# rslmtoasa/rslmtoasa

Hardware: AMD Instinct MI355X
Metric: block-recursion throughput (H|psi> + A_n + B_n recursion levels, recursion.f90 recur_b) (higher is better)
Workload: dtype f64

## Files before the change

### rslmtoasa_amd/csrc/kernels_mfma.hpp

```cpp
#pragma once
#include <hip/hip_runtime.h>
#include <string>
#include <vector>
#include "kernels_valu.hpp"

namespace rsrec {

typedef double double4_t __attribute__((ext_vector_type(4)));

constexpr int GROUP = 8;
constexpr int MF_WAVES = 4;

struct LayoutCI {
    static __device__ __forceinline__ double2 ld(const double* b, int r, int c) { return make_double2(b[36 * r + 2 * c], b[36 * r + 2 * c + 1]); }
    static __device__ __forceinline__ void st(double* b, int r, int c, double2 v) { b[36 * r + 2 * c] = v.x; b[36 * r + 2 * c + 1] = v.y; }
};
__host__ __device__ constexpr int gram_col(int part, int c, int ci) { return ci ? 2 * c + part : 18 * part + c; }

__device__ __forceinline__ int active_workgroups(int ngroups) { return max(1, min((int)gridDim.x, (ngroups + MF_WAVES - 1) / MF_WAVES)); }

struct GroupWalk {
    int g, end, step;
    __device__ __forceinline__ GroupWalk(int ngroups, int wave, int nbx_eff = 0) {
        const int nbx = nbx_eff > 0 ? nbx_eff : gridDim.x, bx = blockIdx.x;
        const int xcd = bx & 7, j = bx >> 3;
        const int per_xcd = (nbx >> 3) + ((xcd < (nbx & 7)) ? 1 : 0);
        const int chunk = (ngroups + 7) >> 3;
        const int lo = xcd * chunk;
        end = min(ngroups, lo + chunk);
        g = lo + j * MF_WAVES + wave;
        step = per_xcd * MF_WAVES;
        if (nbx < 8) { g = bx * MF_WAVES + wave; end = ngroups; step = nbx * MF_WAVES; }
    }
};


struct RowRef { unsigned off; bool valid; };
__device__ __forceinline__ RowRef group_row(const int* __restrict__ grp, int rho, int zero_block) {
    const int slot = rho / 18, r = rho - 18 * slot;
    const int a = grp[slot];
    RowRef R;
    R.valid = a >= 0;
    R.off = (unsigned)BLD * (unsigned)(R.valid ? a : zero_block) + 36u * (unsigned)r;
    return R;
}

struct GramAcc {
    double4_t t00, t01, t10, t11;
    double tr0, tr1;
    double t0r, t1r;
    double trr;
    __device__ __forceinline__ void zero() { t00 = t01 = t10 = t11 = (double4_t){0, 0, 0, 0}; tr0 = tr1 = t0r = t1r = trr = 0.0; }
    __device__ __forceinline__ void to_lds(double* G , int lane, bool sym) const {
        const int l15 = lane & 15, l4 = lane >> 4, l3 = lane & 3, lg = (lane >> 2) & 3;
#pragma unroll
        for (int j = 0; j < 4; ++j) {
            const int r = l4 + 4 * j;
            G[36 * r + l15] = t00[j];
            G[36 * r + 16 + l15] = t01[j];
            G[36 * (16 + r) + 16 + l15] = t11[j];
            if (!sym) G[36 * (16 + r) + l15] = t10[j];
        }
        G[36 * (32 + l4) + l15] = tr0;
        G[36 * (32 + l4) + 16 + l15] = tr1;
        if (!sym) { G[36 * (4 * lg + l4) + 32 + l3] = t0r; G[36 * (16 + 4 * lg + l4) + 32 + l3] = t1r; }
        if (lg == 0) G[36 * (32 + l4) + 32 + l3] = trr;
    }
};

__device__ __forceinline__ void gram_block_out(const GramAcc& A, double* lds , double* gout , bool sym) {
    const int lane = threadIdx.x & 63, wave = threadIdx.x >> 6;
    A.to_lds(lds + wave * 1296, lane, sym);
    __syncthreads();
    for (int e = threadIdx.x; e < 1296; e += blockDim.x) {
        double s = 0.0;
#pragma unroll
        for (int wv = 0; wv < MF_WAVES; ++wv) s += lds[wv * 1296 + e];
        if (sym) {
            const int r = e / 36, c = e % 36;
            const bool have = (r >= 32) || (r < 16) || (c >= 16 && c < 32);
            if (!have || (r < 32 && c >= 32)) {
                double t = 0.0;
#pragma unroll
                for (int wv = 0; wv < MF_WAVES; ++wv) t += lds[wv * 1296 + 36 * c + r];
                s = t;
            }
        }
        gout[e] = s;
    }
}

#ifndef RSREC_NT_STREAMS
#define RSREC_NT_STREAMS 0
#endif
template <class T> __device__ __forceinline__ T ld_stream(const T* p) {
#if RSREC_NT_STREAMS
    return __builtin_nontemporal_load(p);
#else
    return *p;
#endif
}
__device__ __forceinline__ double2 ld_stream(const double2* p) {
#if RSREC_NT_STREAMS
    typedef double nt_d2 __attribute__((ext_vector_type(2)));
    const nt_d2 v = __builtin_nontemporal_load(reinterpret_cast<const nt_d2*>(p));
    return make_double2(v[0], v[1]);
#else
    return *p;
#endif
}
template <class T> __device__ __forceinline__ void st_stream(T* p, T v) {
#if RSREC_NT_STREAMS
    __builtin_nontemporal_store(v, p);
#else
    *p = v;
#endif
}

#ifndef ADOT_UNROLL
#define ADOT_UNROLL 4
#endif
__global__ __launch_bounds__(MF_WAVES * 64, 2) void k_mfma_adot(ChainView CV, int level, int zero_block, const double* __restrict__ psi,
                                                               const double* __restrict__ tvec, double* partial ) {
    __shared__ double lds[MF_WAVES * 1296];
    const int chain = blockIdx.y;
    const int lane = threadIdx.x & 63;
    const int wave = __builtin_amdgcn_readfirstlane(threadIdx.x >> 6);
    const int ngroups = CV.count_of(chain, level) / GROUP;
    const int* order = CV.order_of(chain, level);
    const size_t vo = (size_t)chain * CV.vstride;
    const double* ps = psi + vo;
    const double* tv = tvec + vo;
    const int l15 = lane & 15, l4 = lane >> 4, l3 = lane & 3;
    GramAcc A;
    A.zero();
    const int nbx = active_workgroups(ngroups);
    for (GroupWalk w((int)blockIdx.x < nbx ? ngroups : 0, wave, nbx); w.g < w.end; w.g += w.step) {
        const int* grp = order + (size_t)w.g * GROUP;
#pragma unroll ADOT_UNROLL
        for (int kq = 0; kq < 36; ++kq) {
            const RowRef rk = group_row(grp, 4 * kq + l4, zero_block);
            const double p0 = ld_stream(ps + rk.off + l15), p1 = ld_stream(ps + rk.off + 16 + l15), pr = ld_stream(ps + rk.off + 32 + l3);
            const double h0 = ld_stream(tv + rk.off + l15), h1 = ld_stream(tv + rk.off + 16 + l15), hr = ld_stream(tv + rk.off + 32 + l3);
            A.t00 = __builtin_amdgcn_mfma_f64_16x16x4f64(p0, h0, A.t00, 0, 0, 0);
            A.t01 = __builtin_amdgcn_mfma_f64_16x16x4f64(p0, h1, A.t01, 0, 0, 0);
            A.t10 = __builtin_amdgcn_mfma_f64_16x16x4f64(p1, h0, A.t10, 0, 0, 0);
            A.t11 = __builtin_amdgcn_mfma_f64_16x16x4f64(p1, h1, A.t11, 0, 0, 0);
            A.tr0 = __builtin_amdgcn_mfma_f64_4x4x4f64(pr, h0, A.tr0, 0, 0, 0);
            A.tr1 = __builtin_amdgcn_mfma_f64_4x4x4f64(pr, h1, A.tr1, 0, 0, 0);
            A.t0r = __builtin_amdgcn_mfma_f64_4x4x4f64(p0, hr, A.t0r, 0, 0, 0);
            A.t1r = __builtin_amdgcn_mfma_f64_4x4x4f64(p1, hr, A.t1r, 0, 0, 0);
            A.trr = __builtin_amdgcn_mfma_f64_4x4x4f64(pr, hr, A.trr, 0, 0, 0);
        }
    }
    gram_block_out(A, lds, partial + ((size_t)chain * gridDim.x + blockIdx.x) * 1296, false);
}

struct SpmmDims {
    int kk, nslots, nmax, nlev, cpo, ostride, level; size_t vstride; const int* obase; int nchains = 0;
    int sat_base = 0, run_lo = 0, run_hi = 0, nskip = 0, skip_lo[4] = {0, 0, 0, 0}, skip_hi[4] = {0, 0, 0, 0};
    int nruns = 0, run_tau[4] = {0, 0, 0, 0}, run_glo[4] = {0, 0, 0, 0}, run_ghi[4] = {0, 0, 0, 0}, run_row0[5] = {0, 0, 0, 0, 0};
    int skip_pa = 0;
};

__device__ __forceinline__ double2 reduce_gram(const double* __restrict__ partial , int nblk, double* lds , int ci = 0) {
    for (int e = threadIdx.x; e < 1296; e += blockDim.x) {
        double s = 0.0;
        for (int p = 0; p < nblk; ++p) s += partial[(size_t)p * 1296 + e];
        lds[e] = s;
    }
    __syncthreads();
    double2 c = make_double2(0, 0);
    if (threadIdx.x < BLK) {
        const int cp = threadIdx.x % NB, cc = threadIdx.x / NB;
        const int rp = gram_col(0, cp, ci), ip = gram_col(1, cp, ci), rc = gram_col(0, cc, ci), ic = gram_col(1, cc, ci);
        c.x = lds[36 * rp + rc] + lds[36 * ip + ic];
        c.y = lds[36 * rp + ic] - lds[36 * ip + rc];
    }
    __syncthreads();
    return c;
}

}
```

### rslmtoasa_amd/csrc/kernels_spmm5.hpp

```cpp
#pragma once
#include <hip/hip_runtime.h>
#include <algorithm>
#include <type_traits>
#include <vector>
#include "kernels_valu.hpp"
#include "kernels_mfma.hpp"
#include "kernels_spmm4.hpp"

namespace rsrec {

#ifndef RSREC_S5_KSPLIT_PROBE
#define RSREC_S5_KSPLIT_PROBE 0
#endif
#ifndef RSREC_S5_PRIO
#define RSREC_S5_PRIO 0
#endif
#ifndef S5_WG_GROUPS
#define S5_WG_GROUPS 4
#endif
constexpr int S5_TRIPLE = 640;
constexpr int S5_TRIPLE_BYTES = S5_TRIPLE * 8;
constexpr int S5_HEAD_TRIPLES = 2;
constexpr int S5_HEAD_DOUBLES = 2 * S5_HEAD_TRIPLES * S5_TRIPLE;
constexpr int S5_MAXENT = 2 * S4_MAXSLOTS + 2;
// ... 262 lines not shown
struct S5Acc { double4_t m[9]; double r[9]; };

struct S5Ent { unsigned off[GROUP]; unsigned rem; };

template <int S> struct S5St {
    static constexpr int T = S / 3, K = S % 3;
    static constexpr int W = K == 2 ? 2 : 4;
    static constexpr int o0 = 10 * T + (K == 0 ? 0 : K == 1 ? 4 : 8);
    static constexpr int eA = o0 / 9, mA0 = o0 % 9, sp = 9 - mA0;
    static constexpr bool straddle = sp < W;
    static constexpr bool opens = straddle || mA0 == 0;
    static constexpr int eOpen = mA0 == 0 ? eA : eA + 1;
};

template <int NL, int NM>
__device__ __forceinline__ void s5_interleave() {
    constexpr int PER = NM / NL;
#pragma unroll
    for (int i = 0; i < NL; ++i) {
        __builtin_amdgcn_sched_group_barrier(0x20, 1, 0);
        __builtin_amdgcn_sched_group_barrier(0x8, PER, 0);
    }
    __builtin_amdgcn_sched_group_barrier(0x8, NM - PER * NL, 0);
}

template <int NL = 11>
__device__ __forceinline__ void s5_mfma(S5Acc& acc, const S5Pair& o) {
#pragma unroll
    for (int e = 0; e < 2; ++e)
#pragma unroll
        for (int t = 0; t < 9; ++t) {
            acc.m[t] = __builtin_amdgcn_mfma_f64_16x16x4f64(o.a[0][e], o.b[t][e], acc.m[t], 0, 0, 0);
            acc.r[t] = __builtin_amdgcn_mfma_f64_4x4x4f64(o.a[1][e], o.b[t][e], acc.r[t], 0, 0, 0);
        }
    s5_interleave<NL, 36>();
}
template <int NL = 11>
__device__ __forceinline__ void s5_mfma(S5Acc& acc, const S5Single& o) {
#pragma unroll
    for (int t = 0; t < 9; ++t) {
        acc.m[t] = __builtin_amdgcn_mfma_f64_16x16x4f64(o.a[0], o.b[t], acc.m[t], 0, 0, 0);
        acc.r[t] = __builtin_amdgcn_mfma_f64_4x4x4f64(o.a[1], o.b[t], acc.r[t], 0, 0, 0);
    }
    s5_interleave<NL, 18>();
}

template <int N> using S5C = std::integral_constant<int, N>;
#define S5_GLOBAL __attribute__((address_space(1)))
#define S5_CONST __attribute__((address_space(4)))
#define S5_LDS __attribute__((address_space(3)))
typedef const S5_GLOBAL char* s5_gp;

template <bool TWO, bool LDSA, bool OCT = false>
__device__ __forceinline__ void s5_run_stream(S5Acc& acc, const int* __restrict__ meta, const char* __restrict__ fr , const char* __restrict__ fr_head,
                                              const char* __restrict__ inb, const char* __restrict__ in2b,
                                              const int* __restrict__ nbr5 ,
                                              const int (&atom)[GROUP] , int rem_sel ,
                                              int ncol, int sig, int l4,
                                              unsigned lane_main, unsigned lane_z, unsigned lane_rem, unsigned lane_rem_z, unsigned lane16, unsigned lane8,
                                              const int (&tile_blk)[GROUP], int rem_blk , int kpart = 0) {
    int left = meta[0];
    int ebase = 0, tbase = 0;
    bool first = true;
#if RSREC_S5_KSPLIT_PROBE
    if (kpart == 0) left = min(left, 27);
    else { left -= 27; ebase = 10; tbase = 9; first = false; }
#endif
    if (left <= 0) return;
    const bool extras = TWO && meta[1] != 0;
    const S5_CONST int* codes = (const S5_CONST int*)(meta + 2);
    const S5_CONST int* nbr = (const S5_CONST int*)nbr5;
    S5Ent E0, E1;
    int raw[GROUP];
    int code_cur = codes[ebase], code_nxt = codes[ebase + 1];
    auto load_idx = [&](int col) {
#pragma unroll
        for (int t = 0; t < GROUP; ++t) raw[t] = nbr[(size_t)ncol * atom[t] + col];
    };
    load_idx(code_cur & 255);
    unsigned vlane_main = lane_main, vlane_z = lane_z, vlane16 = lane16, vlane8 = lane8;
    auto open_entry = [&](int j, S5Ent& E) {
        const unsigned so = 2592u * (unsigned)((code_cur >> 8) ? 1 - sig : sig);
#pragma unroll
        for (int t = 0; t < GROUP; ++t) E.off[t] = (unsigned)(OCT ? raw[t] + tile_blk[t] : raw[t]) * (BLD * 8u) + so;
        const int r01 = (rem_sel & 1) ? raw[1] : raw[0], r23 = (rem_sel & 1) ? raw[3] : raw[2], r45 = (rem_sel & 1) ? raw[5] : raw[4], r67 = (rem_sel & 1) ? raw[7] : raw[6];
        const int r03 = (rem_sel & 2) ? r23 : r01, r47 = (rem_sel & 2) ? r67 : r45;
        E.rem = (unsigned)(((rem_sel & 4) ? r47 : r03) + (OCT ? rem_blk : 0)) * (BLD * 8u) + so;
        code_cur = code_nxt;
        code_nxt = codes[j + 2];
        load_idx(code_cur & 255);
    };
    auto issue = [&](auto s2c, auto& o) {
        constexpr int S2 = decltype(s2c)::value, S = S2 % 27, wrap = S2 / 27;
        using I = S5St<S>;
        S5Ent& EA = (I::eA & 1) ? E1 : E0;
        S5Ent& EB = (I::eA & 1) ? E0 : E1;
        if constexpr (I::opens) open_entry(ebase + 10 * wrap + I::eOpen, (I::eOpen & 1) ? E1 : E0);
        const bool head = wrap == 0 && first && extras;
        const char* __restrict__ base = (TWO && S < 5 && head) ? in2b : inb;
        s5_gp fbg = nullptr;
        if constexpr (!LDSA) {
            const char* fb = ((TWO && I::T < S5_HEAD_TRIPLES && head && fr_head) ? fr_head + I::T * S5_TRIPLE_BYTES
                                                                                 : fr + (size_t)(tbase + 9 * wrap + I::T) * S5_TRIPLE_BYTES)
                             + (I::K == 0 ? 0 : I::K == 1 ? 2048 : 4096);
            fbg = (s5_gp)fb;
            asm("" : "+s"(fbg));
        }
        constexpr unsigned rowA = 288u * I::mA0, rowB = 0u - 288u * I::sp;
        unsigned& lm = I::K < 2 ? vlane_main : vlane_z;
        unsigned& lf = I::K < 2 ? vlane16 : vlane8;
        const unsigned lr = I::K < 2 ? lane_rem : lane_rem_z;
        asm volatile("" : "+v"(lm));
        asm volatile("" : "+v"(lf));
        using V = std::remove_reference_t<decltype(o.b[0])>;
        if constexpr (!I::straddle) {
#pragma unroll
            for (int t = 0; t < GROUP; ++t) {
                s5_gp pt = (s5_gp)base + EA.off[t];
                asm("" : "+s"(pt));
                o.b[t] = *(const S5_GLOBAL V*)(pt + lm + rowA);
            }
            o.b[8] = *(const S5_GLOBAL V*)((s5_gp)base + (EA.rem + lr) + rowA);
        } else {
            const bool inB = (I::K < 2 ? l4 : (l4 >> 1)) >= I::sp;
#pragma unroll
            for (int t = 0; t < GROUP; ++t) {
                const unsigned off = (inB ? EB.off[t] + rowB : EA.off[t] + rowA) + lm;
                o.b[t] = *(const S5_GLOBAL V*)((s5_gp)base + off);
            }
            const unsigned off = (inB ? EB.rem + rowB : EA.rem + rowA) + lr;
            o.b[8] = *(const S5_GLOBAL V*)((s5_gp)base + off);
        }
        if constexpr (LDSA) {
            const S5_LDS char* fl = (const S5_LDS char*)fr + (unsigned)(tbase + 9 * wrap + I::T) * S5_TRIPLE_BYTES + (I::K == 0 ? 0 : I::K == 1 ? 2048 : 4096);
#pragma unroll
            for (int q = 0; q < 2; ++q) o.a[q] = *(const S5_LDS V*)(fl + lf + q * (I::K < 2 ? 1024 : 512));
        } else if constexpr (I::K < 2) {
#pragma unroll
            for (int q = 0; q < 2; ++q) o.a[q] = *(const S5_GLOBAL V*)(fbg + lf + q * 1024);
        } else {
#pragma unroll
            for (int q = 0; q < 2; ++q) o.a[q] = *(const S5_GLOBAL V*)(fbg + lf + q * 512);
        }
    };
    S5Pair X, Y;
    S5Single Z;
    issue(S5C<0>{}, X);
    issue(S5C<1>{}, Y);
#define S5_STEP(S, NEXT, CUR)                 \
    if (left > (S)) {                         \
        issue(S5C<(S) + 2>{}, NEXT);          \
        s5_mfma<LDSA ? 9 : 11>(acc, CUR);     \
        __builtin_amdgcn_sched_barrier(0);    \
    }
    for (;; left -= 27) {
        S5_STEP(0, Z, X) S5_STEP(1, X, Y) S5_STEP(2, Y, Z) S5_STEP(3, Z, X) S5_STEP(4, X, Y) S5_STEP(5, Y, Z)
        S5_STEP(6, Z, X) S5_STEP(7, X, Y) S5_STEP(8, Y, Z) S5_STEP(9, Z, X) S5_STEP(10, X, Y) S5_STEP(11, Y, Z)
        S5_STEP(12, Z, X) S5_STEP(13, X, Y) S5_STEP(14, Y, Z) S5_STEP(15, Z, X) S5_STEP(16, X, Y) S5_STEP(17, Y, Z)
        S5_STEP(18, Z, X) S5_STEP(19, X, Y) S5_STEP(20, Y, Z) S5_STEP(21, Z, X) S5_STEP(22, X, Y) S5_STEP(23, Y, Z)
        S5_STEP(24, Z, X) S5_STEP(25, X, Y) S5_STEP(26, Y, Z)
        if (left <= 27) break;
        ebase += 10; tbase += 9; first = false;
    }
#undef S5_STEP
}


template <int NT> struct S5PairN { s5_d2 b[NT]; s5_d2 a[2]; };
template <int NT> struct S5SingleN { double b[NT]; double a[2]; };
template <int NT> struct S5AccN { double4_t m[NT]; double r[NT]; };

template <int NT>
__device__ __forceinline__ void s5_mfma_n(S5AccN<NT>& acc, const S5PairN<NT>& o) {
#pragma unroll
    for (int e = 0; e < 2; ++e)
#pragma unroll
        for (int t = 0; t < NT; ++t) {
            acc.m[t] = __builtin_amdgcn_mfma_f64_16x16x4f64(o.a[0][e], o.b[t][e], acc.m[t], 0, 0, 0);
            acc.r[t] = __builtin_amdgcn_mfma_f64_4x4x4f64(o.a[1][e], o.b[t][e], acc.r[t], 0, 0, 0);
        }
    s5_interleave<NT, 4 * NT>();
}
template <int NT>
__device__ __forceinline__ void s5_mfma_n(S5AccN<NT>& acc, const S5SingleN<NT>& o) {
#pragma unroll
    for (int t = 0; t < NT; ++t) {
        acc.m[t] = __builtin_amdgcn_mfma_f64_16x16x4f64(o.a[0], o.b[t], acc.m[t], 0, 0, 0);
        acc.r[t] = __builtin_amdgcn_mfma_f64_4x4x4f64(o.a[1], o.b[t], acc.r[t], 0, 0, 0);
    }
    s5_interleave<NT, 2 * NT>();
}

struct S5EntN { unsigned off[3]; unsigned rem; };

template <bool TWO, int NMAIN, bool HASREM>
__device__ __forceinline__ void s5_run_stream_n(S5AccN<NMAIN + (HASREM ? 1 : 0)>& acc, const int* __restrict__ meta, const char* __restrict__ fr ,
                                                const char* __restrict__ inb, const char* __restrict__ in2b, const int* __restrict__ nbr5,
                                                const int (&atom)[NMAIN], const int (&ratom)[GROUP], int rem_sel, int ncol, int sig, int l4,
                                                unsigned lane_main, unsigned lane_z, unsigned lane_rem, unsigned lane_rem_z, unsigned lane16, unsigned lane8) {
    constexpr int NT = NMAIN + (HASREM ? 1 : 0);
    int left = meta[0];
    int ebase = 0, tbase = 0;
    bool first = true;
    if (left <= 0) return;
    const bool extras = TWO && meta[1] != 0;
    const S5_CONST int* codes = (const S5_CONST int*)(meta + 2);
    const S5_CONST int* nbr = (const S5_CONST int*)nbr5;
    S5EntN E0, E1;
    int raw[NMAIN], rraw[GROUP];
    int code_cur = codes[ebase], code_nxt = codes[ebase + 1];
    auto load_idx = [&](int col) {
#pragma unroll
        for (int t = 0; t < NMAIN; ++t) raw[t] = nbr[(size_t)ncol * atom[t] + col];
        if constexpr (HASREM) {
#pragma unroll
            for (int t = 0; t < GROUP; ++t) rraw[t] = nbr[(size_t)ncol * ratom[t] + col];
        }
    };
    load_idx(code_cur & 255);
    unsigned vlane_main = lane_main, vlane_z = lane_z, vlane16 = lane16, vlane8 = lane8;
    auto open_entry = [&](int j, S5EntN& E) {
        const unsigned so = 2592u * (unsigned)((code_cur >> 8) ? 1 - sig : sig);
#pragma unroll
        for (int t = 0; t < NMAIN; ++t) E.off[t] = (unsigned)raw[t] * (BLD * 8u) + so;
        if constexpr (HASREM) {
            const int r01 = (rem_sel & 1) ? rraw[1] : rraw[0], r23 = (rem_sel & 1) ? rraw[3] : rraw[2], r45 = (rem_sel & 1) ? rraw[5] : rraw[4], r67 = (rem_sel & 1) ? rraw[7] : rraw[6];
            const int r03 = (rem_sel & 2) ? r23 : r01, r47 = (rem_sel & 2) ? r67 : r45;
            E.rem = (unsigned)((rem_sel & 4) ? r47 : r03) * (BLD * 8u) + so;
        }
        code_cur = code_nxt;
        code_nxt = codes[j + 2];
        load_idx(code_cur & 255);
    };
    auto issue = [&](auto s2c, auto& o) {
        constexpr int S2 = decltype(s2c)::value, S = S2 % 27, wrap = S2 / 27;
        using I = S5St<S>;
        S5EntN& EA = (I::eA & 1) ? E1 : E0;
        S5EntN& EB = (I::eA & 1) ? E0 : E1;
        if constexpr (I::opens) open_entry(ebase + 10 * wrap + I::eOpen, (I::eOpen & 1) ? E1 : E0);
        const bool head = wrap == 0 && first && extras;
        const char* __restrict__ base = (TWO && S < 5 && head) ? in2b : inb;
        constexpr unsigned rowA = 288u * I::mA0, rowB = 0u - 288u * I::sp;
        unsigned& lm = I::K < 2 ? vlane_main : vlane_z;
        unsigned& lf = I::K < 2 ? vlane16 : vlane8;
        const unsigned lr = I::K < 2 ? lane_rem : lane_rem_z;
        asm volatile("" : "+v"(lm));
        asm volatile("" : "+v"(lf));
        using V = std::remove_reference_t<decltype(o.b[0])>;
        if constexpr (!I::straddle) {
#pragma unroll
            for (int t = 0; t < NMAIN; ++t) {
                s5_gp pt = (s5_gp)base + EA.off[t];
                asm("" : "+s"(pt));
                o.b[t] = *(const S5_GLOBAL V*)(pt + lm + rowA);
            }
            if constexpr (HASREM) o.b[NMAIN] = *(const S5_GLOBAL V*)((s5_gp)base + (EA.rem + lr) + rowA);
        } else {
            const bool inB = (I::K < 2 ? l4 : (l4 >> 1)) >= I::sp;
#pragma unroll
            for (int t = 0; t < NMAIN; ++t) {
                const unsigned off = (inB ? EB.off[t] + rowB : EA.off[t] + rowA) + lm;
                o.b[t] = *(const S5_GLOBAL V*)((s5_gp)base + off);
            }
            if constexpr (HASREM) {
                const unsigned off = (inB ? EB.rem + rowB : EA.rem + rowA) + lr;
                o.b[NMAIN] = *(const S5_GLOBAL V*)((s5_gp)base + off);
            }
        }
        const S5_LDS char* fl = (const S5_LDS char*)fr + (unsigned)(tbase + 9 * wrap + I::T) * S5_TRIPLE_BYTES + (I::K == 0 ? 0 : I::K == 1 ? 2048 : 4096);
#pragma unroll
        for (int q = 0; q < 2; ++q) o.a[q] = *(const S5_LDS V*)(fl + lf + q * (I::K < 2 ? 1024 : 512));
    };
    S5PairN<NT> X0, Y0, X1, Y1;
    S5SingleN<NT> Z0, Z1;
    issue(S5C<0>{}, X0);
    issue(S5C<1>{}, Y0);
    issue(S5C<2>{}, Z0);
    issue(S5C<3>{}, X1);
    issue(S5C<4>{}, Y1);
#define S5_STEP(S, NEXT, CUR)                 \
    if (left > (S)) {                         \
        issue(S5C<(S) + 5>{}, NEXT);          \
        s5_mfma_n<NT>(acc, CUR);              \
        __builtin_amdgcn_sched_barrier(0);    \
    }
    for (;; left -= 54) {
        S5_STEP(0, Z1, X0) S5_STEP(1, X0, Y0) S5_STEP(2, Y0, Z0) S5_STEP(3, Z0, X1) S5_STEP(4, X1, Y1) S5_STEP(5, Y1, Z1)
        S5_STEP(6, Z1, X0) S5_STEP(7, X0, Y0) S5_STEP(8, Y0, Z0) S5_STEP(9, Z0, X1) S5_STEP(10, X1, Y1) S5_STEP(11, Y1, Z1)
        S5_STEP(12, Z1, X0) S5_STEP(13, X0, Y0) S5_STEP(14, Y0, Z0) S5_STEP(15, Z0, X1) S5_STEP(16, X1, Y1) S5_STEP(17, Y1, Z1)
        S5_STEP(18, Z1, X0) S5_STEP(19, X0, Y0) S5_STEP(20, Y0, Z0) S5_STEP(21, Z0, X1) S5_STEP(22, X1, Y1) S5_STEP(23, Y1, Z1)
        S5_STEP(24, Z1, X0) S5_STEP(25, X0, Y0) S5_STEP(26, Y0, Z0) S5_STEP(27, Z0, X1) S5_STEP(28, X1, Y1) S5_STEP(29, Y1, Z1)
        S5_STEP(30, Z1, X0) S5_STEP(31, X0, Y0) S5_STEP(32, Y0, Z0) S5_STEP(33, Z0, X1) S5_STEP(34, X1, Y1) S5_STEP(35, Y1, Z1)
        S5_STEP(36, Z1, X0) S5_STEP(37, X0, Y0) S5_STEP(38, Y0, Z0) S5_STEP(39, Z0, X1) S5_STEP(40, X1, Y1) S5_STEP(41, Y1, Z1)
        S5_STEP(42, Z1, X0) S5_STEP(43, X0, Y0) S5_STEP(44, Y0, Z0) S5_STEP(45, Z0, X1) S5_STEP(46, X1, Y1) S5_STEP(47, Y1, Z1)
        S5_STEP(48, Z1, X0) S5_STEP(49, X0, Y0) S5_STEP(50, Y0, Z0) S5_STEP(51, Z0, X1) S5_STEP(52, X1, Y1) S5_STEP(53, Y1, Z1)
        if (left <= 54) break;
        ebase += 20; tbase += 18; first = false;
    }
#undef S5_STEP
}

struct S5Epilogue { int kind = 0; const double* cur = nullptr; const double* old = nullptr; double a = 1.0, b = 0.0; };

template <bool TWO, bool LDSA, bool OCT = false, int NSP = 1>
__global__ __launch_bounds__(NSP == 3 ? 768 : S5_WG_GROUPS * 128) void k_spmm5(SpmmDims D, const int* __restrict__ order_all, const int* __restrict__ cum,
                                               const int* __restrict__ nbr ,
                                               const int* __restrict__ izp, const double* __restrict__ frag, const int* __restrict__ meta, int ntr,
                                               const double* __restrict__ in_all, double* __restrict__ out_all,
                                               const double* __restrict__ in2_all = nullptr,
                                               const double* __restrict__ frag_head = nullptr ,
                                               int ntau = 0, int lds_tau = 0 ,
                                               int* __restrict__ queue = nullptr ,
                                               int spin_by_xcd = 1 ,
                                               S5Epilogue epi = S5Epilogue()) {
    extern __shared__ double s5_lds[];
    const int lane = threadIdx.x & 63;
    const int wave = __builtin_amdgcn_readfirstlane(threadIdx.x >> 6);
    const int sig = LDSA ? (int)((spin_by_xcd ? blockIdx.x : (blockIdx.x >> 3)) & 1) : wave / S5_WG_GROUPS, gslot = LDSA ? wave : wave % S5_WG_GROUPS;
#if RSREC_S5_PRIO
    if (wave >= (int)(blockDim.x >> 7)) __builtin_amdgcn_s_setprio(1);
#endif
    const int WGG = LDSA ? (int)(blockDim.x >> 6) : S5_WG_GROUPS;
    int bxl = blockIdx.x, gdxl = gridDim.x, run_lo = D.run_lo, run_hi = D.run_hi, qrun = 0;
    if (LDSA && D.nruns > 0) {
        const int row = spin_by_xcd ? 8 : 16, rowi = (int)blockIdx.x / row;
        int r = 0;
#pragma unroll
        for (int q = 1; q < 4; ++q) if (q < D.nruns && rowi >= D.run_row0[q]) r = q;
        lds_tau = D.run_tau[r]; run_lo = D.run_glo[r]; run_hi = D.run_ghi[r];
        bxl = (int)blockIdx.x - row * D.run_row0[r];
        gdxl = row * (D.run_row0[r + 1] - D.run_row0[r]);
        qrun = r;
    }
    if constexpr (LDSA) {
        const s5_d2* __restrict__ src = reinterpret_cast<const s5_d2*>(frag + ((size_t)lds_tau * 2 + sig) * ntr * S5_TRIPLE);
        s5_d2* dst = reinterpret_cast<s5_d2*>(s5_lds);
        const int n = ntr * (S5_TRIPLE / 2);
        constexpr int PER = (int)(160 * 1024 / 16 / (NSP == 3 ? 512 : S5_WG_GROUPS * 64));
        const int nthr = (int)blockDim.x;
        s5_d2 v[PER];
#pragma unroll
        for (int i = 0; i < PER; ++i) { const int e = threadIdx.x + i * nthr; if (e < n) v[i] = src[e]; }
#pragma unroll
        for (int i = 0; i < PER; ++i) { const int e = threadIdx.x + i * nthr; if (e < n) dst[e] = v[i]; }
        __syncthreads();
    }
    const int l15 = lane & 15, l4 = lane >> 4;
    const unsigned lane_main = 8u * (36 * l4 + 2 * l15), lane_z = 8u * (36 * (l4 >> 1) + 2 * l15 + (l4 & 1));
    const unsigned lane_rem = 8u * (36 * l4 + 32 + 2 * (l15 & 1)), lane_rem_z = 8u * (36 * (l4 >> 1) + 32 + 2 * (l15 & 1) + (l4 & 1));
    const unsigned lane16 = 16u * lane, lane8 = 8u * lane;
    const int ncol = D.nslots + 2;
#pragma unroll 1
    for (int chain = OCT ? GROUP * (int)blockIdx.y : (int)blockIdx.y; chain < D.nchains; chain += OCT ? GROUP * (int)gridDim.y : (int)gridDim.y) {
    const int count = cum[(chain / D.cpo) * D.nlev + D.level];
    int ngroups = count / GROUP;
    const int ob = D.obase[(chain / D.cpo) * D.nlev + D.level];
    const int* __restrict__ order = order_all + (size_t)(chain / D.cpo) * D.ostride + ob;
    const bool on_full_list = D.sat_base > 0 && ob == D.sat_base;
    if constexpr (OCT) ngroups = D.nmax;
    else if (run_hi > 0) {
        if (!on_full_list) continue;
        order += (size_t)run_lo * GROUP;
        ngroups = run_hi - run_lo;
    }
    const bool skipping = D.nskip > 0 && on_full_list;
    const size_t vo = (size_t)chain * D.vstride;
    const char* __restrict__ inb = reinterpret_cast<const char*>(in_all + vo);
    const char* __restrict__ in2b = TWO ? reinterpret_cast<const char*>(in2_all + vo) : nullptr;
    double* __restrict__ out = out_all + vo;
    const int zero_block = D.kk;

    int g, gend, gstep, glo = 0;
    bool dynamic = false;
    {
        const int bx = bxl;
        const int need = (ngroups + WGG - 1) / WGG;
        if constexpr (!LDSA) {
            const int nbx = max(1, min((int)gridDim.x, need));
            if (bx >= nbx) continue;
            if (nbx < 8) { g = bx * WGG + gslot; gend = ngroups; gstep = nbx * WGG; }
            else {
                const int xcd = bx & 7, j = bx >> 3;
                const int per_xcd = (nbx >> 3) + ((xcd < (nbx & 7)) ? 1 : 0);
                const int chunk = (ngroups + 7) >> 3;
                const int lo = xcd * chunk;
                gend = min(ngroups, lo + chunk);
                g = lo + j * WGG + gslot;
                gstep = per_xcd * WGG;
            }
        } else {
            const int row = spin_by_xcd ? 8 : 16;
            const int nbx = max(row, min(gdxl / row * row, (2 * need + row - 1) / row * row));
            if (bx >= nbx) continue;
            const int xcd = bx & 7, j = bx >> 3;
            if (2 * need <= row) {
                const int per_spin = row / 2, idx = spin_by_xcd ? (xcd >> 1) : xcd;
                if (j >= row / 8) continue;
                g = idx * WGG + gslot; gend = ngroups; gstep = per_spin * WGG;
            } else {
                const int rows = nbx / row;
                const int nchunk = spin_by_xcd ? 4 : 8, ichunk = spin_by_xcd ? (xcd >> 1) : xcd;
                const int chunk = (ngroups + nchunk - 1) / nchunk;
                const int lo = ichunk * chunk;
                gend = min(ngroups, lo + chunk);
                g = lo + (spin_by_xcd ? j : (j >> 1)) * WGG + gslot;
                gstep = rows * WGG;
                glo = lo;
                dynamic = queue != nullptr;
            }
        }
    }
    int* __restrict__ ctr = dynamic ? queue + ((size_t)qrun * D.nchains + chain) * 16 + 2 * (blockIdx.x & 7) + (spin_by_xcd ? 0 : sig) : nullptr;
    int part = 0;
    auto next_task = [&]() {
        if (NSP == 3 && !dynamic && part < 2) { ++part; return; }
        part = 0; g += gstep;
    };
    for (;; next_task()) {
        int kpart = 0;
        if (dynamic) {
            int gi = 0;
            if (lane == 0) gi = atomicAdd(ctr, 1);
            gi = __builtin_amdgcn_readfirstlane(gi);
#if RSREC_S5_KSPLIT_PROBE
            kpart = gi & 1; gi >>= 1;
#endif
            if constexpr (NSP == 3) { const unsigned gu = (unsigned)gi, gq = gu / 3u; part = (int)(gu - 3u * gq); gi = (int)gq; }
            g = glo + gi;
        }
        if (g >= gend) break;
        if (skipping) {
            bool skip = false;
#pragma unroll
            for (int r = 0; r < 4; ++r) skip |= r < D.nskip && g >= D.skip_lo[r] && g < D.skip_hi[r];
            if (skip) continue;
        }
        const int* __restrict__ grp = order + (size_t)g * GROUP;
        if constexpr (NSP == 3) {
            static_assert(NSP != 3 || (LDSA && !OCT), "split tasks: LDS / persistent form only");
            const int g0 = grp[0];
            const int first3 = g0 >= 0 ? g0 : zero_block;
            if (D.skip_pa && first3 < D.nmax) continue;
            const int tau3 = first3 < D.nmax ? first3 : D.nmax + izp[first3];
            const int* __restrict__ M3 = meta + (size_t)tau3 * Spmm5Operator::META;
            const char* __restrict__ fr3 = reinterpret_cast<const char*>(s5_lds);
            S5AccN<3> acc3;
#pragma unroll
            for (int t = 0; t < 3; ++t) { acc3.m[t] = (double4_t){0, 0, 0, 0}; acc3.r[t] = 0.0; }
            auto finish3 = [&](auto remc, const int (&av)[3]) {
                constexpr bool REM = decltype(remc)::value;
                size_t eo[3];
#pragma unroll
                for (int i = 0; i < 3; ++i) eo[i] = (size_t)BLD * av[i] + 324 * sig + ((REM && i == 2) ? 32 + 2 * (l15 & 1) : 2 * l15);
                s5_d2 ec[3][2], ez[3][2];
                double ecr[3], ezr[3];
                if (epi.kind) {
                    const double* cb = epi.cur + vo;
#pragma unroll
                    for (int i = 0; i < 3; ++i) {
#pragma unroll
                        for (int p = 0; p < 2; ++p) ec[i][p] = *reinterpret_cast<const s5_d2*>(cb + eo[i] + 36 * (4 * p + l4));
                        ecr[i] = cb[eo[i] + 288 + (l4 & 1)];
                    }
                    if (epi.kind == 2) {
                        const double* zb = epi.old + vo;
#pragma unroll
                        for (int i = 0; i < 3; ++i) {
#pragma unroll
                            for (int p = 0; p < 2; ++p) ez[i][p] = *reinterpret_cast<const s5_d2*>(zb + eo[i] + 36 * (4 * p + l4));
                            ezr[i] = zb[eo[i] + 288 + (l4 & 1)];
                        }
                    }
                }
#pragma unroll
                for (int i = 0; i < 3; ++i) {
                    const int a = av[i];
                    double* ob = out + eo[i];
#pragma unroll
                    for (int p = 0; p < 2; ++p) {
                        s5_d2 v; v[0] = acc3.m[i][2 * p]; v[1] = acc3.m[i][2 * p + 1];
                        if (epi.kind) {
                            v[0] = (v[0] - epi.b * ec[i][p][0]) / epi.a; v[1] = (v[1] - epi.b * ec[i][p][1]) / epi.a;
                            if (epi.kind == 2) { v[0] = v[0] * 2.0 - ez[i][p][0]; v[1] = v[1] * 2.0 - ez[i][p][1]; }
                        }
                        if (a != zero_block) *reinterpret_cast<s5_d2*>(ob + 36 * (4 * p + l4)) = v;
                    }
                    double r = acc3.r[i];
                    if (epi.kind) {
                        r = (r - epi.b * ecr[i]) / epi.a;
                        if (epi.kind == 2) r = r * 2.0 - ezr[i];
                    }
                    if (a != zero_block && l4 < 2) ob[288 + l4] = r;
                }
            };
            int ratom[GROUP];
            if (part < 2) {
                int a3[3];
#pragma unroll
                for (int j = 0; j < 3; ++j) { const int a = grp[3 * part + j]; a3[j] = a >= 0 ? a : zero_block; }
#pragma unroll
                for (int t = 0; t < GROUP; ++t) ratom[t] = zero_block;
                s5_run_stream_n<TWO, 3, false>(acc3, M3, fr3, inb, in2b, nbr, a3, ratom, 0, ncol, sig, l4, lane_main, lane_z, lane_rem, lane_rem_z, lane16, lane8);
                finish3(std::false_type{}, a3);
            } else {
#pragma unroll
                for (int t = 0; t < GROUP; ++t) { const int a = grp[t]; ratom[t] = a >= 0 ? a : zero_block; }
                const int a2[2] = {ratom[6], ratom[7]};
                int mra = grp[l15 >> 1];
                mra = mra >= 0 ? mra : zero_block;
                s5_run_stream_n<TWO, 2, true>(acc3, M3, fr3, inb, in2b, nbr, a2, ratom, l15 >> 1, ncol, sig, l4, lane_main, lane_z, lane_rem, lane_rem_z, lane16, lane8);
                const int av[3] = {a2[0], a2[1], mra};
                finish3(std::true_type{}, av);
            }
            continue;
        }
        int atom[GROUP];
        int vatom[GROUP], tile_blk[GROUP];
        int my_rem_atom, rem_blk = 0;
        if constexpr (OCT) {
            const int a0 = g;
#pragma unroll
            for (int t = 0; t < GROUP; ++t) {
                const bool ok = a0 >= 0 && chain + t < D.nchains;
                atom[t] = ok ? a0 : zero_block;
                tile_blk[t] = ok ? t * (D.kk + 1) : 0;
                vatom[t] = ok ? a0 + t * (D.kk + 1) : zero_block;
            }
            const int tr = l15 >> 1;
            const bool okr = a0 >= 0 && chain + tr < D.nchains;
            rem_blk = okr ? tr * (D.kk + 1) : 0;
            my_rem_atom = okr ? a0 + tr * (D.kk + 1) : zero_block;
        } else {
#pragma unroll
            for (int t = 0; t < GROUP; ++t) { const int a = grp[t]; atom[t] = a >= 0 ? a : zero_block; vatom[t] = atom[t]; tile_blk[t] = 0; }
            my_rem_atom = grp[l15 >> 1];
            my_rem_atom = my_rem_atom >= 0 ? my_rem_atom : zero_block;
        }
        const int first = atom[0];
        if (!OCT && D.skip_pa && first < D.nmax) continue;
        const int tau = first < D.nmax ? first : D.nmax + izp[first];
        const int* __restrict__ M = meta + (size_t)tau * Spmm5Operator::META;
        const char* __restrict__ fr = LDSA ? reinterpret_cast<const char*>(s5_lds) : reinterpret_cast<const char*>(frag + ((size_t)tau * 2 + sig) * ntr * S5_TRIPLE);
        const char* __restrict__ fh = (TWO && frag_head) ? reinterpret_cast<const char*>(frag_head + ((size_t)chain * ntau + tau) * S5_HEAD_DOUBLES + (size_t)sig * S5_HEAD_TRIPLES * S5_TRIPLE) : nullptr;

        S5Acc acc;
#pragma unroll
        for (int t = 0; t < 9; ++t) { acc.m[t] = (double4_t){0, 0, 0, 0}; acc.r[t] = 0.0; }

        if constexpr (OCT) s5_run_stream<TWO, LDSA, true>(acc, M, fr, fh, inb, in2b, nbr, atom, l15 >> 1, ncol, sig, l4, lane_main, lane_z, lane_rem, lane_rem_z, lane16, lane8, tile_blk, rem_blk);
        else s5_run_stream<TWO, LDSA>(acc, M, fr, fh, inb, in2b, nbr, atom, l15 >> 1, ncol, sig, l4, lane_main, lane_z, lane_rem, lane_rem_z, lane16, lane8, tile_blk, rem_blk, kpart);
#if RSREC_S5_KSPLIT_PROBE
        if (kpart) continue;
#endif

        auto finish = [&](auto t0c, auto t1c) {
            constexpr int T0 = decltype(t0c)::value, T1 = decltype(t1c)::value, NT = T1 - T0;
            size_t eo[NT];
#pragma unroll
            for (int i = 0; i < NT; ++i) { const int t = T0 + i; eo[i] = (size_t)BLD * ((t < 8) ? vatom[t] : my_rem_atom) + 324 * sig + ((t < 8) ? 2 * l15 : 32 + 2 * (l15 & 1)); }
            s5_d2 ec[NT][2], ez[NT][2];
            double ecr[NT], ezr[NT];
            if (epi.kind) {
                const double* cb = epi.cur + vo;
#pragma unroll
                for (int i = 0; i < NT; ++i) {
#pragma unroll
                    for (int p = 0; p < 2; ++p) ec[i][p] = *reinterpret_cast<const s5_d2*>(cb + eo[i] + 36 * (4 * p + l4));
                    ecr[i] = cb[eo[i] + 288 + (l4 & 1)];
                }
                if (epi.kind == 2) {
                    const double* zb = epi.old + vo;
#pragma unroll
                    for (int i = 0; i < NT; ++i) {
#pragma unroll
                        for (int p = 0; p < 2; ++p) ez[i][p] = *reinterpret_cast<const s5_d2*>(zb + eo[i] + 36 * (4 * p + l4));
                        ezr[i] = zb[eo[i] + 288 + (l4 & 1)];
                    }
                }
            }
#pragma unroll
            for (int i = 0; i < NT; ++i) {
                const int t = T0 + i;
                const int a = (t < 8) ? vatom[t] : my_rem_atom;
                double* ob = out + eo[i];
#pragma unroll
                for (int p = 0; p < 2; ++p) {
                    s5_d2 v; v[0] = acc.m[t][2 * p]; v[1] = acc.m[t][2 * p + 1];
                    if (epi.kind) {
                        v[0] = (v[0] - epi.b * ec[i][p][0]) / epi.a; v[1] = (v[1] - epi.b * ec[i][p][1]) / epi.a;
                        if (epi.kind == 2) { v[0] = v[0] * 2.0 - ez[i][p][0]; v[1] = v[1] * 2.0 - ez[i][p][1]; }
                    }
                    if (a != zero_block) *reinterpret_cast<s5_d2*>(ob + 36 * (4 * p + l4)) = v;
                }
                double r = acc.r[t];
                if (epi.kind) {
                    r = (r - epi.b * ecr[i]) / epi.a;
                    if (epi.kind == 2) r = r * 2.0 - ezr[i];
                }
                if (a != zero_block && l4 < 2) ob[288 + l4] = r;
            }
        };
        finish(S5C<0>{}, S5C<5>{});
        finish(S5C<5>{}, S5C<9>{});
    }
    }
}

}
```

### rslmtoasa_amd/csrc/rsrec.hip

```cpp
#include <hip/hip_runtime.h>
#include <hsa/hsa.h>
#include <hsa/hsa_ext_amd.h>
#include <dlfcn.h>
#include <algorithm>
#include <atomic>
#include <chrono>
#include <cmath>
#include <cstdarg>
#include <cstdio>
#include <cstdlib>
#include <cstring>
#include <memory>
#include <string>
#include <thread>
#include <tuple>
#include <vector>

#include "../../include/rsrec.h"
#include "kernels_valu.hpp"
#include "kernels_mfma.hpp"
#include "kernels_spmm4.hpp"
#include "kernels_spmm5.hpp"
#include "kernels_uscheme.hpp"
#include "kernels_green.hpp"
#include "kernels_ldos.hpp"
#include "kernels_spectra.hpp"
#include "kernels_kubo.hpp"
#include "kernels_cond.hpp"
#include "kernels_exchange.hpp"
#include "kernels_auxgreen.hpp"
#include "kernels_contour.hpp"
#include "kernels_assemble.hpp"

using namespace rsrec;

namespace {

struct DevBuf {
    void* p = nullptr;
    size_t bytes = 0;
    DevBuf() = default;
    DevBuf(DevBuf&& o) noexcept : p(o.p), bytes(o.bytes) { o.p = nullptr; o.bytes = 0; }
    DevBuf& operator=(DevBuf&& o) noexcept { std::swap(p, o.p); std::swap(bytes, o.bytes); return *this; }
    ~DevBuf() { release(); }
    hipError_t reserve(size_t n) {
        if (n <= bytes) return hipSuccess;
        release();
        hipError_t e = hipMalloc(&p, n);
        if (e == hipSuccess) bytes = n;
        return e;
    }
    void release() { if (p) (void)hipFree(p); p = nullptr; bytes = 0; }
    template <class T> T* as() const { return reinterpret_cast<T*>(p); }
};

}

struct rsrec_handle {
    int device = 0;
    hipStream_t stream = nullptr;
    hipStream_t copy_stream = nullptr;
    hipEvent_t ev_green[2] = {nullptr, nullptr};
    hipStream_t side_stream = nullptr;
    hipEvent_t ev_orth = nullptr, ev_bred = nullptr;
    hipStream_t oct_stream = nullptr;
    hipEvent_t ev_oct_in = nullptr, ev_oct_out = nullptr;
    size_t p2_slot = 0;
    std::string err;
    bool have_lattice = false, have_ham = false;
    std::vector<int32_t> lat_nn, lat_iz;
    int lat_nncols = 0;
    std::vector<double> lat_cr;
    int kk = 0, nslots = 0, nmax = 0, ntype = 0;
    std::vector<int> nbr;
    std::vector<int> iz0;
    std::vector<int> radj_ptr, radj;
    DevBuf d_nbr, d_iz, d_nbr5;
    int hslots = 0, hoh = 0, nsp = 2;
    DevBuf d_hst, d_hloc, d_host, d_holoc, d_enim, d_lsham;
    Spmm4Operator s4_op;
    int s4_built_split = 0;
    Spmm5Operator s5_op;
    DevBuf d_s5queue;
    int s5_built = 0;
    size_t s5_lds_limit = (size_t)-1;
    int n_cu = 0;
    bool s4_attr = false;
    size_t term_lds = 0, cheb_ldos_lds = (size_t)64 * 1024, cheb_spec_lds = (size_t)64 * 1024;
    std::vector<double> host_ee, host_lsham, host_eeo, host_enim, host_hall, host_hallo;
    std::vector<double> host_st, host_loc;
    DevBuf d_asm[2][2], d_asm_in;
    std::vector<double> asm_host[2][2];
    int asm_nslots[2] = {0, 0}, asm_ncls[2] = {0, 0}, asm_hoh[2] = {0, 0};
    int n_octet_launch = 0;
    int n_asm_reused = 0;
    long n_asm_calls = 0, n_ldos_calls = 0, n_recursion_calls = 0;
    Spmm5Operator s5_la; int s5_la_ok = 0;
    DevBuf d_la_extra, d_rot;
    Spmm5Operator kubo_op[2], kubo_hbulk;
    Spmm5Operator orb_plain;
    DevBuf d_green_in, d_green_out;
    DevBuf d_kubo[5];
    DevBuf d_cond[4];
    DevBuf d_ctens[2];
    DevBuf d_bsqrt, d_term, d_gim, d_ldos;
    DevBuf d_ops, d_spec;
    void* pin = nullptr;
    size_t pin_bytes = 0;
    DevBuf d_frags, d_vec[6], d_partial, d_partial2, d_coefA, d_coefB, d_bmats, d_status, d_seed, d_seedcoef, d_mu, d_scal, d_zsqr;
    long opt_batch = 0, opt_kernels = 0, opt_nblk = 0, opt_spmm5 = 2, opt_chain_fold = 1, opt_s5_cap = 0, opt_side = 1, opt_s5_lds = 1, opt_s5_queue = 1, opt_cheb_fused = 1;
    long opt_s5_waves = 8;
    long opt_sat_pct = 100;
    long opt_orth_oop = 1;
    long opt_s5_split = 0;
    long opt_s5_run_min = 0;
    long opt_s5_spin_xcd = 0;
    long opt_s5_octet = 8;
    long opt_s5_host_emit = 0;
    long opt_kubo_lchunk = 0;
    long opt_kubo_vbatch = 0;
    int n_kubo_left_chunks = 0;
    int kubo_diag_nvec = 0, kubo_diag_ll = 0;
    long opt_orth3 = 1;
    long opt_graph = 1;
    hipGraphExec_t graph_exec = nullptr;
    std::vector<uintptr_t> graph_key;
    bool capturing = false;
    double t_total_ms = 0, t_hop_ms = 0, t_rest_ms = 0, t_host_ms = 0;
    double t_rot_ms = 0;
    double n_hop_launch = 0, n_atom_steps = 0, n_block_mult = 0, n_hop_mfma_flop = 0;
    double n_req_flop = 0;
    int hop_fuses_a = 1;
    std::vector<hipEvent_t> ev_pool;
    size_t ev_used = 0;
    struct RegionEntry {
        std::vector<int> seeds;
        int nlev, napply, flags, epoch, ostride;
        double atom_steps, block_mults;
        DevBuf order, cum;
        std::vector<int> level_max;
        std::vector<double> level_groups;
        std::vector<double> mult_hist;
        struct ClassRun { int tau, lo, hi; };
        std::vector<ClassRun> sat_runs;
        std::vector<int> level_sat;
        int sat_base = 0;
    };
    std::vector<std::unique_ptr<RegionEntry>> region_cache;
    int lattice_epoch = 0;
    const int* cur_order = nullptr;
    const int* cur_cum = nullptr;
    const std::vector<int>* cur_level_max = nullptr;
    const std::vector<double>* cur_level_groups = nullptr;
    const std::vector<double>* cur_mult_hist = nullptr;
    const RegionEntry* cur_entry = nullptr;
    int cur_nrows = 0;
    std::vector<unsigned> spatial_key;
    int res_kind = 0, res_n = 0, res_lld = 0;
    bool res_seeded = false;
    void* comm = nullptr;
    int comm_rank = 0, comm_nranks = 1;
    DevBuf d_comm;
    ~rsrec_handle();
};

namespace {

struct OptionEntry { const char* name; long rsrec_handle::*member; };
const OptionEntry OPTIONS[] = {
    {"batch", &rsrec_handle::opt_batch},
    {"kernels", &rsrec_handle::opt_kernels},
    {"nblk", &rsrec_handle::opt_nblk},
    {"spmm5", &rsrec_handle::opt_spmm5},
    {"chain_fold", &rsrec_handle::opt_chain_fold},
    {"s5_cap", &rsrec_handle::opt_s5_cap},
    {"s5_lds", &rsrec_handle::opt_s5_lds},
    {"s5_queue", &rsrec_handle::opt_s5_queue},
    {"cheb_fused", &rsrec_handle::opt_cheb_fused},
    {"side_stream", &rsrec_handle::opt_side},
    {"graph", &rsrec_handle::opt_graph},
    {"orth3", &rsrec_handle::opt_orth3},
    {"s5_waves", &rsrec_handle::opt_s5_waves},
    {"s5_split", &rsrec_handle::opt_s5_split},
    {"orth_oop", &rsrec_handle::opt_orth_oop},
    {"sat_pct", &rsrec_handle::opt_sat_pct},
    {"kubo_lchunk", &rsrec_handle::opt_kubo_lchunk},
    {"kubo_vbatch", &rsrec_handle::opt_kubo_vbatch},
    {"s5_host_emit", &rsrec_handle::opt_s5_host_emit},
    {"s5_octet", &rsrec_handle::opt_s5_octet},
    {"s5_spin_xcd", &rsrec_handle::opt_s5_spin_xcd},
    {"s5_run_min", &rsrec_handle::opt_s5_run_min},
};

int fail(rsrec_t* h, int code, const char* fmt, ...) {
    char buf[512];
    va_list ap;
    va_start(ap, fmt);
    vsnprintf(buf, sizeof buf, fmt, ap);
    va_end(ap);
    if (h) h->err = buf;
    return code;
}

#define HIPCK(h, call)                                                                                         \
    do {                                                                                                       \
        hipError_t e_ = (call);                                                                                \
        if (e_ != hipSuccess) return fail(h, RSREC_ERR_DEVICE, "%s failed: %s (%s:%d)", #call, hipGetErrorString(e_), __FILE__, __LINE__); \
    } while (0)

hipEvent_t next_event(rsrec_t* h) {
    static const bool off = getenv("RSREC_NO_EVENTS") != nullptr;
    if (off || h->capturing) return nullptr;
    if (h->ev_used == h->ev_pool.size()) {
        hipEvent_t e;
        if (hipEventCreate(&e) != hipSuccess) return nullptr;
        h->ev_pool.push_back(e);
    }
    hipEvent_t e = h->ev_pool[h->ev_used++];
    (void)hipEventRecord(e, h->stream);
    return e;
}

constexpr size_t PIN_BYTES = (size_t)8 << 20;
int pin_ready(rsrec_t* h) {
    if (h->pin) return RSREC_OK;
    if (hipHostMalloc(&h->pin, PIN_BYTES, hipHostMallocDefault) != hipSuccess) { h->pin = nullptr; return fail(h, RSREC_ERR_DEVICE, "hipHostMalloc of the staging buffer failed"); }
    h->pin_bytes = PIN_BYTES;
    return RSREC_OK;
}
constexpr size_t PIN_MAX_XFER = (size_t)8 << 20;
int xfer_d2h(rsrec_t* h, void* dst, const void* src_dev, size_t bytes) {
    if (bytes > PIN_MAX_XFER) {
        HIPCK(h, hipMemcpyAsync(dst, src_dev, bytes, hipMemcpyDeviceToHost, h->stream));
        HIPCK(h, hipStreamSynchronize(h->stream));
        return RSREC_OK;
    }
    int rc = pin_ready(h);
    if (rc) return rc;
    for (size_t off = 0; off < bytes; off += h->pin_bytes) {
        const size_t n = std::min(h->pin_bytes, bytes - off);
        HIPCK(h, hipMemcpyAsync(h->pin, static_cast<const char*>(src_dev) + off, n, hipMemcpyDeviceToHost, h->stream));
        HIPCK(h, hipStreamSynchronize(h->stream));
        memcpy(static_cast<char*>(dst) + off, h->pin, n);
    }
    return RSREC_OK;
}
int xfer_h2d(rsrec_t* h, void* dst_dev, const void* src, size_t bytes) {
    if (bytes > PIN_MAX_XFER) {
        HIPCK(h, hipMemcpyAsync(dst_dev, src, bytes, hipMemcpyHostToDevice, h->stream));
        HIPCK(h, hipStreamSynchronize(h->stream));
        return RSREC_OK;
    }
    int rc = pin_ready(h);
    if (rc) return rc;
    for (size_t off = 0; off < bytes; off += h->pin_bytes) {
        const size_t n = std::min(h->pin_bytes, bytes - off);
        memcpy(h->pin, static_cast<const char*>(src) + off, n);
        HIPCK(h, hipMemcpyAsync(static_cast<char*>(dst_dev) + off, h->pin, n, hipMemcpyHostToDevice, h->stream));
        HIPCK(h, hipStreamSynchronize(h->stream));
    }
    return RSREC_OK;
}
#define XFER(call) do { int rc__ = (call); if (rc__) return rc__; } while (0)

struct Region {
    std::vector<int> order;
    std::vector<int> cum;
};

void grow_region(const rsrec_t* h, const int* seeds, int nseed, int nlev, Region& R) {
    const int kk = h->kk;
    std::vector<int> dist(kk, -1);
    R.order.clear();
    R.order.reserve(kk);
    R.cum.assign(nlev, 0);
    std::vector<int> frontier, next;
    for (int s = 0; s < nseed; ++s)
        if (dist[seeds[s]] < 0) { dist[seeds[s]] = 0; frontier.push_back(seeds[s]); }
    std::sort(frontier.begin(), frontier.end());
    int level = 0;
    while (!frontier.empty() && level < nlev) {
        R.order.insert(R.order.end(), frontier.begin(), frontier.end());
        R.cum[level] = (int)R.order.size();
        next.clear();
        for (int n : frontier)
            for (int q = h->radj_ptr[n]; q < h->radj_ptr[n + 1]; ++q) {
                const int i = h->radj[q];
                if (dist[i] < 0) { dist[i] = level + 1; next.push_back(i); }
            }
        std::sort(next.begin(), next.end());
        frontier.swap(next);
        ++level;
    }
    for (int L = std::max(level, 1); L < nlev; ++L) R.cum[L] = R.cum[L - 1];
    R.order.resize(kk, 0);
}

inline unsigned spread3(unsigned v) {
    v &= 1023u;
    v = (v | (v << 16)) & 0x030000FFu;
    v = (v | (v << 8)) & 0x0300F00Fu;
    v = (v | (v << 4)) & 0x030C30C3u;
    v = (v | (v << 2)) & 0x09249249u;
    return v;
}
inline unsigned morton3(unsigned x, unsigned y, unsigned z) { return spread3(x) | (spread3(y) << 1) | (spread3(z) << 2); }

void bfs_dist(const rsrec_t* h, int start, std::vector<int>& dist) {
    const int kk = h->kk, ns = h->nslots;
    dist.assign(kk, -1);
    std::vector<int> cur{start}, nxt;
    dist[start] = 0;
    int d = 0;
    while (!cur.empty()) {
        nxt.clear();
        for (int n : cur) {
            for (int j = 1; j < ns; ++j) { const int i = h->nbr[(size_t)n * ns + j]; if (i >= 0 && dist[i] < 0) { dist[i] = d + 1; nxt.push_back(i); } }
            for (int q = h->radj_ptr[n]; q < h->radj_ptr[n + 1]; ++q) { const int i = h->radj[q]; if (dist[i] < 0) { dist[i] = d + 1; nxt.push_back(i); } }
        }
        cur.swap(nxt);
        ++d;
    }
}

void spatial_key_from_graph(rsrec_t* h) {
    const int kk = h->kk;
    std::vector<int> d0, d1, d2;
    bfs_dist(h, 0, d0);
    int l1 = 0;
    for (int i = 0; i < kk; ++i) if (d0[i] >= d0[l1]) l1 = i;
    bfs_dist(h, l1, d1);
    int l2 = 0, best = -1;
    for (int i = 0; i < kk; ++i) { const int m = std::min(d0[i], d1[i]); if (m >= best) { best = m; l2 = i; } }
    bfs_dist(h, l2, d2);
    h->spatial_key.resize(kk);
    for (int i = 0; i < kk; ++i) h->spatial_key[i] = morton3((unsigned)std::max(d0[i], 0), (unsigned)std::max(d1[i], 0), (unsigned)std::max(d2[i], 0));
}

}

extern "C" int rsrec_version(void) { return 101; }

extern "C" int rsrec_device_count(void) {
    int n = 0;
    if (hipGetDeviceCount(&n) != hipSuccess) return 0;
    return n;
}

static rsrec_handle* g_report_handle = nullptr;
static void report_at_exit() {
    const rsrec_handle* h = g_report_handle;
    if (!h) return;
    std::printf("rsrec report: library_calls=%ld device_assemblies=%ld operator_arrays_from_device=%d device_ldos_calls=%ld\n", h->n_recursion_calls, h->n_asm_calls,
                h->n_asm_reused, h->n_ldos_calls);
    std::fflush(stdout);
}

extern "C" int rsrec_create(rsrec_t** out, int device) {
    if (!out) return RSREC_ERR_ARG;
    *out = nullptr;
    int ndev = 0;
    if (hipGetDeviceCount(&ndev) != hipSuccess || ndev <= 0) return RSREC_ERR_DEVICE;
    if (device < 0 || device >= ndev) return RSREC_ERR_ARG;
    if (hipSetDevice(device) != hipSuccess) return RSREC_ERR_DEVICE;
    rsrec_t* h = new rsrec_handle();
    h->device = device;
    if (hipStreamCreateWithFlags(&h->stream, hipStreamNonBlocking) != hipSuccess) { delete h; return RSREC_ERR_DEVICE; }
    if (hipDeviceGetAttribute(&h->n_cu, hipDeviceAttributeMultiprocessorCount, device) != hipSuccess || h->n_cu <= 0) h->n_cu = 256;
    *out = h;
    if (getenv("RSREC_REPORT") && !g_report_handle) {
        static bool registered = false;
        if (!registered) { registered = std::atexit(report_at_exit) == 0; }
        g_report_handle = h;
    }
    return RSREC_OK;
}

rsrec_handle::~rsrec_handle() {
    (void)hipSetDevice(device);
    if (stream) (void)hipStreamSynchronize(stream);
    if (graph_exec) (void)hipGraphExecDestroy(graph_exec);
    (void)rsrec_comm_destroy(this);
    for (hipEvent_t e : ev_pool) (void)hipEventDestroy(e);
    for (hipStream_t s : {stream, copy_stream, side_stream, oct_stream}) if (s) (void)hipStreamDestroy(s);
    for (hipEvent_t e : {ev_green[0], ev_green[1], ev_orth, ev_bred, ev_oct_in, ev_oct_out}) if (e) (void)hipEventDestroy(e);
    if (pin) (void)hipHostFree(pin);
}

extern "C" int rsrec_destroy(rsrec_t* h) {
    if (!h) return RSREC_ERR_ARG;
    if (g_report_handle == h) { report_at_exit(); g_report_handle = nullptr; }
    delete h;
    return RSREC_OK;
}

extern "C" int rsrec_last_error(rsrec_t* h, char* buf, size_t n) {
    if (!h || !buf || n == 0) return RSREC_ERR_ARG;
    snprintf(buf, n, "%s", h->err.c_str());
    return RSREC_OK;
}

extern "C" int rsrec_set_option(rsrec_t* h, const char* key, long value) {
    if (!h || !key) return RSREC_ERR_ARG;
    for (const OptionEntry& o : OPTIONS)
        if (!strcmp(key, o.name)) { h->*o.member = value; return RSREC_OK; }
    return fail(h, RSREC_ERR_ARG, "unknown option '%s'", key);
}

extern "C" int rsrec_get_timing(rsrec_t* h, double* out, int n) {
    if (!h || !out) return RSREC_ERR_ARG;
    const double v[13] = {h->t_total_ms, h->t_hop_ms, h->n_hop_launch, h->n_atom_steps, h->n_block_mult, h->t_rest_ms, h->t_host_ms, (double)h->hop_fuses_a, h->n_hop_mfma_flop,
                          h->n_req_flop, (double)h->n_asm_reused, (double)h->n_octet_launch, h->t_rot_ms};
    for (int i = 0; i < n && i < 13; ++i) out[i] = v[i];
    return RSREC_OK;
}

extern "C" void rsrec_site_partition(int rank, int nprocs, int nsites, int* start_atom, int* end_atom) {
    int per = nsites / nprocs;
    const int rem = nsites % nprocs;
    int start;
    if (rank < rem) { per += 1; start = rank * per + 1; }
    else start = rank * per + rem + 1;
    *start_atom = start;
    *end_atom = start + per - 1;
}

static void release_graph(rsrec_t* h) {
    if (h->graph_exec) { (void)hipDeviceSynchronize(); (void)hipGraphExecDestroy(h->graph_exec); h->graph_exec = nullptr; }
    h->graph_key.clear();
}

static void release_regions(rsrec_t* h) {
    release_graph(h);
    if (!h->region_cache.empty()) (void)hipDeviceSynchronize();
    h->region_cache.clear();
    h->cur_order = nullptr; h->cur_cum = nullptr; h->cur_entry = nullptr; h->cur_level_max = nullptr; h->cur_level_groups = nullptr; h->cur_mult_hist = nullptr;
}

extern "C" int rsrec_set_lattice(rsrec_t* h, int kk, int nncols, const int32_t* nn, const int32_t* iz, int nmax, int ntype) {
    if (!h || !nn || !iz || kk <= 0 || nncols < 1 || nmax < 0 || nmax > kk || ntype < 1) return fail(h, RSREC_ERR_ARG, "rsrec_set_lattice: bad argument");
    HIPCK(h, hipSetDevice(h->device));
    if (h->have_lattice && kk == h->kk && nncols == h->lat_nncols && nmax == h->nmax && ntype == h->ntype &&
        h->lat_nn.size() == (size_t)kk * nncols && std::memcmp(h->lat_nn.data(), nn, h->lat_nn.size() * sizeof(int32_t)) == 0 &&
        std::memcmp(h->lat_iz.data(), iz, (size_t)kk * sizeof(int32_t)) == 0)
        return RSREC_OK;
    int nslots = 1;
    for (int i = 0; i < kk; ++i) {
        const int nr = nn[i];
        if (nr < 0 || nr > nncols) return fail(h, RSREC_ERR_ARG, "rsrec_set_lattice: nn(%d,1)=%d outside 0..%d", i + 1, nr, nncols);
        nslots = std::max(nslots, nr);
        if (iz[i] < 1 || iz[i] > ntype) return fail(h, RSREC_ERR_ARG, "rsrec_set_lattice: iz(%d)=%d outside 1..%d", i + 1, iz[i], ntype);
    }
    std::vector<int> nbr_new((size_t)kk * nslots, -1), iz_new(kk), deg(kk + 1, 0);
    for (int i = 0; i < kk; ++i) {
        iz_new[i] = iz[i] - 1;
        nbr_new[(size_t)i * nslots] = i;
        const int nr = nn[i];
        for (int j = 1; j < nr; ++j) {
            const int n = nn[(size_t)i + (size_t)kk * j];
            if (n == 0) continue;
            if (n < 0 || n > kk) return fail(h, RSREC_ERR_ARG, "rsrec_set_lattice: nn(%d,%d)=%d outside 0..%d", i + 1, j + 1, n, kk);
            nbr_new[(size_t)i * nslots + j] = n - 1;
            deg[n - 1]++;
        }
    }
    h->have_lattice = false;
    h->have_ham = false;
    h->kubo_diag_nvec = h->kubo_diag_ll = 0;
    h->lat_nn.clear(); h->lat_iz.clear();
    release_regions(h);
    h->kk = kk; h->nslots = nslots; h->nmax = nmax; h->ntype = ntype;
    h->nbr.swap(nbr_new);
    h->iz0.swap(iz_new);
    h->radj_ptr.assign(kk + 1, 0);
    for (int n = 0; n < kk; ++n) h->radj_ptr[n + 1] = h->radj_ptr[n] + deg[n];
    h->radj.resize(h->radj_ptr[kk]);
    std::vector<int> fill(h->radj_ptr.begin(), h->radj_ptr.end() - 1);
    for (int i = 0; i < kk; ++i)
        for (int j = 1; j < nslots; ++j) {
            const int n = h->nbr[(size_t)i * nslots + j];
            if (n >= 0) h->radj[fill[n]++] = i;
        }
    HIPCK(h, h->d_nbr.reserve(h->nbr.size() * sizeof(int)));
    HIPCK(h, h->d_iz.reserve((size_t)kk * sizeof(int)));
    HIPCK(h, hipMemcpy(h->d_nbr.p, h->nbr.data(), h->nbr.size() * sizeof(int), hipMemcpyHostToDevice));
    HIPCK(h, hipMemcpy(h->d_iz.p, h->iz0.data(), (size_t)kk * sizeof(int), hipMemcpyHostToDevice));
    {
        std::vector<int> n5((size_t)(kk + 1) * (nslots + 2), kk);
        for (int i = 0; i < kk; ++i) {
            for (int j = 0; j < nslots; ++j) { const int n = h->nbr[(size_t)i * nslots + j]; if (n >= 0) n5[(size_t)i * (nslots + 2) + j] = n; }
            n5[(size_t)i * (nslots + 2) + nslots] = i;
        }
        HIPCK(h, h->d_nbr5.reserve(n5.size() * sizeof(int)));
        HIPCK(h, hipMemcpy(h->d_nbr5.p, n5.data(), n5.size() * sizeof(int), hipMemcpyHostToDevice));
    }
    spatial_key_from_graph(h);
    h->lat_nn.assign(nn, nn + (size_t)kk * nncols);
    h->lat_iz.assign(iz, iz + kk);
    h->lat_nncols = nncols;
    h->lat_cr.clear();
    h->have_lattice = true;
    h->lattice_epoch++;
    h->have_ham = false;
    return RSREC_OK;
}

extern "C" int rsrec_set_positions(rsrec_t* h, const double* cr) {
    if (!h || !cr) return fail(h, RSREC_ERR_ARG, "rsrec_set_positions: bad argument");
    if (!h->have_lattice) return fail(h, RSREC_ERR_ARG, "rsrec_set_positions: call rsrec_set_lattice first");
    const int kk = h->kk;
    if (h->lat_cr.size() == 3 * (size_t)kk && std::memcmp(h->lat_cr.data(), cr, h->lat_cr.size() * sizeof(double)) == 0) return RSREC_OK;
    h->lat_cr.assign(cr, cr + 3 * (size_t)kk);
    double lo[3] = {1e300, 1e300, 1e300}, hi[3] = {-1e300, -1e300, -1e300};
    for (int i = 0; i < kk; ++i)
        for (int a = 0; a < 3; ++a) { lo[a] = std::min(lo[a], cr[3 * (size_t)i + a]); hi[a] = std::max(hi[a], cr[3 * (size_t)i + a]); }
    double span = 1e-300;
    for (int a = 0; a < 3; ++a) span = std::max(span, hi[a] - lo[a]);
    h->spatial_key.resize(kk);
    for (int i = 0; i < kk; ++i) {
        unsigned q[3];
        for (int a = 0; a < 3; ++a) q[a] = (unsigned)std::min(1023.0, std::max(0.0, (cr[3 * (size_t)i + a] - lo[a]) / span * 1023.0));
        h->spatial_key[i] = morton3(q[0], q[1], q[2]);
    }
    h->lattice_epoch++;
    release_regions(h);
    return RSREC_OK;
}

extern "C" int rsrec_set_hamiltonian(rsrec_t* h, int nslots, int hoh, int nsp, const double* ee, const double* lsham, const double* eeo,
                                     const double* enim, const double* hall, const double* hallo) {
    if (!h) return RSREC_ERR_ARG;
    if (!h->have_lattice) return fail(h, RSREC_ERR_ARG, "rsrec_set_hamiltonian: call rsrec_set_lattice first");
    if (!ee || !lsham || nslots < h->nslots) return fail(h, RSREC_ERR_ARG, "rsrec_set_hamiltonian: ee/lsham missing or nslots=%d < lattice slots %d", nslots, h->nslots);
    if (hoh && (!eeo || !enim)) return fail(h, RSREC_ERR_ARG, "rsrec_set_hamiltonian: hoh requires eeo and enim");
    if (h->nmax > 0 && (!hall || (hoh && !hallo))) return fail(h, RSREC_ERR_ARG, "rsrec_set_hamiltonian: nmax>0 requires hall (and hallo with hoh)");
    HIPCK(h, hipSetDevice(h->device));
    const size_t B = 2 * (size_t)BLK;
    const int ntype = h->ntype, nmax = h->nmax;
    h->hslots = nslots; h->hoh = hoh ? 1 : 0; h->nsp = nsp;
    h->kubo_diag_nvec = h->kubo_diag_ll = 0;
    h->host_ee.assign(ee, ee + 2 * (size_t)BLK * nslots * h->ntype);
    h->host_lsham.assign(lsham, lsham + 2 * (size_t)BLK * h->ntype);
    h->host_eeo.clear(); h->host_enim.clear(); h->host_hall.clear(); h->host_hallo.clear();
    if (hoh) { h->host_eeo.assign(eeo, eeo + 2 * (size_t)BLK * nslots * h->ntype); h->host_enim.assign(enim, enim + 2 * (size_t)BLK * h->ntype); }
    if (h->nmax > 0) { h->host_hall.assign(hall, hall + 2 * (size_t)BLK * nslots * h->nmax); if (hoh) h->host_hallo.assign(hallo, hallo + 2 * (size_t)BLK * nslots * h->nmax); }
    h->s5_la_ok = 0;
    std::vector<double> st(ee, ee + B * nslots * ntype);
    if (!hoh)
        for (int t = 0; t < ntype; ++t)
            for (size_t e = 0; e < B; ++e) st[B * nslots * t + e] += lsham[B * t + e];
    h->n_asm_reused = 0;
    auto resident = [&](int part, int which, const double* arr, int ncls) -> const double* {
        const size_t n = B * nslots * ncls;
        if (!arr || h->asm_nslots[part] != nslots || h->asm_ncls[part] != ncls || h->asm_host[part][which].size() != n) return nullptr;
        if (std::memcmp(arr, h->asm_host[part][which].data(), n * 8) != 0) return nullptr;
        h->n_asm_reused++;
        return h->d_asm[part][which].as<double>();
    };
    auto place = [&](DevBuf& dst, const double* dev_src, const double* host_src, size_t n) -> hipError_t {
        hipError_t e = dst.reserve(n * 8);
        if (e != hipSuccess) return e;
        if (dev_src) return hipMemcpyAsync(dst.p, dev_src, n * 8, hipMemcpyDeviceToDevice, h->stream);
        return hipMemcpy(dst.p, host_src, n * 8, hipMemcpyHostToDevice);
    };
    HIPCK(h, h->d_lsham.reserve(B * ntype * 8));
    HIPCK(h, hipMemcpy(h->d_lsham.p, lsham, B * ntype * 8, hipMemcpyHostToDevice));
    {
        const double* dev = resident(0, 0, ee, ntype);
        HIPCK(h, place(h->d_hst, dev, st.data(), st.size()));
        if (dev && !hoh) k_fold_onsite<<<ntype, 324, 0, h->stream>>>(h->d_hst.as<double2>(), nslots, h->d_lsham.as<double2>(), nullptr);
    }
    std::vector<double> loc;
    if (nmax > 0) {
        loc.assign(hall, hall + B * nslots * nmax);
        if (!hoh)
            for (int i = 0; i < nmax; ++i)
                for (size_t e = 0; e < B; ++e) loc[B * nslots * i + e] += lsham[B * h->iz0[i] + e];
        const double* dev = resident(1, 0, hall, nmax);
        HIPCK(h, place(h->d_hloc, dev, loc.data(), loc.size()));
        if (dev && !hoh) k_fold_onsite<<<nmax, 324, 0, h->stream>>>(h->d_hloc.as<double2>(), nslots, h->d_lsham.as<double2>(), h->d_iz.as<int>());
    }
    if (hoh) {
        HIPCK(h, place(h->d_host, resident(0, 1, eeo, ntype), eeo, B * nslots * ntype));
        HIPCK(h, h->d_enim.reserve(B * ntype * 8));
        HIPCK(h, hipMemcpy(h->d_enim.p, enim, B * ntype * 8, hipMemcpyHostToDevice));
        if (nmax > 0) HIPCK(h, place(h->d_holoc, resident(1, 1, hallo, nmax), hallo, B * nslots * nmax));
    }
    HIPCK(h, hipGetLastError());
    {
        h->s4_built_split = 0; h->s5_built = 0;
        if (h->nslots + 1 <= S4_MAXSLOTS) {
            h->host_st.swap(st);
            h->host_loc.swap(loc);
            const double* dev[6] = {h->d_hst.as<double>(), h->d_hloc.as<double>(), h->d_host.as<double>(), h->d_holoc.as<double>(), h->d_enim.as<double>(), h->d_lsham.as<double>()};
            const char* msg = h->s5_op.build(h->nslots, nslots, ntype, nmax, h->hoh, h->host_st.data(), nmax > 0 ? h->host_loc.data() : nullptr, hoh ? eeo : nullptr,
                                             (hoh && nmax > 0) ? hallo : nullptr, hoh ? enim : nullptr, lsham, h->iz0.data(), h->opt_s5_host_emit ? nullptr : dev, h->stream);
            if (msg) return fail(h, RSREC_ERR_DEVICE, "rsrec_set_hamiltonian: %s", msg);
            h->s5_built = 1;
        }
    }
    h->have_ham = true;
    return RSREC_OK;
}

extern "C" int rsrec_assemble_blocks(rsrec_t* h, int part, int ncls, int nslots, int hoh, const double* hmag, const int32_t* nbr_type, const double* obarm, int ntype,
                                     double* blocks, double* blocks_o) {
    if (!h) return RSREC_ERR_ARG;
    if (part < 0 || part > 1 || ncls < 1 || nslots < 1 || !hmag || !blocks) return fail(h, RSREC_ERR_ARG, "rsrec_assemble_blocks: part=%d ncls=%d nslots=%d or a missing array", part, ncls, nslots);
    if (hoh && (!nbr_type || !obarm || !blocks_o || ntype < 1)) return fail(h, RSREC_ERR_ARG, "rsrec_assemble_blocks: hoh needs nbr_type, obarm (ntype=%d) and blocks_o", ntype);
    if (hoh)
        for (size_t q = 0; q < (size_t)ncls * nslots; ++q)
            if (nbr_type[q] < 0 || nbr_type[q] > ntype) return fail(h, RSREC_ERR_ARG, "rsrec_assemble_blocks: nbr_type[%zu]=%d outside 0..%d", q, nbr_type[q], ntype);
    HIPCK(h, hipSetDevice(h->device));
    h->n_asm_calls++;
    h->asm_nslots[part] = h->asm_ncls[part] = 0;
    const size_t nblk = (size_t)ncls * nslots, hm_bytes = nblk * 4 * 81 * 16, ty_bytes = nblk * 4, ob_bytes = hoh ? (size_t)ntype * 324 * 16 : 0;
    const size_t ty_off = (hm_bytes + 255) / 256 * 256, ob_off = ty_off + (ty_bytes + 255) / 256 * 256;
    HIPCK(h, h->d_asm_in.reserve(ob_off + ob_bytes + 256));
    char* in = h->d_asm_in.as<char>();
    XFER(xfer_h2d(h, in, hmag, hm_bytes));
    if (hoh) { XFER(xfer_h2d(h, in + ty_off, nbr_type, ty_bytes)); XFER(xfer_h2d(h, in + ob_off, obarm, ob_bytes)); }
    HIPCK(h, h->d_asm[part][0].reserve(nblk * 324 * 16));
    if (hoh) HIPCK(h, h->d_asm[part][1].reserve(nblk * 324 * 16));
    k_assemble_blocks<<<dim3(nslots, ncls), 384, 0, h->stream>>>(reinterpret_cast<const double2*>(in), reinterpret_cast<const int*>(in + ty_off),
                                                                 reinterpret_cast<const double2*>(in + ob_off), nslots, hoh ? 1 : 0, h->d_asm[part][0].as<double2>(),
                                                                 hoh ? h->d_asm[part][1].as<double2>() : nullptr);
    HIPCK(h, hipGetLastError());
    XFER(xfer_d2h(h, blocks, h->d_asm[part][0].p, nblk * 324 * 16));
    if (hoh) XFER(xfer_d2h(h, blocks_o, h->d_asm[part][1].p, nblk * 324 * 16));
    h->asm_host[part][0].assign(blocks, blocks + nblk * 648);
    if (hoh) h->asm_host[part][1].assign(blocks_o, blocks_o + nblk * 648); else h->asm_host[part][1].clear();
    h->asm_nslots[part] = nslots; h->asm_ncls[part] = ncls; h->asm_hoh[part] = hoh ? 1 : 0;
    return RSREC_OK;
}

namespace {

DevProblem make_problem(const rsrec_t* h) {
    DevProblem P;
    P.kk = h->kk; P.nslots = h->nslots; P.hstride = h->hslots; P.nmax = h->nmax; P.hoh = h->hoh;
    P.nbr = h->d_nbr.as<int>(); P.iz = h->d_iz.as<int>();
    P.h_st = h->d_hst.as<double2>(); P.h_loc = h->d_hloc.as<double2>();
    P.ho_st = h->d_host.as<double2>(); P.ho_loc = h->d_holoc.as<double2>();
    P.enim = h->d_enim.as<double2>(); P.lsham = h->d_lsham.as<double2>();
    return P;
}

void release_kubo_buffers(rsrec_t* h, bool moments, bool integrand) {
    if (moments) { for (auto& kb : h->d_kubo) kb.release(); h->kubo_diag_nvec = h->kubo_diag_ll = 0; }
    if (integrand) { for (auto& cb : h->d_cond) cb.release(); for (auto& cb : h->d_ctens) cb.release(); }
}

struct BatchPlan {
    int batch = 1, nblk = 1;
};

int plan_batch(rsrec_t* h, int nchains, int nvec, size_t vec_elems_per_chain, BatchPlan& bp) {
    release_kubo_buffers(h, true, true);
    size_t free_b = 0, total_b = 0;
    HIPCK(h, hipMemGetInfo(&free_b, &total_b));
    size_t reusable = 0;
    for (int v = 0; v < 5; ++v) reusable += h->d_vec[v].bytes;
    const double per_chain = (double)nvec * vec_elems_per_chain * sizeof(double2) + (double)h->kk * 4 + 4096;
    long cap = (long)((0.85 * (double)(free_b + reusable)) / per_chain);
    if (cap < 1) return fail(h, RSREC_ERR_DEVICE, "not enough device memory for one chain (%.1f MB needed, %.1f MB free)", per_chain / 1e6, free_b / 1e6);
    long b = h->opt_batch > 0 ? h->opt_batch : 64;
    b = std::min<long>(b, cap);
    b = std::min<long>(b, nchains);
    bp.batch = (int)std::max<long>(b, 1);
    long nblk = h->opt_nblk > 0 ? h->opt_nblk : std::max<long>(2048 / bp.batch, 16);
    nblk = std::min<long>(nblk, 256);
    nblk = std::min<long>(nblk, (h->kk + TILE_ATOMS - 1) / TILE_ATOMS);
    bp.nblk = (int)std::max<long>(nblk, 1);
    return RSREC_OK;
}

int upload_regions(rsrec_t* h, const int* seeds0, int nb, int nseed, int nlev, int napply, bool two_pass, bool grouped, int& ostride,
                   double& atom_steps, double& block_mults) {
    const int kk = h->kk;
    const int cap = grouped ? kk + 7 * h->nmax + 7 * h->ntype + 8 : kk;
    const int cap_pre = ((grouped ? kk + 7 * h->nmax + 7 * h->ntype * nlev + 8 : kk) + GROUP - 1) / GROUP * GROUP;
    const int flags = (two_pass ? 1 : 0) | (grouped ? 2 : 0) | ((int)std::min<long>(100, std::max<long>(1, h->opt_sat_pct)) << 2) | (nseed << 9);
    for (const auto& e : h->region_cache)
        if (e->epoch == h->lattice_epoch && e->nlev == nlev && e->napply == napply && e->flags == flags && (int)e->seeds.size() == nb * nseed &&
            std::equal(e->seeds.begin(), e->seeds.end(), seeds0)) {
            h->cur_order = e->order.as<int>(); h->cur_cum = e->cum.as<int>(); h->cur_nrows = nb; h->cur_level_max = &e->level_max; h->cur_level_groups = &e->level_groups;
            h->cur_mult_hist = &e->mult_hist;
            h->cur_entry = e.get();
            ostride = e->ostride;
            atom_steps += e->atom_steps; block_mults += e->block_mults;
            return RSREC_OK;
        }
    const int ntau_h = h->nmax + h->ntype, nfs_h = h->nslots + 1;
    const int sat_pct = (int)std::min<long>(100, std::max<long>(1, h->opt_sat_pct));
    const int sat_from = (int)(((long)sat_pct * kk + 99) / 100);
    std::vector<Region> regs(nb);
    auto run_threads = [&](auto&& fn) {
        const int nthr = std::max(1, std::min({nb, 8, (int)std::thread::hardware_concurrency()}));
        if (nthr == 1) { for (int c = 0; c < nb; ++c) fn(c); return; }
        std::atomic<int> next_chain{0};
        std::vector<std::thread> pool;
        for (int t = 0; t < nthr; ++t)
            pool.emplace_back([&]() { for (int c = next_chain++; c < nb; c = next_chain++) fn(c); });
        for (auto& th : pool) th.join();
    };
    run_threads([&](int c) { grow_region(h, seeds0 + (size_t)c * nseed, nseed, nlev, regs[c]); });
    size_t lvneed = 8;
    for (int c = 0; c < nb; ++c) {
        size_t need = 0;
        for (int L = 0; L < nlev; ++L) {
            const int n = regs[c].cum[L];
            if (n >= sat_from || (L > 0 && n == regs[c].cum[L - 1])) continue;
            need += (size_t)n + (grouped ? (size_t)7 * std::min(ntau_h, n) + 8 : 0);
        }
        lvneed = std::max(lvneed, need);
    }
    lvneed = (lvneed + 7) / 8 * 8;
    if (lvneed + (size_t)cap > (size_t)INT32_MAX) return fail(h, RSREC_ERR_ARG, "region lists of %zu entries per chain exceed the index range", lvneed + (size_t)cap);
    if ((size_t)cap_pre + lvneed + (size_t)cap > (size_t)INT32_MAX) return fail(h, RSREC_ERR_ARG, "region lists of %zu entries per chain exceed the index range", (size_t)cap_pre + lvneed + (size_t)cap);
    const int sat_off = cap_pre + (int)lvneed;
    ostride = sat_off + cap;
    std::vector<int> order((size_t)nb * ostride, -1), cum((size_t)4 * nb * nlev, 0);
    std::vector<double> as(nb, 0.0), bm(nb, 0.0);
    const size_t hist_n = (size_t)2 * ntau_h * nfs_h;
    std::vector<double> hist((size_t)nb * hist_n, 0.0);
    auto tau = [&](int i) { return i < h->nmax ? i : h->nmax + h->iz0[i]; };
    const std::vector<unsigned>& key = h->spatial_key;
    auto before = [&](int x, int y) {
        const int tx = grouped ? tau(x) : 0, ty = grouped ? tau(y) : 0;
        if (tx != ty) return tx < ty;
        if (key[x] != key[y]) return key[x] < key[y];
        return x < y;
    };
    std::vector<int> all(kk), sat_list;
    for (int i = 0; i < kk; ++i) all[i] = i;
    std::sort(all.begin(), all.end(), before);
    sat_list.reserve(cap);
    for (int q = 0; q < kk; ++q) {
        if (grouped && q > 0 && tau(all[q]) != tau(all[q - 1])) while (sat_list.size() % GROUP) sat_list.push_back(-1);
        sat_list.push_back(all[q]);
    }
    if (grouped) while (sat_list.size() % GROUP) sat_list.push_back(-1);
    const int sat_count = (int)sat_list.size();
    std::vector<double> lgroups((size_t)nb * nlev * ntau_h, 0.0);
    auto build_chain = [&](int c) {
        const Region& R = regs[c];
        int* orow = order.data() + (size_t)c * ostride;
        int* crow = cum.data() + (size_t)c * nlev;
        int* brow = cum.data() + (size_t)(nb + c) * nlev;
        int* crow2 = cum.data() + (size_t)(2 * nb + c) * nlev;
        int* brow2 = cum.data() + (size_t)(3 * nb + c) * nlev;
        std::copy(sat_list.begin(), sat_list.end(), orow + sat_off);
        int w = cap_pre, wp = 0;
        std::vector<int> lev, region, merged;
        for (int L = 0; L < nlev; ++L) {
            const int lo = L ? R.cum[L - 1] : 0, hi = R.cum[L];
            if (hi >= sat_from) { crow[L] = crow2[L] = sat_count; brow[L] = brow2[L] = sat_off; continue; }
            lev.assign(R.order.begin() + lo, R.order.begin() + hi);
            std::sort(lev.begin(), lev.end(), before);
            for (size_t q = 0; q < lev.size(); ++q) {
                if (grouped && q > 0 && tau(lev[q]) != tau(lev[q - 1])) while (wp % GROUP) orow[wp++] = -1;
                orow[wp++] = lev[q];
            }
            if (grouped) while (wp % GROUP) orow[wp++] = -1;
            crow2[L] = wp; brow2[L] = 0;
            if (L > 0 && hi == lo) { crow[L] = crow[L - 1]; brow[L] = brow[L - 1]; continue; }
            merged.resize(region.size() + lev.size());
            std::merge(region.begin(), region.end(), lev.begin(), lev.end(), merged.begin(), before);
            region.swap(merged);
            brow[L] = w;
            double* G = lgroups.data() + ((size_t)c * nlev + L) * ntau_h;
            for (size_t q = 0; q < region.size(); ++q) {
                if (grouped && q > 0 && tau(region[q]) != tau(region[q - 1])) while (w % GROUP) orow[w++] = -1;
                if (w % GROUP == 0) G[grouped ? tau(region[q]) : 0] += 1.0;
                orow[w++] = region[q];
            }
            if (grouped) while (w % GROUP) orow[w++] = -1;
            crow[L] = w - brow[L];
        }
        double a_s = 0.0, b_m = 0.0;
        for (int t = 1; t <= napply; ++t) {
            const int lv_after = two_pass ? 2 * t : t;
            a_s += R.cum[std::min(lv_after, nlev - 1)];
        }
        std::vector<int> lev_of(kk, -1);
        {
            int lv = 0;
            for (int q = 0; q < R.cum[nlev - 1]; ++q) {
                while (q >= R.cum[lv]) ++lv;
                lev_of[R.order[q]] = lv;
            }
        }
        std::vector<double> uses1(nlev + 1, 0.0), uses2(nlev + 1, 0.0);
        for (int d = 0; d < nlev; ++d)
            for (int t = 1; t <= napply; ++t) {
                if (!two_pass) { if (d <= t - 1) uses1[d] += 1.0; }
                else { if (d <= 2 * (t - 1)) uses1[d] += 1.0; if (d <= 2 * t - 1) uses2[d] += 1.0; }
            }
        double* H = hist.data() + (size_t)c * hist_n;
        const int ns = h->nslots;
        for (int i = 0; i < kk; ++i) {
            const int ti = tau(i);
            for (int s = 0; s < ns; ++s) {
                const int n = h->nbr[(size_t)i * ns + s];
                if (n < 0 || lev_of[n] < 0) continue;
                H[(size_t)ti * nfs_h + s] += uses1[lev_of[n]];
                if (two_pass) H[((size_t)ntau_h + ti) * nfs_h + s] += uses2[lev_of[n]];
            }
            if (two_pass && lev_of[i] >= 0) H[((size_t)ntau_h + ti) * nfs_h + ns] += uses1[lev_of[i]];
        }
        for (size_t q = 0; q < hist_n; ++q) b_m += H[q];
        if (two_pass) for (int t2 = 0; t2 < ntau_h; ++t2) b_m += H[((size_t)ntau_h + t2) * nfs_h + ns];
        as[c] = a_s; bm[c] = b_m;
    };
    run_threads(build_chain);
    double as_sum = 0.0, bm_sum = 0.0;
    for (int c = 0; c < nb; ++c) { as_sum += as[c]; bm_sum += bm[c]; }
    atom_steps += as_sum; block_mults += bm_sum;
    if (h->region_cache.size() >= 256) {
        HIPCK(h, hipStreamSynchronize(h->stream));
        h->region_cache.clear();
        h->cur_entry = nullptr;
    }
    h->region_cache.push_back(std::make_unique<rsrec_handle::RegionEntry>());
    rsrec_handle::RegionEntry* e = h->region_cache.back().get();
    e->seeds.assign(seeds0, seeds0 + (size_t)nb * nseed);
    e->nlev = nlev; e->napply = napply; e->flags = flags; e->epoch = h->lattice_epoch; e->ostride = ostride;
    e->atom_steps = as_sum; e->block_mults = bm_sum;
    e->mult_hist.assign(hist_n, 0.0);
    for (int c = 0; c < nb; ++c)
        for (size_t q = 0; q < hist_n; ++q) e->mult_hist[q] += hist[(size_t)c * hist_n + q];
    HIPCK(h, e->order.reserve(order.size() * 4));
    HIPCK(h, e->cum.reserve(cum.size() * 4));
    XFER(xfer_h2d(h, e->order.p, order.data(), order.size() * 4));
    XFER(xfer_h2d(h, e->cum.p, cum.data(), cum.size() * 4));
    HIPCK(h, hipStreamSynchronize(h->stream));
    e->level_max.assign(nlev, 0);
    e->level_groups.assign((size_t)nlev * ntau_h, 0.0);
    {
        std::vector<double> sat_hist(ntau_h, 0.0);
        for (int g = 0; g < sat_count / GROUP; ++g) sat_hist[tau(sat_list[(size_t)g * GROUP])] += 1.0;
        e->sat_base = sat_off;
        e->level_sat.assign(nlev, 0);
        if (grouped)
            for (int g = 0; g < sat_count / GROUP; ++g) {
                const int t = tau(sat_list[(size_t)g * GROUP]);
                if (e->sat_runs.empty() || e->sat_runs.back().tau != t) e->sat_runs.push_back({t, g, g + 1});
                else e->sat_runs.back().hi = g + 1;
            }
        for (int c = 0; c < nb; ++c) {
            const double* prev = nullptr;
            for (int l = 0; l < nlev; ++l) {
                const int cnt = cum[(size_t)c * nlev + l];
                e->level_max[l] = std::max(e->level_max[l], cnt);
                const bool sat = cum[(size_t)(nb + c) * nlev + l] == sat_off;
                e->level_max[l] = std::max(e->level_max[l], cum[(size_t)(2 * nb + c) * nlev + l]);
                if (sat) e->level_sat[l] += 1;
                const double* G = lgroups.data() + ((size_t)c * nlev + l) * ntau_h;
                if (!sat && l > 0 && cum[(size_t)(nb + c) * nlev + l] == cum[(size_t)(nb + c) * nlev + l - 1] && prev) G = prev;
                for (int t2 = 0; t2 < ntau_h; ++t2) e->level_groups[(size_t)l * ntau_h + t2] += sat ? sat_hist[t2] : G[t2];
                prev = sat ? nullptr : G;
            }
        }
    }
    h->cur_order = e->order.as<int>(); h->cur_cum = e->cum.as<int>(); h->cur_nrows = nb; h->cur_level_max = &e->level_max; h->cur_level_groups = &e->level_groups;
    h->cur_mult_hist = &e->mult_hist;
    h->cur_entry = e;
    return RSREC_OK;
}

double required_hop_flops(const rsrec_t* h, const Spmm5Operator& op) {
    if (!h->cur_mult_hist) return 0.0;
    const int ntau = h->nmax + h->ntype, nfs = h->nslots + 1;
    const std::vector<double>& H = *h->cur_mult_hist;
    if (H.size() != (size_t)2 * ntau * nfs) return 0.0;
    double f = 0.0;
    for (int pass = 0; pass < 2; ++pass)
        for (int t = 0; t < ntau; ++t)
            for (int s = 0; s < nfs; ++s) {
                const double n = H[((size_t)pass * ntau + t) * nfs + s];
                if (n == 0.0) continue;
                const double w = (op.mixing.empty() || op.ntau != ntau || op.nslots != h->nslots) ? 46656.0 : op.required_flops(pass, t, s);
                f += n * (w > 0.0 ? w : 46656.0);
            }
    return f;
}

void reset_timing(rsrec_t* h) {
    h->t_total_ms = h->t_hop_ms = h->t_rest_ms = h->t_host_ms = h->t_rot_ms = 0;
    h->n_hop_launch = h->n_atom_steps = h->n_block_mult = h->n_hop_mfma_flop = h->n_req_flop = 0;
    h->n_octet_launch = 0;
    h->ev_used = 0;
    h->n_recursion_calls++;
}

double ev_ms(hipEvent_t a, hipEvent_t b) {
    float ms = 0.f;
    if (!a || !b || hipEventElapsedTime(&ms, a, b) != hipSuccess) return 0.0;
    return ms;
}

int check_ready(rsrec_t* h, const char* who) {
    if (!h) return RSREC_ERR_ARG;
    if (!h->have_lattice || !h->have_ham) return fail(h, RSREC_ERR_ARG, "%s: lattice and hamiltonian must be set first", who);
    return RSREC_OK;
}

int check_seeds(rsrec_t* h, const char* who, const int32_t* atoms, size_t n, int lo) {
    for (size_t q = 0; q < n; ++q)
        if (atoms[q] < lo || atoms[q] > h->kk) return fail(h, RSREC_ERR_ARG, "%s: seed atom %d outside %d..%d", who, atoms[q], lo, h->kk);
    return RSREC_OK;
}

void stage_seeds(const int32_t* seed_atoms, const double* seed_coef, int c0, int nb, int nseed, std::vector<int>& seeds0, std::vector<double>& coef) {
    const size_t n = (size_t)nb * nseed, g0 = (size_t)c0 * nseed;
    seeds0.resize(n);
    coef.resize(2 * n);
    for (size_t q = 0; q < n; ++q) {
        seeds0[q] = seed_atoms[g0 + q] - 1;
        coef[2 * q] = seed_coef ? seed_coef[2 * (g0 + q)] : 1.0;
        coef[2 * q + 1] = seed_coef ? seed_coef[2 * (g0 + q) + 1] : 0.0;
    }
}

int ensure_side_stream(rsrec_t* h) {
    if (h->side_stream) return RSREC_OK;
    HIPCK(h, hipStreamCreateWithFlags(&h->side_stream, hipStreamNonBlocking));
    HIPCK(h, hipEventCreateWithFlags(&h->ev_orth, hipEventDisableTiming));
    HIPCK(h, hipEventCreateWithFlags(&h->ev_bred, hipEventDisableTiming));
    return RSREC_OK;
}

int reserve_partials(rsrec_t* h, int B, size_t first_stage_bytes) {
    HIPCK(h, h->d_partial.reserve(first_stage_bytes));
    h->p2_slot = (size_t)B * 16 * 2 * 1296;
    HIPCK(h, h->d_partial2.reserve(2 * h->p2_slot * sizeof(double)));
    return RSREC_OK;
}

void chain_views(const rsrec_t* h, int nlev, size_t velems, int cpo, int ostride, ChainView& CV, ChainView* CVp = nullptr) {
    const size_t tab = (size_t)h->cur_nrows * nlev;
    CV.order = h->cur_order; CV.cum = h->cur_cum; CV.obase = h->cur_cum + tab; CV.nlev = nlev; CV.vstride = velems; CV.cpo = cpo; CV.ostride = ostride;
    if (!CVp) return;
    *CVp = CV;
    CVp->cum = h->cur_cum + 2 * tab; CVp->obase = h->cur_cum + 3 * tab;
}

void finish_timing(rsrec_t* h, hipEvent_t ev_begin, hipEvent_t ev_end, const std::vector<std::pair<hipEvent_t, hipEvent_t>>& hop_ev) {
    h->t_total_ms = ev_ms(ev_begin, ev_end);
    for (auto& pr : hop_ev) h->t_hop_ms += ev_ms(pr.first, pr.second);
    h->t_rest_ms = h->t_total_ms - h->t_hop_ms;
}

int finish_status(rsrec_t* h) {
    int status = 0;
    XFER(xfer_d2h(h, &status, h->d_status.p, 4));
    HIPCK(h, hipStreamSynchronize(h->stream));
    if (status & 1) return fail(h, RSREC_ERR_EIG, "Diagonalization error (18x18 Jacobi did not converge)");
    if (status & 2) return fail(h, RSREC_ERR_DIVERGED, "Chebyshev moments did not converge. Check energy limits energy_min and energy_max");
    return RSREC_OK;
}

int mfma_workgroups_per_chain(const rsrec_t* h, int batch) {
    if (h->opt_nblk > 0) return (int)std::min<long>(2 * h->opt_nblk, 256);
    return batch >= 32 ? 8 : (batch >= 16 ? 32 : 256);
}

dim3 level_grid(const rsrec_t* h, dim3 full, int level) {
    if (!h->cur_level_max || level < 0 || level >= (int)h->cur_level_max->size()) return full;
    const int groups = (*h->cur_level_max)[level] / GROUP;
    return dim3(std::max(1, std::min((int)full.x, (groups + MF_WAVES - 1) / MF_WAVES)), full.y);
}

dim3 s5_grid(const rsrec_t* h, dim3 full, int level) {
    int gx = full.x;
    if (h->cur_level_max && level >= 0 && level < (int)h->cur_level_max->size()) {
        const int groups = (*h->cur_level_max)[level] / GROUP;
        gx = std::max(1, (groups + S5_WG_GROUPS - 1) / S5_WG_GROUPS);
        if (gx > 8) gx = (gx + 7) / 8 * 8;
        if (h->opt_s5_cap > 0) gx = std::min(gx, (int)h->opt_s5_cap);
    }
    const int fold = (int)std::max<long>(1, h->opt_chain_fold);
    return dim3(gx, (full.y + fold - 1) / fold);
}

const double* presum(rsrec_t* h, const double* partial, int nb, int& nblk, int width, hipStream_t stream = nullptr, int slot = 0) {
    if (nblk <= 32) return partial;
    const int nblk2 = (nblk + 15) / 16;
    const size_t need = (size_t)nb * nblk2 * width;
    if (slot == 0 && h->p2_slot == 0) {
        if (h->d_partial2.reserve(need * sizeof(double)) != hipSuccess) return partial;
    } else if (need > h->p2_slot) return partial;
    double* out = h->d_partial2.as<double>() + (size_t)slot * h->p2_slot;
    const int nchunk = (width + 255) / 256;
    k_presum16<<<dim3(nblk2 * nchunk, nb), 256, 0, stream ? stream : h->stream>>>(partial, nblk, nblk2, width, out);
    nblk = nblk2;
    return out;
}

constexpr size_t S5_LDS_LIMIT = 160 * 1024;
void s5_prepare(rsrec_t* h) {
    if (h->s5_lds_limit != (size_t)-1) return;
    int optin = 0;
    h->s5_lds_limit = 0;
    if (hipDeviceGetAttribute(&optin, hipDeviceAttributeSharedMemPerBlockOptin, h->device) == hipSuccess && optin > 64 * 1024) {
        const int ask = (int)std::min<size_t>((size_t)optin, S5_LDS_LIMIT);
        if (hipFuncSetAttribute(reinterpret_cast<const void*>(k_spmm5<false, true>), hipFuncAttributeMaxDynamicSharedMemorySize, ask) == hipSuccess &&
            hipFuncSetAttribute(reinterpret_cast<const void*>(k_spmm5<true, true>), hipFuncAttributeMaxDynamicSharedMemorySize, ask) == hipSuccess &&
            hipFuncSetAttribute(reinterpret_cast<const void*>(k_spmm5<false, true, false, 3>), hipFuncAttributeMaxDynamicSharedMemorySize, ask) == hipSuccess &&
            hipFuncSetAttribute(reinterpret_cast<const void*>(k_spmm5<true, true, false, 3>), hipFuncAttributeMaxDynamicSharedMemorySize, ask) == hipSuccess)
            h->s5_lds_limit = (size_t)ask;
    }
    (void)hipGetLastError();
}
template <bool TWO>
void launch_s5_one(rsrec_t* h, dim3 grid, const SpmmDims& SD, const int* order, const int* cum, const int* iz, const Spmm5Operator& op, int set,
                   const double* in, double* out, const double* in2, const double* extra, int ntau, S5Epilogue epi, int one) {
    const size_t lds_bytes = (size_t)op.ntr * S5_TRIPLE * sizeof(double);
    const bool want = h->opt_s5_lds >= 1;
    s5_prepare(h);
    const size_t lds_limit = h->s5_lds_limit;
    if (want && one >= 0 && !extra && lds_bytes <= lds_limit) {
        const int spin_by_xcd = (op.spin_mixing || !h->opt_s5_spin_xcd) ? 0 : 1;
        const unsigned row = spin_by_xcd ? 8 : 16;
        dim3 g2(std::max(row, (grid.x + row - 1) / row * row), grid.y);
        int* queue = nullptr;
        const unsigned ncu = (unsigned)std::max(16, h->n_cu / 16 * 16);
        if ((h->opt_s5_queue == 1 && grid.x >= ncu) || h->opt_s5_queue >= 2) {
            if ((!h->capturing || h->d_s5queue.bytes >= (size_t)SD.nchains * 16 * sizeof(int)) &&
                h->d_s5queue.reserve((size_t)SD.nchains * 16 * sizeof(int)) == hipSuccess &&
                hipMemsetAsync(h->d_s5queue.p, 0, (size_t)SD.nchains * 16 * sizeof(int), h->stream) == hipSuccess) {
                queue = h->d_s5queue.as<int>();
                g2 = dim3(ncu, 1);
            }
        }
        const unsigned thr = (queue && h->opt_s5_waves == 4) ? S5_WG_GROUPS * 64 : S5_WG_GROUPS * 128;
        if (queue && h->opt_s5_split == 3) {
            const unsigned thr3 = 64u * (unsigned)std::min<long>(12, std::max<long>(8, h->opt_s5_waves));
            const size_t lds3 = std::min(lds_limit, lds_bytes + (size_t)S5_TRIPLE_BYTES);
            k_spmm5<TWO, true, false, 3><<<g2, thr3, lds3, h->stream>>>(SD, order, cum, h->d_nbr5.as<int>(), iz, op.frag_set(set), op.meta_set(set), op.ntr, in, out, in2, nullptr, ntau, one, queue, spin_by_xcd, epi);
        } else
        k_spmm5<TWO, true><<<g2, thr, lds_bytes, h->stream>>>(SD, order, cum, h->d_nbr5.as<int>(), iz, op.frag_set(set), op.meta_set(set), op.ntr, in, out, in2, nullptr, ntau, one, queue, spin_by_xcd, epi);
    } else
        k_spmm5<TWO, false><<<grid, S5_WG_GROUPS * 128, 0, h->stream>>>(SD, order, cum, h->d_nbr5.as<int>(), iz, op.frag_set(set), op.meta_set(set), op.ntr, in, out, in2, extra, ntau, 0, nullptr, 1, epi);
}

template <bool TWO>
void launch_s5(rsrec_t* h, dim3 grid, const SpmmDims& SD0, const int* order, const int* cum, const int* iz, const Spmm5Operator& op, int set,
               const double* in, double* out, const double* in2 = nullptr, const double* extra = nullptr, int ntau = 0, S5Epilogue epi = S5Epilogue()) {
    SpmmDims SD = SD0;
    const int one = op.single_class(set);
    const rsrec_handle::RegionEntry* E = h->cur_entry;
    const bool multi = one < 0 && h->opt_s5_lds >= 2 && !extra && E && E->sat_base > 0 && SD.cpo == 1 && SD.level >= 0 && SD.level < (int)E->level_sat.size() &&
                       E->level_sat[SD.level] > 0 && op.ntau == h->nmax + h->ntype && (grid.x >= (unsigned)std::max(16, h->n_cu / 16 * 16) || h->opt_s5_queue >= 2) && (size_t)op.ntr * S5_TRIPLE * sizeof(double) <= (s5_prepare(h), h->s5_lds_limit);
    bool octets = false, oct_aside = false;
    double pa_pairs = 0.0;
    if (h->cur_level_groups && SD.level >= 0 && (size_t)(SD.level + 1) * op.ntau <= h->cur_level_groups->size() && op.ntau == h->nmax + h->ntype)
        for (int t = 0; t < h->nmax; ++t) pa_pairs += (*h->cur_level_groups)[(size_t)SD.level * op.ntau + t];
    if (!multi && one < 0 && h->opt_s5_octet > 0 && h->nmax >= h->opt_s5_octet && !extra && E && SD.cpo == 1 && SD.nchains >= 2 && op.ntau == h->nmax + h->ntype &&
        2.0 * pa_pairs >= (double)h->nmax * SD.nchains && (double)GROUP * (double)(h->kk + 1) * BLD * 8.0 < 4294967296.0) {
        SpmmDims SO = SD;
        const dim3 go((unsigned)((h->nmax + S5_WG_GROUPS - 1) / S5_WG_GROUPS), (unsigned)((SD.nchains + GROUP - 1) / GROUP));
        hipStream_t so = h->stream;
        if (h->opt_side && !h->oct_stream && !h->capturing &&
            (hipStreamCreateWithFlags(&h->oct_stream, hipStreamNonBlocking) != hipSuccess || hipEventCreateWithFlags(&h->ev_oct_in, hipEventDisableTiming) != hipSuccess ||
             hipEventCreateWithFlags(&h->ev_oct_out, hipEventDisableTiming) != hipSuccess)) { h->oct_stream = nullptr; (void)hipGetLastError(); }
        if (h->opt_side && h->oct_stream && h->ev_oct_in && h->ev_oct_out && hipEventRecord(h->ev_oct_in, h->stream) == hipSuccess &&
            hipStreamWaitEvent(h->oct_stream, h->ev_oct_in, 0) == hipSuccess) { so = h->oct_stream; oct_aside = true; }
        k_spmm5<TWO, false, true><<<go, S5_WG_GROUPS * 128, 0, so>>>(SO, order, cum, h->d_nbr5.as<int>(), iz, op.frag_set(set), op.meta_set(set), op.ntr, in, out, in2, nullptr, ntau,
                                                                   0, nullptr, 1, epi);
        if (oct_aside) (void)hipEventRecord(h->ev_oct_out, h->oct_stream);
        const bool all_sat = E->sat_base > 0 && SD.level < (int)E->level_sat.size() && E->level_sat[SD.level] == SD.nchains && (int)E->sat_runs.size() >= h->nmax &&
                             E->sat_runs[0].tau == 0 && E->sat_runs[0].lo == 0 && E->sat_runs[h->nmax - 1].tau == h->nmax - 1 && E->sat_runs[h->nmax - 1].hi == h->nmax;
        if (all_sat) {
            SD.sat_base = E->sat_base; SD.run_lo = h->nmax; SD.run_hi = E->sat_runs.back().hi;
        } else SD.skip_pa = 1;
        octets = true;
        h->n_octet_launch++;
    }
    if (!multi) {
        launch_s5_one<TWO>(h, grid, SD, order, cum, iz, op, set, in, out, in2, extra, ntau, epi, one);
        if (oct_aside) (void)hipStreamWaitEvent(h->stream, h->ev_oct_out, 0);
    } else {
        SD.sat_base = E->sat_base;
        const long min_groups = h->opt_s5_run_min > 0 ? h->opt_s5_run_min : std::max<long>(64, 2L * h->n_cu * 8 / std::max(1, E->level_sat[SD.level]));
        const int spin_by_xcd = op.spin_mixing ? 0 : 1;
        const int row = spin_by_xcd ? 8 : 16;
        const int ncu = std::max(16, h->n_cu / 16 * 16), total_rows = ncu / row;
        SpmmDims SR = SD;
        long sum_groups = 0;
        for (const auto& R : E->sat_runs) {
            if (SR.nruns == 4 || R.hi - R.lo < min_groups || op.ksteps[(size_t)set * op.ntau + R.tau] == 0) continue;
            SR.run_tau[SR.nruns] = R.tau; SR.run_glo[SR.nruns] = R.lo; SR.run_ghi[SR.nruns] = R.hi; ++SR.nruns;
            sum_groups += R.hi - R.lo;
        }
        const size_t qbytes = (size_t)4 * SD.nchains * 16 * sizeof(int);
        const bool can = SR.nruns > 0 && SR.nruns <= total_rows && (h->opt_s5_queue >= 1) && (!h->capturing || h->d_s5queue.bytes >= qbytes) &&
                         h->d_s5queue.reserve(qbytes) == hipSuccess && hipMemsetAsync(h->d_s5queue.p, 0, qbytes, h->stream) == hipSuccess;
        if (can) {
            int left = total_rows - SR.nruns, acc = 0;
            for (int r = 0; r < SR.nruns; ++r) {
                const long gr = SR.run_ghi[r] - SR.run_glo[r];
                int extra_rows = r == SR.nruns - 1 ? left : (int)std::min<long>(left, (gr * (total_rows - SR.nruns) + sum_groups / 2) / std::max(1L, sum_groups));
                left -= extra_rows;
                SR.run_row0[r] = acc;
                acc += 1 + extra_rows;
            }
            SR.run_row0[SR.nruns] = acc;
            const size_t lds_bytes = (size_t)op.ntr * S5_TRIPLE * sizeof(double);
            k_spmm5<TWO, true><<<dim3(ncu, 1), S5_WG_GROUPS * 128, lds_bytes, h->stream>>>(SR, order, cum, h->d_nbr5.as<int>(), iz, op.frag_set(set), op.meta_set(set), op.ntr, in, out, in2, nullptr, ntau,
                                                                                          0, h->d_s5queue.as<int>(), spin_by_xcd, epi);
            for (int r = 0; r < SR.nruns; ++r) { SD.skip_lo[r] = SR.run_glo[r]; SD.skip_hi[r] = SR.run_ghi[r]; }
            SD.nskip = SR.nruns;
        }
        launch_s5_one<TWO>(h, grid, SD, order, cum, iz, op, set, in, out, in2, nullptr, ntau, epi, -1);
    }
    if (h->cur_level_groups && SD.level >= 0 && (size_t)(SD.level + 1) * op.ntau <= h->cur_level_groups->size() && SD.cpo == 1 && op.ntau == h->nmax + h->ntype)
        for (int t = 0; t < op.ntau; ++t) {
            double groups = (*h->cur_level_groups)[(size_t)SD.level * op.ntau + t];
            if (octets && t < h->nmax) groups = (double)((SD.nchains + GROUP - 1) / GROUP);
            h->n_hop_mfma_flop += groups * op.flops_per_group(set, t);
        }
}

bool spmm4_usable(const rsrec_t* h) { return h->s5_built && !h->hoh && (size_t)(h->kk + 1) * BLD * sizeof(double) < ((size_t)1 << 32); }

int ensure_s4(rsrec_t* h) {
    if (h->s4_built_split) return RSREC_OK;
    const char* msg = h->s4_op.build(h->nslots, h->hslots, h->ntype, h->nmax, 0, h->host_st.data(), h->nmax > 0 ? h->host_loc.data() : nullptr, nullptr, nullptr, 1);
    if (msg) return fail(h, RSREC_ERR_DEVICE, "k_spmm4 operator tables: %s", msg);
    h->s4_built_split = 1;
    return RSREC_OK;
}

int s4_prepare(rsrec_t* h) {
    if (!h->s4_attr) {
        HIPCK(h, hipFuncSetAttribute(reinterpret_cast<const void*>(k_spmm4<4>), hipFuncAttributeMaxDynamicSharedMemorySize, (int)S4_LDS_BYTES));
        h->s4_attr = true;
    }
    return RSREC_OK;
}
int launch_spmm(rsrec_t* h, const SpmmDims& SD, const ChainView& CV, const DevProblem& P, int set, const double* in, double* out, dim3 grid_mf) {
    { const int rc = s4_prepare(h); if (rc) return rc; }
    dim3 g4(std::min<unsigned>(grid_mf.x * 4, 1024), grid_mf.y);
    k_spmm4<4><<<g4, MF_WAVES * 64, S4_LDS_BYTES, h->stream>>>(SD, CV.order, CV.cum, P.nbr, P.iz, h->s4_op.frag_set(set), h->s4_op.meta_set(set), in, out);
    return RSREC_OK;
}

__global__ __launch_bounds__(256) void k_rotate_coef(double2* __restrict__ A, double2* __restrict__ B, const double2* __restrict__ rot, int lld) {
#pragma clang fp contract(off)
    __shared__ double2 sM[BLK], sR[BLK], sT[BLK];
    const int chain = blockIdx.y, m = blockIdx.x;
    const bool is_a = m < lld - 1;
    double2* M = (is_a ? A : B) + ((size_t)chain * lld + (is_a ? m : m - (lld - 1) + 1)) * BLK;
    const double2* R = rot + (size_t)chain * BLK;
    for (int e = threadIdx.x; e < BLK; e += blockDim.x) { sM[e] = M[e]; sR[e] = R[e]; }
    __syncthreads();
    for (int e = threadIdx.x; e < BLK; e += blockDim.x) {
        const int i = e % NB, j = e / NB;
        double sr = 0.0, si = 0.0;
#pragma unroll
        for (int k = 0; k < NB; ++k) {
            const double ar = sM[i + NB * k].x, ai = sM[i + NB * k].y, br = sR[k + NB * j].x, bi = sR[k + NB * j].y;
            sr += ar * br - ai * bi; si += ar * bi + ai * br;
        }
        sT[e] = make_double2(sr, si);
    }
    __syncthreads();
    for (int e = threadIdx.x; e < BLK; e += blockDim.x) {
        const int i = e % NB, j = e / NB;
        double sr = 0.0, si = 0.0;
#pragma unroll
        for (int k = 0; k < NB; ++k) {
            const double ar = sR[k + NB * i].x, ai = -sR[k + NB * i].y, br = sT[k + NB * j].x, bi = sT[k + NB * j].y;
            sr += ar * br - ai * bi; si += ar * bi + ai * br;
        }
        M[e] = make_double2(sr, si);
    }
}

struct RecursionCall {
    bool mfma = false, side = false;
    int nchains = 0, nseed = 1, napply = 0, nlev = 0;
    const double* rot = nullptr;
    const Spmm5Operator* op = nullptr;
    int ci = 0;
    size_t velems = 0;
    int nvec = 0, skip_vec = -1, B = 1, nblk = 1;
    DevProblem P;
    hipEvent_t ev_begin = nullptr;
    std::vector<std::pair<hipEvent_t, hipEvent_t>> hop_ev, rot_ev;
};

RecursionCall recursion_call(const rsrec_t* h, bool mfma, int nchains, int nseed, int napply, const double* rot = nullptr) {
    RecursionCall RC;
    RC.mfma = mfma; RC.nchains = nchains; RC.nseed = nseed; RC.napply = napply; RC.rot = rot;
    RC.nlev = (h->hoh ? 2 * napply : napply) + 1; RC.op = rot ? &h->s5_la : &h->s5_op; RC.velems = (size_t)(h->kk + 1) * BLD;
    const bool large = (long)std::min(nchains, 64) * (h->kk / GROUP + 1) >= 4096;
    RC.ci = (mfma && (h->hoh || rot || h->opt_spmm5 == 2 || (h->opt_spmm5 == 1 && large) || !spmm4_usable(h))) ? 1 : 0;
    return RC;
}

int recursion_begin(rsrec_t* h, RecursionCall& RC, int nvec, int skip_vec, int coef_slots) {
    if (RC.mfma && !RC.ci) XFER(ensure_s4(h));
    RC.nvec = nvec; RC.skip_vec = skip_vec;
    BatchPlan bp;
    XFER(plan_batch(h, RC.nchains, nvec - (skip_vec >= 0 ? 1 : 0), RC.velems / 2, bp));
    const int B = RC.B = bp.batch; RC.nblk = bp.nblk;
    for (int v = 0; v < nvec; ++v) if (v != skip_vec) HIPCK(h, h->d_vec[v].reserve((size_t)B * RC.velems * sizeof(double)));
    XFER(reserve_partials(h, B, (size_t)B * 256 * 2 * 1296 * sizeof(double)));
    XFER(ensure_side_stream(h));
    RC.side = h->opt_side && h->side_stream;
    if (RC.rot) HIPCK(h, h->d_la_extra.reserve((size_t)B * (h->nmax + h->ntype) * S5_HEAD_DOUBLES * sizeof(double)));
    HIPCK(h, h->d_status.reserve(64));
    HIPCK(h, h->d_seed.reserve((size_t)B * RC.nseed * 4));
    HIPCK(h, h->d_seedcoef.reserve((size_t)B * coef_slots * sizeof(double2)));
    HIPCK(h, hipMemsetAsync(h->d_status.p, 0, 64, h->stream));
    RC.P = make_problem(h); RC.ev_begin = next_event(h);
    return RSREC_OK;
}

void local_axis_fragments(const rsrec_t* h, const Spmm5Operator& OP, const double* rot, int c0, int nb, std::vector<double>& fr) {
    const bool hoh = h->hoh != 0;
    const int ntau = h->nmax + h->ntype, la_fps = S5_HEAD_DOUBLES;
    std::vector<double> E(2 * BLK), T(2 * BLK); fr.assign((size_t)nb * ntau * la_fps, 0.0);
    for (int c = 0; c < nb; ++c) {
        const double* R = rot + 2 * (size_t)BLK * (c0 + c);
        for (int tau = 0; tau < ntau; ++tau) {
            const int ty = tau < h->nmax ? h->iz0[tau] : tau - h->nmax;
            const double* ls = h->host_lsham.data() + 2 * (size_t)BLK * ty;
            for (int j = 0; j < NB; ++j)
                for (int i = 0; i < NB; ++i) {
                    double sr = 0.0, si = 0.0;
                    for (int k = 0; k < NB; ++k) {
                        const double ar = ls[2 * (i + NB * k)], ai = ls[2 * (i + NB * k) + 1], br = R[2 * (j + NB * k)], bi = -R[2 * (j + NB * k) + 1];
                        sr += ar * br - ai * bi; si += ar * bi + ai * br;
                    }
                    T[2 * (i + NB * j)] = sr; T[2 * (i + NB * j) + 1] = si;
                }
            for (int j = 0; j < NB; ++j)
                for (int i = 0; i < NB; ++i) {
                    double sr = 0.0, si = 0.0;
                    for (int k = 0; k < NB; ++k) {
                        const double ar = R[2 * (i + NB * k)], ai = R[2 * (i + NB * k) + 1], br = T[2 * (k + NB * j)], bi = T[2 * (k + NB * j) + 1];
                        sr += ar * br - ai * bi; si += ar * bi + ai * br;
                    }
                    E[2 * (i + NB * j)] = sr; E[2 * (i + NB * j) + 1] = si;
                }
            if (hoh) for (int e = 0; e < 2 * BLK; ++e) E[e] += h->host_enim[2 * (size_t)BLK * ty + e];
            OP.emit_head(hoh ? 1 : 0, tau, E.data(), fr.data() + ((size_t)c * ntau + tau) * la_fps);
        }
    }
}

struct RecursionBatch {
    int nb = 0, ostride = 0;
    ChainView CV, CVp;
    dim3 grid_mf;
    const double* la_extra = nullptr;
};
using SeedCoefHook = void (*)(int nb, int nseed, const std::vector<int>& seeds0, std::vector<double>& coef);
int recursion_batch(rsrec_t* h, const RecursionCall& RC, const int32_t* seed_atoms, const double* seed_coef, int c0, int nb, RecursionBatch& b,
                    SeedCoefHook extra_coef = nullptr) {
    const auto th0 = std::chrono::steady_clock::now();
    std::vector<int> seeds0;
    std::vector<double> coef, fr;
    stage_seeds(seed_atoms, seed_coef, c0, nb, RC.nseed, seeds0, coef);
    if (extra_coef) extra_coef(nb, RC.nseed, seeds0, coef);
    b.nb = nb; b.ostride = h->kk;
    XFER(upload_regions(h, seeds0.data(), nb, RC.nseed, RC.nlev, RC.napply, h->hoh != 0, RC.mfma, b.ostride, h->n_atom_steps, h->n_block_mult));
    h->n_req_flop += required_hop_flops(h, *RC.op);
    XFER(xfer_h2d(h, h->d_seed.p, seeds0.data(), seeds0.size() * 4));
    XFER(xfer_h2d(h, h->d_seedcoef.p, coef.data(), coef.size() * 8));
    if (RC.rot) {
        local_axis_fragments(h, *RC.op, RC.rot, c0, nb, fr);
        XFER(xfer_h2d(h, h->d_la_extra.p, fr.data(), fr.size() * sizeof(double)));
        b.la_extra = h->d_la_extra.as<double>();
    }
    HIPCK(h, hipStreamSynchronize(h->stream));
    h->t_host_ms += std::chrono::duration<double, std::milli>(std::chrono::steady_clock::now() - th0).count();
    chain_views(h, RC.nlev, RC.velems, 1, b.ostride, b.CV, &b.CVp);
    b.grid_mf = dim3(std::max(1, std::min(mfma_workgroups_per_chain(h, RC.B), (b.ostride / GROUP + MF_WAVES - 1) / MF_WAVES)), nb);
    return RSREC_OK;
}

int clear_vectors(rsrec_t* h, const RecursionCall& RC, int nb, int zero_block_only = -1) {
    for (int v = 0; v < RC.nvec; ++v) {
        if (v == RC.skip_vec) continue;
        if (v == zero_block_only)
            HIPCK(h, hipMemset2DAsync(static_cast<char*>(h->d_vec[v].p) + (size_t)h->kk * BLD * sizeof(double), RC.velems * sizeof(double), 0, BLD * sizeof(double), (size_t)nb, h->stream));
        else HIPCK(h, hipMemsetAsync(h->d_vec[v].p, 0, (size_t)nb * RC.velems * sizeof(double), h->stream));
    }
    return RSREC_OK;
}
int apply_h(rsrec_t* h, RecursionCall& RC, const RecursionBatch& b, int step, const double* src, double* dst, double* hps, const double* extra, int ntau,
            S5Epilogue epi = S5Epilogue()) {
    const bool hoh = h->hoh != 0;
    const int lv_final = hoh ? 2 * step : step;
    const Spmm5Operator& OP = *RC.op; const DevProblem& P = RC.P; const ChainView& CV = b.CV;
    hipEvent_t e0 = next_event(h);
    SpmmDims SD{h->kk, P.nslots, P.nmax, RC.nlev, 1, b.ostride, hoh ? 2 * step - 1 : lv_final, RC.velems, CV.obase, b.nb};
    if (!RC.ci) XFER(launch_spmm(h, SD, CV, P, 0, src, dst, b.grid_mf));
    else if (hoh) {
        launch_s5<false>(h, s5_grid(h, b.grid_mf, 2 * step - 1), SD, CV.order, CV.cum, P.iz, OP, 0, src, hps);
        SD.level = lv_final;
        launch_s5<true>(h, s5_grid(h, b.grid_mf, lv_final), SD, CV.order, CV.cum, P.iz, OP, 1, hps, dst, src, extra, ntau, epi);
    } else if (extra) launch_s5<true>(h, s5_grid(h, b.grid_mf, lv_final), SD, CV.order, CV.cum, P.iz, OP, 0, src, dst, src, extra, ntau, epi);
    else launch_s5<false>(h, s5_grid(h, b.grid_mf, lv_final), SD, CV.order, CV.cum, P.iz, OP, 0, src, dst, nullptr, nullptr, 0, epi);
    RC.hop_ev.emplace_back(e0, next_event(h)); h->n_hop_launch += hoh ? 2 : 1;
    return RSREC_OK;
}

S5Epilogue cheb_epilogue(bool first, const double* cur, const double* old, double a, double b) {
    S5Epilogue E; E.kind = first ? 1 : 2; E.cur = cur; E.old = first ? nullptr : old; E.a = a; E.b = b;
    return E;
}
struct SideReduce { bool side = false, pending = false; };
int side_reduce_begin(rsrec_t* h, const SideReduce& S, hipStream_t& st) {
    st = S.side ? h->side_stream : h->stream;
    if (S.side) { HIPCK(h, hipEventRecord(h->ev_orth, h->stream)); HIPCK(h, hipStreamWaitEvent(h->side_stream, h->ev_orth, 0)); }
    return RSREC_OK;
}
int side_reduce_end(rsrec_t* h, SideReduce& S) { if (S.side) { HIPCK(h, hipEventRecord(h->ev_bred, h->side_stream)); S.pending = true; } return RSREC_OK; }
int side_reduce_wait(rsrec_t* h, SideReduce& S) { if (S.pending) { HIPCK(h, hipStreamWaitEvent(h->stream, h->ev_bred, 0)); S.pending = false; } return RSREC_OK; }

template <class Enqueue>
int replay_level_loop(rsrec_t* h, const std::vector<uintptr_t>& key, Enqueue&& enqueue) {
    if (!h->graph_exec || key != h->graph_key) {
        if (h->graph_exec) { (void)hipGraphExecDestroy(h->graph_exec); h->graph_exec = nullptr; }
        h->graph_key.clear();
        s5_prepare(h);
        XFER(s4_prepare(h));
        HIPCK(h, hipStreamSynchronize(h->stream));
        HIPCK(h, hipStreamBeginCapture(h->stream, hipStreamCaptureModeRelaxed));
        h->capturing = true;
        const int rc = enqueue();
        h->capturing = false;
        hipGraph_t graph = nullptr;
        const hipError_t ec = hipStreamEndCapture(h->stream, &graph);
        if (rc) { if (graph) (void)hipGraphDestroy(graph); return rc; }
        if (ec != hipSuccess || !graph) return fail(h, RSREC_ERR_DEVICE, "hipStreamEndCapture failed: %s", hipGetErrorString(ec));
        const hipError_t ei = hipGraphInstantiate(&h->graph_exec, graph, nullptr, nullptr, 0);
        (void)hipGraphDestroy(graph);
        if (ei != hipSuccess) { h->graph_exec = nullptr; return fail(h, RSREC_ERR_DEVICE, "hipGraphInstantiate failed: %s", hipGetErrorString(ei)); }
        h->graph_key = key;
    }
    HIPCK(h, hipGraphLaunch(h->graph_exec, h->stream));
    return RSREC_OK;
}

int rotate_resident_coef(rsrec_t* h, RecursionCall& RC, double2* dA, double2* dB, int c0, int nb, int lld) {
    hipEvent_t r0 = next_event(h);
    k_rotate_coef<<<dim3(2 * (lld - 1), nb), 256, 0, h->stream>>>(dA, dB, h->d_rot.as<double2>() + (size_t)c0 * BLK, lld);
    HIPCK(h, hipGetLastError());
    RC.rot_ev.emplace_back(r0, next_event(h));
    return RSREC_OK;
}
int recursion_end(rsrec_t* h, const RecursionCall& RC, int res_kind, int lld, bool seeded) {
    hipEvent_t ev_end = next_event(h);
    const int rc = finish_status(h);
    finish_timing(h, RC.ev_begin, ev_end, RC.hop_ev);
    for (auto& pr : RC.rot_ev) h->t_rot_ms += ev_ms(pr.first, pr.second);
    if (rc) return rc;
    h->res_kind = res_kind; h->res_n = RC.nchains; h->res_lld = lld; h->res_seeded = seeded;
    return RSREC_OK;
}

template <class L, bool MFMA>
int run_block_lanczos(rsrec_t* h, int nchains, int nseed, const int32_t* seed_atoms, const double* seed_coef, int lld, double* a_b, double* b2_b,
                      const double* rot = nullptr ) {
    const int kk = h->kk;
    const bool hoh = h->hoh != 0;
    const int nsteps = lld - 1;
    if (rot && !MFMA) return fail(h, RSREC_ERR_ARG, "local-axis recursion needs the matrix-core kernel set (option kernels = 0 or 2)");
    RecursionCall RC = recursion_call(h, MFMA, nchains, nseed, nsteps, rot);
    const int ci = RC.ci, ntau = h->nmax + h->ntype;
    const size_t velems = RC.velems, cstride = (size_t)lld * BLK, orth_lds = TILE_ATOMS * BLK * sizeof(double2);
    h->res_kind = 0;
    HIPCK(h, h->d_coefA.reserve((size_t)nchains * lld * BLK * sizeof(double2)));
    HIPCK(h, h->d_coefB.reserve((size_t)nchains * lld * BLK * sizeof(double2)));
    if (rot) {
        HIPCK(h, h->d_rot.reserve((size_t)nchains * BLK * sizeof(double2)));
        XFER(xfer_h2d(h, h->d_rot.p, rot, (size_t)nchains * BLK * sizeof(double2)));
    }
    const bool oop = MFMA && h->opt_orth_oop != 0 && h->opt_orth3 != 2;
    const int nvec = MFMA ? (oop && hoh ? 5 : 4) : (hoh ? 3 : 2);
    const bool use_v1 = !MFMA || hoh || oop;
    XFER(recursion_begin(h, RC, nvec, use_v1 ? -1 : 1, nseed));
    const int B = RC.B, nblk = RC.nblk;
    HIPCK(h, h->d_frags.reserve((size_t)B * 3 * 27 * 64 * sizeof(double)));
    HIPCK(h, h->d_bmats.reserve((size_t)B * 2 * BLK * sizeof(double2)));
    const size_t gram_elems = (size_t)B * 256 * 1296;
    double *pmn = h->d_vec[1].as<double>(), *hpsi = h->d_vec[2].as<double>();
    double2* partial = h->d_partial.as<double2>();
    double *gpartial = h->d_partial.as<double>(), *bfrags = h->d_frags.as<double>();
    HIPCK(h, hipFuncSetAttribute(reinterpret_cast<const void*>(k_orth<L>), hipFuncAttributeMaxDynamicSharedMemorySize, TILE_ATOMS * BLK * (int)sizeof(double2)));
    h->hop_fuses_a = MFMA ? 0 : 1;

    for (int c0 = 0; c0 < nchains; c0 += B) {
        const int nb = std::min(B, nchains - c0);
        double2* dA = h->d_coefA.as<double2>() + (size_t)c0 * cstride;
        double2* dB = h->d_coefB.as<double2>() + (size_t)c0 * cstride;
        RecursionBatch bt;
        XFER(recursion_batch(h, RC, seed_atoms, seed_coef, c0, nb, bt));
        const ChainView &CV = bt.CV, &CVp = bt.CVp;
        auto enqueue_levels = [&]() -> int {
            XFER(clear_vectors(h, RC, nb, MFMA && !hoh ? 2 : -1));
            HIPCK(h, hipMemsetAsync(dA, 0, (size_t)nb * cstride * sizeof(double2), h->stream));
            HIPCK(h, hipMemsetAsync(dB, 0, (size_t)nb * cstride * sizeof(double2), h->stream));
            if (MFMA) HIPCK(h, hipMemsetAsync(bfrags, 0, (size_t)nb * 3 * 27 * 64 * sizeof(double), h->stream));
            double *psi = h->d_vec[0].as<double>(), *t2 = h->d_vec[3].as<double>();
            double* t3 = oop ? h->d_vec[hoh ? 4 : 1].as<double>() : nullptr;
            if (ci) k_seed<LayoutCI><<<nb, 64, 0, h->stream>>>(psi, velems, h->d_seed.as<int>(), h->d_seedcoef.as<double2>(), nseed);
            else k_seed<L><<<nb, 64, 0, h->stream>>>(psi, velems, h->d_seed.as<int>(), h->d_seedcoef.as<double2>(), nseed);
            k_set_identity<<<nb, 256, 0, h->stream>>>(dB, cstride);
            if (MFMA) k_uscheme_init<<<nb, 256, 0, h->stream>>>(h->d_bmats.as<double2>(), bfrags, ci);
            const dim3 grid(nblk, nb);
            SideReduce SR{RC.side};
            double* gp_b = SR.side ? gpartial + gram_elems : gpartial;
            for (int ll = 0; ll < nsteps; ++ll) {
                const int lv_final = hoh ? 2 * ll + 2 : ll + 1;
                if (MFMA) {
                    XFER(apply_h(h, RC, bt, ll + 1, psi, hpsi, pmn, bt.la_extra, ntau));
                    const dim3 gl = level_grid(h, bt.grid_mf, lv_final);
                    k_mfma_adot<<<gl, MF_WAVES * 64, 0, h->stream>>>(CVp, lv_final, kk, psi, hpsi, gpartial);
                    int n2 = gl.x; const double* p2 = presum(h, gpartial, nb, n2, 1296);
                    XFER(side_reduce_wait(h, SR));
                    k_reduce_a_u<<<nb, 1024, 0, h->stream>>>(p2, n2, dA + (size_t)ll * BLK, cstride, h->d_bmats.as<double2>(), bfrags, ci);
                    if (h->opt_orth3 == 2) k_mfma_orth3w<<<gl, MF_WAVES * 64, 0, h->stream>>>(CVp, lv_final, kk, hpsi, psi, t2, bfrags, gp_b);
                    else k_mfma_orth3<<<gl, MF_WAVES * 64, 0, h->stream>>>(CVp, lv_final, kk, hpsi, psi, t2, bfrags, gp_b, t3);
                    hipStream_t st; XFER(side_reduce_begin(h, SR, st));
                    n2 = gl.x; p2 = presum(h, gp_b, nb, n2, 1296, st, SR.side ? 1 : 0);
                    k_reduce_b_u<<<nb, 1024, 0, st>>>(p2, n2, dB + (size_t)(ll + 1) * BLK, cstride, h->d_bmats.as<double2>(), bfrags, h->d_status.as<int>(), ci);
                    XFER(side_reduce_end(h, SR));
                    if (oop) { double* f = t2; t2 = psi; psi = t3; t3 = f; }
                    else std::swap(psi, t2);
                    continue;
                }
                hipEvent_t e0 = next_event(h);
                ApplyArgs G{}; G.partial = partial;
                if (!hoh) {
                    G.in = psi; G.v0 = psi; G.out = pmn; G.level = lv_final;
                    k_apply<AM_LANCZOS, L><<<grid, NTHREADS, 0, h->stream>>>(RC.P, CV, G);
                } else {
                    G.in = psi; G.out = hpsi; G.level = 2 * ll + 1;
                    k_apply<AM_STORE, L><<<grid, NTHREADS, 0, h->stream>>>(RC.P, CV, G);
                    G.in = hpsi; G.v1 = hpsi; G.cur = psi; G.v0 = psi; G.out = pmn; G.level = lv_final;
                    k_apply<AM_HOH_LANCZOS, L><<<grid, NTHREADS, 0, h->stream>>>(RC.P, CV, G);
                }
                RC.hop_ev.emplace_back(e0, next_event(h)); h->n_hop_launch += hoh ? 2 : 1;
                k_reduce_a<<<nb, 1024, 0, h->stream>>>(partial, nblk, dA + (size_t)ll * BLK, cstride);
                k_orth<L><<<grid, NTHREADS, orth_lds, h->stream>>>(CV, lv_final, psi, pmn, (const double*)nullptr, dA + (size_t)ll * BLK, cstride, partial);
                k_reduce_b_eig<<<nb, 1024, 0, h->stream>>>(partial, nblk, dB + (size_t)(ll + 1) * BLK, cstride, h->d_bmats.as<double2>(), h->d_status.as<int>());
                k_update<L><<<grid, NTHREADS, 0, h->stream>>>(CV, lv_final, psi, pmn, h->d_bmats.as<double2>());
            }
            HIPCK(h, hipGetLastError());
            return side_reduce_wait(h, SR);
        };
        const bool use_graph = MFMA && nchains <= B && ((h->opt_graph == 1 && nchains <= 8) || h->opt_graph >= 2) && getenv("RSREC_NO_GRAPH") == nullptr;
        if (!use_graph) XFER(enqueue_levels());
        else {
            if (ci) HIPCK(h, h->d_s5queue.reserve((size_t)nb * 16 * sizeof(int)));
            const Spmm5Operator& OP = *RC.op;
            std::vector<uintptr_t> key = {(uintptr_t)1 , (uintptr_t)nb, (uintptr_t)lld, (uintptr_t)nseed, (uintptr_t)hoh, (uintptr_t)ci, (uintptr_t)(rot != nullptr), (uintptr_t)kk,
                                          (uintptr_t)h->cur_order, (uintptr_t)h->cur_cum, (uintptr_t)bt.ostride, (uintptr_t)OP.d_frag, (uintptr_t)OP.d_meta, (uintptr_t)OP.ntr,
                                          (uintptr_t)h->s4_op.frag_set(0), (uintptr_t)h->s4_op.meta_set(0), (uintptr_t)h->d_nbr.p, (uintptr_t)h->d_nbr5.p, (uintptr_t)h->d_iz.p,
                                          (uintptr_t)h->d_partial.p, (uintptr_t)h->d_partial2.p, (uintptr_t)h->d_frags.p, (uintptr_t)dA, (uintptr_t)dB, (uintptr_t)h->d_bmats.p,
                                          (uintptr_t)h->d_status.p, (uintptr_t)h->d_seed.p, (uintptr_t)h->d_seedcoef.p, (uintptr_t)h->d_la_extra.p, (uintptr_t)h->d_s5queue.p,
                                          (uintptr_t)h->cur_entry, (uintptr_t)h->p2_slot, (uintptr_t)OP.single_class(0), (uintptr_t)OP.spin_mixing,
                                          (uintptr_t)h->lattice_epoch, (uintptr_t)OP.sched_epoch, (uintptr_t)h->nslots, (uintptr_t)h->nmax, (uintptr_t)h->ntype, (uintptr_t)h->hslots,
                                          (uintptr_t)B, (uintptr_t)h->n_cu};
            for (int v = 0; v < nvec; ++v) key.push_back((uintptr_t)h->d_vec[v].p);
            for (const OptionEntry& o : OPTIONS)
                if (o.member != &rsrec_handle::opt_graph) key.push_back((uintptr_t)(h->*o.member));
            XFER(replay_level_loop(h, key, enqueue_levels));
            h->n_hop_launch += (double)nsteps * (hoh ? 2 : 1);
        }
        if (rot && lld > 1) XFER(rotate_resident_coef(h, RC, dA, dB, c0, nb, lld));
        XFER(xfer_d2h(h, a_b + (size_t)c0 * cstride * 2, dA, (size_t)nb * cstride * sizeof(double2)));
        XFER(xfer_d2h(h, b2_b + (size_t)c0 * cstride * 2, dB, (size_t)nb * cstride * sizeof(double2)));
        HIPCK(h, hipStreamSynchronize(h->stream));
    }
    return recursion_end(h, RC, 1, lld, seed_coef != nullptr);
}

}

extern "C" int rsrec_block_lanczos_seeded(rsrec_t* h, int nchains, int nseed, const int32_t* seed_atoms, const double* seed_coef, int lld,
                                          double* a_b, double* b2_b) {
    int rc = check_ready(h, "rsrec_block_lanczos");
    if (rc) return rc;
    if (nchains < 0 || nseed < 1 || lld < 1 || !a_b || !b2_b || (nchains > 0 && !seed_atoms)) return fail(h, RSREC_ERR_ARG, "rsrec_block_lanczos: bad argument");
    XFER(check_seeds(h, "rsrec_block_lanczos", seed_atoms, (size_t)nchains * nseed, 1));
    HIPCK(h, hipSetDevice(h->device));
    reset_timing(h);
    if (nchains == 0) return RSREC_OK;
    const bool use_mfma = (h->opt_kernels != 1) && h->s5_built;
    if (use_mfma) return run_block_lanczos<LayoutRM, true>(h, nchains, nseed, seed_atoms, seed_coef, lld, a_b, b2_b);
    return run_block_lanczos<LayoutCM, false>(h, nchains, nseed, seed_atoms, seed_coef, lld, a_b, b2_b);
}

extern "C" int rsrec_block_lanczos(rsrec_t* h, int nsites, const int32_t* seed_atoms, int lld, double* a_b, double* b2_b) {
    return rsrec_block_lanczos_seeded(h, nsites, 1, seed_atoms, nullptr, lld, a_b, b2_b);
}

namespace {

int build_local_axis_operator(rsrec_t* h) {
    if (h->s5_la_ok) return RSREC_OK;
    const int ntau = h->nmax + h->ntype, nfs = h->nslots + 1, nset = h->hoh ? 2 : 1;
    const size_t B = 2 * (size_t)BLK;
    std::vector<const double*> blk((size_t)nset * ntau * nfs, nullptr);
    std::vector<double> dense(B, 1.0), neg((size_t)ntau * h->nslots * B, 0.0);
    for (int tau = 0; tau < ntau; ++tau) {
        for (int s = 0; s < h->nslots; ++s) {
            const double* src = tau < h->nmax ? h->host_hall.data() + B * (s + (size_t)h->hslots * tau) : h->host_ee.data() + B * (s + (size_t)h->hslots * (tau - h->nmax));
            blk[((size_t)0 * ntau + tau) * nfs + s] = src;
            if (nset > 1) {
                const double* so = tau < h->nmax ? h->host_hallo.data() + B * (s + (size_t)h->hslots * tau) : h->host_eeo.data() + B * (s + (size_t)h->hslots * (tau - h->nmax));
                double* d = neg.data() + B * (s + (size_t)h->nslots * tau);
                for (size_t e = 0; e < B; ++e) d[e] = -so[e];
                if (s == 0) for (int q = 0; q < NB; ++q) d[2 * (q + NB * q)] += 1.0;
                blk[((size_t)1 * ntau + tau) * nfs + s] = d;
            }
        }
        blk[((size_t)(nset - 1) * ntau + tau) * nfs + h->nslots] = dense.data();
    }
    const char* msg = h->s5_la.build_custom(h->nslots, ntau, nset, blk);
    if (msg) return fail(h, RSREC_ERR_DEVICE, "rsrec_block_lanczos_local_axis: %s", msg);
    h->s5_la_ok = 1;
    return RSREC_OK;
}

}

extern "C" int rsrec_block_lanczos_local_axis(rsrec_t* h, int nsites, const int32_t* seed_atoms, const double* rot, int lld, double* a_b, double* b2_b) {
    int rc = check_ready(h, "rsrec_block_lanczos_local_axis");
    if (rc) return rc;
    if (nsites < 0 || lld < 1 || !a_b || !b2_b || (nsites > 0 && (!seed_atoms || !rot))) return fail(h, RSREC_ERR_ARG, "rsrec_block_lanczos_local_axis: bad argument");
    XFER(check_seeds(h, "rsrec_block_lanczos_local_axis", seed_atoms, (size_t)nsites, 1));
    if (!h->s5_built) return fail(h, RSREC_ERR_ARG, "rsrec_block_lanczos_local_axis: lattice has too many neighbour slots for the SpMM kernel");
    HIPCK(h, hipSetDevice(h->device));
    reset_timing(h);
    if (nsites == 0) return RSREC_OK;
    rc = build_local_axis_operator(h); if (rc) return rc;
    return run_block_lanczos<LayoutRM, true>(h, nsites, 1, seed_atoms, nullptr, lld, a_b, b2_b, rot);
}

namespace {

bool is_device_ptr(const void* p) {
    hipPointerAttribute_t at;
    if (hipPointerGetAttributes(&at, p) == hipSuccess) return at.type == hipMemoryTypeDevice;
    (void)hipGetLastError();
    hsa_amd_pointer_info_t info;
    memset(&info, 0, sizeof info);
    info.size = sizeof info;
    if (hsa_amd_pointer_info(const_cast<void*>(p), &info, nullptr, nullptr, nullptr) != HSA_STATUS_SUCCESS) return false;
    if (info.type != HSA_EXT_POINTER_TYPE_HSA) return false;
    hsa_device_type_t dt = HSA_DEVICE_TYPE_CPU;
    if (hsa_agent_get_info(info.agentOwner, HSA_AGENT_INFO_DEVICE, &dt) != HSA_STATUS_SUCCESS) return false;
    return dt == HSA_DEVICE_TYPE_GPU;
}

__global__ void k_pack_diag(const double2* __restrict__ A, const double2* __restrict__ B, int lld, int n, int off, int ntot,
                            double* __restrict__ a_img, double* __restrict__ b_img) {
    const size_t total = (size_t)lld * NB * ntot;
    for (size_t e = (size_t)blockIdx.x * blockDim.x + threadIdx.x; e < total; e += (size_t)gridDim.x * blockDim.x) {
        const int ll = (int)(e % lld), l = (int)((e / lld) % NB), s = (int)(e / ((size_t)lld * NB)) - off;
        double a = 0.0, b = 0.0;
        if (s >= 0 && s < n) {
            const size_t q = ((size_t)s * lld + ll) * BLK + (size_t)l * (NB + 1);
            a = A[q].x; b = B[q].x;
        }
        a_img[e] = a; b_img[e] = b;
    }
}

}

extern "C" int rsrec_pack_diag(rsrec_t* h, int site_offset, int nsites_total, double* a_img, double* b2_img) {
    if (!h || !a_img || !b2_img || site_offset < 0) return fail(h, RSREC_ERR_ARG, "rsrec_pack_diag: bad argument");
    if (h->res_kind != 1) return fail(h, RSREC_ERR_ARG, "rsrec_pack_diag: no block-Lanczos coefficients resident (call rsrec_block_lanczos first)");
    if (site_offset + h->res_n > nsites_total) return fail(h, RSREC_ERR_ARG, "rsrec_pack_diag: sites %d..%d outside 1..%d", site_offset + 1, site_offset + h->res_n, nsites_total);
    HIPCK(h, hipSetDevice(h->device));
    const size_t n = (size_t)h->res_lld * NB * nsites_total;
    const bool dev = is_device_ptr(a_img) && is_device_ptr(b2_img);
    double *da = a_img, *db = b2_img;
    if (!dev) { HIPCK(h, h->d_scal.reserve(2 * n * sizeof(double))); da = h->d_scal.as<double>(); db = da + n; }
    const int blocks = (int)std::min<size_t>(1024, (n + 255) / 256);
    k_pack_diag<<<blocks, 256, 0, h->stream>>>(h->d_coefA.as<double2>(), h->d_coefB.as<double2>(), h->res_lld, h->res_n, site_offset, nsites_total, da, db);
    HIPCK(h, hipGetLastError());
    if (!dev) { XFER(xfer_d2h(h, a_img, da, n * sizeof(double))); XFER(xfer_d2h(h, b2_img, db, n * sizeof(double))); }
    HIPCK(h, hipStreamSynchronize(h->stream));
    return RSREC_OK;
}

namespace {

__global__ void k_pack_moments(const double2* __restrict__ mu, size_t per_site, int n, int off, int ntot, double2* __restrict__ img) {
    const size_t total = per_site * (size_t)ntot;
    for (size_t e = (size_t)blockIdx.x * blockDim.x + threadIdx.x; e < total; e += (size_t)gridDim.x * blockDim.x) {
        const int s = (int)(e / per_site) - off;
        img[e] = (s >= 0 && s < n) ? mu[(size_t)s * per_site + e % per_site] : make_double2(0.0, 0.0);
    }
}

}

extern "C" int rsrec_pack_moments(rsrec_t* h, int site_offset, int nsites_total, double* mu_img) {
    if (!h || !mu_img || site_offset < 0) return fail(h, RSREC_ERR_ARG, "rsrec_pack_moments: bad argument");
    if (h->res_kind != 2) return fail(h, RSREC_ERR_ARG, "rsrec_pack_moments: no Chebyshev moments resident (call rsrec_chebyshev first)");
    if (site_offset + h->res_n > nsites_total) return fail(h, RSREC_ERR_ARG, "rsrec_pack_moments: sites %d..%d outside 1..%d", site_offset + 1, site_offset + h->res_n, nsites_total);
    HIPCK(h, hipSetDevice(h->device));
    const size_t per_site = (size_t)(2 * h->res_lld + 2) * BLK, n = per_site * nsites_total;
    const bool dev = is_device_ptr(mu_img);
    double2* out = reinterpret_cast<double2*>(mu_img);
    if (!dev) { HIPCK(h, h->d_scal.reserve(n * sizeof(double2))); out = h->d_scal.as<double2>(); }
    k_pack_moments<<<(int)std::min<size_t>(2048, (n + 255) / 256), 256, 0, h->stream>>>(h->d_mu.as<double2>(), per_site, h->res_n, site_offset, nsites_total, out);
    HIPCK(h, hipGetLastError());
    if (!dev) XFER(xfer_d2h(h, mu_img, out, n * sizeof(double2)));
    HIPCK(h, hipStreamSynchronize(h->stream));
    return RSREC_OK;
}

namespace {

struct NcclId { char internal[RSREC_COMM_ID_BYTES]; };
struct RcclApi {
    void* lib = nullptr;
    int (*get_unique_id)(NcclId*) = nullptr;
    int (*comm_init_rank)(void**, int, NcclId, int) = nullptr;
    int (*all_reduce)(const void*, void*, size_t, int, int, void*, hipStream_t) = nullptr;
    int (*comm_destroy)(void*) = nullptr;
    const char* (*get_error_string)(int) = nullptr;
};
RcclApi g_rccl;

const char* rccl_ready() {
    if (g_rccl.lib) return nullptr;
    void* lib = dlopen("librccl.so", RTLD_NOW | RTLD_LOCAL);
    if (!lib) lib = dlopen("librccl.so.1", RTLD_NOW | RTLD_LOCAL);
    if (!lib) lib = dlopen("/opt/rocm/lib/librccl.so", RTLD_NOW | RTLD_LOCAL);
    if (!lib) return "RCCL (librccl.so) not found";
    g_rccl.get_unique_id = reinterpret_cast<decltype(g_rccl.get_unique_id)>(dlsym(lib, "ncclGetUniqueId"));
    g_rccl.comm_init_rank = reinterpret_cast<decltype(g_rccl.comm_init_rank)>(dlsym(lib, "ncclCommInitRank"));
    g_rccl.all_reduce = reinterpret_cast<decltype(g_rccl.all_reduce)>(dlsym(lib, "ncclAllReduce"));
    g_rccl.comm_destroy = reinterpret_cast<decltype(g_rccl.comm_destroy)>(dlsym(lib, "ncclCommDestroy"));
    g_rccl.get_error_string = reinterpret_cast<decltype(g_rccl.get_error_string)>(dlsym(lib, "ncclGetErrorString"));
    if (!g_rccl.get_unique_id || !g_rccl.comm_init_rank || !g_rccl.all_reduce || !g_rccl.comm_destroy) return "RCCL symbols missing";
    g_rccl.lib = lib;
    return nullptr;
}
const char* rccl_err(int rc) { return g_rccl.get_error_string ? g_rccl.get_error_string(rc) : "RCCL error"; }

}

extern "C" int rsrec_comm_unique_id(char* id) {
    if (!id) return RSREC_ERR_ARG;
    if (rccl_ready()) return RSREC_ERR_DEVICE;
    NcclId u;
    if (g_rccl.get_unique_id(&u) != 0) return RSREC_ERR_DEVICE;
    memcpy(id, u.internal, RSREC_COMM_ID_BYTES);
    return RSREC_OK;
}

extern "C" int rsrec_comm_destroy(rsrec_t* h) {
    if (!h) return RSREC_ERR_ARG;
    if (h->comm) {
        (void)hipSetDevice(h->device);
        (void)hipStreamSynchronize(h->stream);
        (void)g_rccl.comm_destroy(h->comm);
        h->comm = nullptr;
    }
    h->comm_rank = 0; h->comm_nranks = 1;
    return RSREC_OK;
}

extern "C" int rsrec_comm_init(rsrec_t* h, int rank, int nranks, const char* id) {
    if (!h || !id || nranks < 1 || rank < 0 || rank >= nranks) return fail(h, RSREC_ERR_ARG, "rsrec_comm_init: bad argument");
    if (const char* msg = rccl_ready()) return fail(h, RSREC_ERR_DEVICE, "rsrec_comm_init: %s", msg);
    (void)rsrec_comm_destroy(h);
    HIPCK(h, hipSetDevice(h->device));
    NcclId u;
    memcpy(u.internal, id, RSREC_COMM_ID_BYTES);
    const int rc = g_rccl.comm_init_rank(&h->comm, nranks, u, rank);
    if (rc != 0) { h->comm = nullptr; return fail(h, RSREC_ERR_DEVICE, "ncclCommInitRank failed: %s", rccl_err(rc)); }
    h->comm_rank = rank; h->comm_nranks = nranks;
    return RSREC_OK;
}

extern "C" int rsrec_comm_init_file(rsrec_t* h, int rank, int nranks, const char* path, double timeout_s) {
    if (!h || !path || nranks < 1 || rank < 0 || rank >= nranks) return fail(h, RSREC_ERR_ARG, "rsrec_comm_init_file: bad argument");
    char id[RSREC_COMM_ID_BYTES];
    if (rank == 0) {
        if (rsrec_comm_unique_id(id) != RSREC_OK) return fail(h, RSREC_ERR_DEVICE, "rsrec_comm_init_file: ncclGetUniqueId failed");
        const std::string tmp = std::string(path) + ".tmp";
        FILE* f = fopen(tmp.c_str(), "wb");
        if (!f || fwrite(id, 1, sizeof id, f) != sizeof id) { if (f) fclose(f); return fail(h, RSREC_ERR_ARG, "rsrec_comm_init_file: cannot write %s", tmp.c_str()); }
        fclose(f);
        if (rename(tmp.c_str(), path) != 0) return fail(h, RSREC_ERR_ARG, "rsrec_comm_init_file: cannot publish %s", path);
    } else {
        const auto t0 = std::chrono::steady_clock::now();
        for (;;) {
            FILE* f = fopen(path, "rb");
            if (f) {
                const size_t got = fread(id, 1, sizeof id, f);
                fclose(f);
                if (got == sizeof id) break;
            }
            if (std::chrono::duration<double>(std::chrono::steady_clock::now() - t0).count() > timeout_s)
                return fail(h, RSREC_ERR_DEVICE, "rsrec_comm_init_file: no id at %s after %.0f s", path, timeout_s);
            std::this_thread::sleep_for(std::chrono::milliseconds(20));
        }
    }
    return rsrec_comm_init(h, rank, nranks, id);
}

extern "C" int rsrec_allreduce_sum(rsrec_t* h, double* buf, size_t n) {
    if (!h || (!buf && n > 0)) return fail(h, RSREC_ERR_ARG, "rsrec_allreduce_sum: bad argument");
    if (n == 0) return RSREC_OK;
    HIPCK(h, hipSetDevice(h->device));
    if (!h->comm) { HIPCK(h, hipStreamSynchronize(h->stream)); return RSREC_OK; }
    const bool dev = is_device_ptr(buf);
    double* d = buf;
    if (!dev) {
        HIPCK(h, h->d_comm.reserve(n * sizeof(double)));
        d = h->d_comm.as<double>();
        XFER(xfer_h2d(h, d, buf, n * sizeof(double)));
    }
    const int rc = g_rccl.all_reduce(d, d, n, 8 , 0 , h->comm, h->stream);
    if (rc != 0) return fail(h, RSREC_ERR_DEVICE, "ncclAllReduce failed: %s", rccl_err(rc));
    if (!dev) XFER(xfer_d2h(h, buf, d, n * sizeof(double)));
    HIPCK(h, hipStreamSynchronize(h->stream));
    return RSREC_OK;
}

extern "C" int rsrec_comm_size(rsrec_t* h, int* rank, int* nranks) {
    if (!h) return RSREC_ERR_ARG;
    if (rank) *rank = h->comm_rank;
    if (nranks) *nranks = h->comm ? h->comm_nranks : 1;
    return RSREC_OK;
}

extern "C" int rsrec_zsqr(rsrec_t* h, int nmat, double* b2_b) {
    if (!h || nmat < 0 || (nmat > 0 && !b2_b)) return fail(h, RSREC_ERR_ARG, "rsrec_zsqr: bad argument");
    if (nmat == 0) return RSREC_OK;
    HIPCK(h, hipSetDevice(h->device));
    const size_t bytes = (size_t)nmat * BLK * sizeof(double2);
    HIPCK(h, h->d_zsqr.reserve(bytes));
    HIPCK(h, h->d_status.reserve(64));
    HIPCK(h, hipMemsetAsync(h->d_status.p, 0, 64, h->stream));
    XFER(xfer_h2d(h, h->d_zsqr.p, b2_b, bytes));
    k_zsqr<<<nmat, 256, 0, h->stream>>>(h->d_zsqr.as<double2>(), h->d_status.as<int>());
    HIPCK(h, hipGetLastError());
    XFER(xfer_d2h(h, b2_b, h->d_zsqr.p, bytes));
    return finish_status(h);
}

namespace {

template <class Launch>
int green_pipeline(rsrec_t* h, int nsites, size_t gbytes, double* g0, Launch launch) {
    if (!h->copy_stream) HIPCK(h, hipStreamCreateWithFlags(&h->copy_stream, hipStreamNonBlocking));
    for (hipEvent_t& e : h->ev_green)
        if (!e) HIPCK(h, hipEventCreateWithFlags(&e, hipEventDisableTiming));
    const size_t cap = ((size_t)1 << 29) / gbytes;
    const int chunk = (int)std::max<size_t>(1, std::min<size_t>(cap, ((size_t)nsites + 7) / 8));
    HIPCK(h, h->d_green_out.reserve(2 * (size_t)chunk * gbytes));
    char* out[2] = {static_cast<char*>(h->d_green_out.p), static_cast<char*>(h->d_green_out.p) + (size_t)chunk * gbytes};
    std::vector<std::pair<hipEvent_t, hipEvent_t>> spans;
    auto drain = [&](int s0, int ns, int b) -> int {
        HIPCK(h, hipStreamWaitEvent(h->copy_stream, h->ev_green[b], 0));
        HIPCK(h, hipMemcpyAsync(reinterpret_cast<char*>(g0) + (size_t)s0 * gbytes, out[b], (size_t)ns * gbytes, hipMemcpyDeviceToHost, h->copy_stream));
        HIPCK(h, hipStreamSynchronize(h->copy_stream));
        return RSREC_OK;
    };
    int prev_s0 = -1, prev_ns = 0, c = 0;
    for (int s0 = 0; s0 < nsites; s0 += chunk, ++c) {
        const int ns = std::min(chunk, nsites - s0);
        hipEvent_t k0 = next_event(h);
        launch(s0, ns, out[c & 1]);
        hipEvent_t k1 = next_event(h);
        HIPCK(h, hipGetLastError());
        HIPCK(h, hipEventRecord(h->ev_green[c & 1], h->stream));
// ... 1727 lines not shown
```

### rslmtoasa_amd/recursion.py

```python
import ctypes as C
import os
from dataclasses import dataclass, field

import numpy as np

from . import _lib


@dataclass
class Control:
    lld: int = 21
    llsp: int = 0
    nsp: int = 2
    recur: str = "block"


@dataclass
class Energy:
    energy_min: float = -1.0
    energy_max: float = 1.0


@dataclass
class Lattice:
    nn: np.ndarray
    iz: np.ndarray
    irec: np.ndarray
    nmax: int = 0
    ntype: int = 1
    ijpair: np.ndarray = None
    cr: np.ndarray = None

    @property
    def kk(self):
        return self.nn.shape[0]

    @property
    def nrec(self):
        return len(self.irec)


@dataclass
class Hamiltonian:
    ee: np.ndarray
    lsham: np.ndarray
    eeo: np.ndarray = None
    enim: np.ndarray = None
    hall: np.ndarray = None
    hallo: np.ndarray = None
    hoh: bool = False
    local_axis: bool = False


def site_partition(rank, nprocs, nsites):
    s, e = C.c_int(), C.c_int()
    _lib.lib().rsrec_site_partition(rank, nprocs, nsites, C.byref(s), C.byref(e))
    return s.value, e.value


def chebyshev_scaling(energy_min, energy_max):
    a = (energy_max - energy_min) / float(np.float32(2) - np.float32(0.3))
    b = (energy_max + energy_min) / 2
    return a, b


def _fc(a, dtype):
    return np.asfortranarray(np.asarray(a, dtype=dtype))


def _ptr(a):
    return None if a is None else a.ctypes.data_as(C.c_void_p)


class Recursion:

    def __init__(self, hamiltonian, lattice, control, energy=None, device=0, rank=0, nprocs=1):
        self.hamiltonian, self.lattice, self.control, self.en = hamiltonian, lattice, control, energy or Energy()
        self.rank, self.nprocs = rank, nprocs
        self._L = _lib.lib()
        self._h = C.c_void_p()
        rc = self._L.rsrec_create(C.byref(self._h), device)
        if rc != 0:
            raise _lib.RsrecError(rc, "rsrec_create failed (no usable gfx950 device? there is no CPU fallback)")
        self.restore_to_default()
        self.update_lattice()
        self.update_hamiltonian()

    def close(self):
        if getattr(self, "_h", None) is not None and self._h.value:
            self._L.rsrec_destroy(self._h)
            self._h = C.c_void_p()

    def __del__(self):
        try:
            self.close()
        except Exception:
            pass

    def _check(self, rc):
        if rc != 0:
            buf = C.create_string_buffer(512)
            self._L.rsrec_last_error(self._h, buf, 512)
            raise _lib.RsrecError(rc, buf.value.decode(errors="replace"))

    def set_option(self, key, value):
        self._check(self._L.rsrec_set_option(self._h, key.encode(), int(value)))


    def timing(self):
        out = (C.c_double * 13)()
        self._L.rsrec_get_timing(self._h, out, 13)
        keys = ("total_ms", "hop_ms", "hop_launches", "atom_steps", "block_multiplies", "rest_ms", "host_ms", "hop_fuses_a", "hop_mfma_flop", "hop_required_flop",
                "operator_arrays_from_device", "octet_launches", "rotate_ms")
        return dict(zip(keys, list(out)))

    def restore_to_default(self):
        lat, ctl = self.lattice, self.control
        llmax = max(ctl.llsp, ctl.lld)
        nrec = lat.nrec
        njij = 0 if lat.ijpair is None else len(lat.ijpair)
        nsites = nrec if njij == 0 else 4 * njij
        self.a = np.zeros((llmax, 18, nrec, 3), np.float64, order="F")
        self.b2 = np.zeros((llmax, 18, nrec, 3), np.float64, order="F")
        self.a_b = np.zeros((18, 18, ctl.lld, nsites), np.complex128, order="F")
        self.b2_b = np.zeros((18, 18, ctl.lld, nsites), np.complex128, order="F")
        self.mu_n = np.zeros((18, 18, 2 * ctl.lld + 2, nsites), np.complex128, order="F")
        self.mu_ng = np.zeros_like(self.mu_n)

    def update_lattice(self):
        lat = self.lattice
        self._nn = _fc(lat.nn, np.int32)
        self._iz = _fc(lat.iz, np.int32)
        self._check(self._L.rsrec_set_lattice(self._h, lat.kk, self._nn.shape[1], _ptr(self._nn), _ptr(self._iz), int(lat.nmax), int(lat.ntype)))
        if lat.cr is not None:
            cr = _fc(lat.cr, np.float64)
            assert cr.shape == (3, lat.kk)
            self._check(self._L.rsrec_set_positions(self._h, _ptr(cr)))

    def update_hamiltonian(self):
        ham = self.hamiltonian
        keep = {}
        for k in ("ee", "lsham", "eeo", "enim", "hall", "hallo"):
            v = getattr(ham, k)
            keep[k] = None if v is None else _fc(v, np.complex128)
        self._ham_keep = keep
        self._check(self._L.rsrec_set_hamiltonian(self._h, keep["ee"].shape[2], int(bool(ham.hoh)), int(self.control.nsp),
                                                  _ptr(keep["ee"]), _ptr(keep["lsham"]), _ptr(keep["eeo"]), _ptr(keep["enim"]),
                                                  _ptr(keep["hall"]), _ptr(keep["hallo"])))

    def _assemble(self, part, hmag, nbr_type, obarm):
        hoh = bool(self.hamiltonian.hoh)
        hm = _fc(hmag, np.complex128)
        assert hm.ndim == 5 and hm.shape[:2] == (9, 9) and hm.shape[3] == 4, "hmag is (9,9,nslots,4,ncls)"
        nslots, ncls = hm.shape[2], hm.shape[4]
        ty = ob = None
        ntype = 0
        if hoh:
            ty, ob = _fc(nbr_type, np.int32), _fc(obarm, np.complex128)
            assert ty.shape == (nslots, ncls) and ob.shape[:2] == (18, 18)
            ntype = ob.shape[2]
        blocks = np.zeros((18, 18, nslots, ncls), np.complex128, order="F")
        blocks_o = np.zeros_like(blocks) if hoh else None
        self._check(self._L.rsrec_assemble_blocks(self._h, part, ncls, nslots, int(hoh), _ptr(hm), _ptr(ty), _ptr(ob), ntype, _ptr(blocks), _ptr(blocks_o)))
        return blocks, blocks_o

    def build_bulkham(self, hmag, nbr_type=None, obarm=None):
        self.hamiltonian.ee, eeo = self._assemble(0, hmag, nbr_type, obarm)
        if eeo is not None:
            self.hamiltonian.eeo = eeo

    def build_locham(self, hmag, nbr_type=None, obarm=None):
        self.hamiltonian.hall, hallo = self._assemble(1, hmag, nbr_type, obarm)
        if hallo is not None:
            self.hamiltonian.hallo = hallo

    def _my_sites(self):
        start, end = site_partition(self.rank, self.nprocs, self.lattice.nrec)
        return start, end, np.ascontiguousarray(self.lattice.irec[start - 1:end], dtype=np.int32)

    def recur_b(self):
        lld = self.control.lld
        start, end, seeds = self._my_sites()
        n = len(seeds)
        a_b = np.zeros((18, 18, lld, n), np.complex128, order="F")
        b2_b = np.zeros_like(a_b)
        self._check(self._L.rsrec_block_lanczos(self._h, n, _ptr(seeds), lld, _ptr(a_b), _ptr(b2_b)))
        self.a_b[:, :, :, :n] = a_b
        self.b2_b[:, :, :, :n] = b2_b
        d = np.arange(18)
        self.a[:lld, :, :n, 0] = a_b[d, d].real.transpose(1, 0, 2)
        self.b2[:lld, :, :n, 0] = b2_b[d, d].real.transpose(1, 0, 2)

    def recur_b_local_axis(self, rot):
        lld = self.control.lld
        start, end, seeds = self._my_sites()
        n = len(seeds)
        r = _fc(np.asarray(rot)[:, :, start - 1:end], np.complex128)
        a_b = np.zeros((18, 18, lld, n), np.complex128, order="F")
        b2_b = np.zeros_like(a_b)
        self._check(self._L.rsrec_block_lanczos_local_axis(self._h, n, _ptr(seeds), _ptr(r), lld, _ptr(a_b), _ptr(b2_b)))
        self.a_b[:, :, :, :n] = a_b
        self.b2_b[:, :, :, :n] = b2_b
        d = np.arange(18)
        self.a[:lld, :, :n, 0] = a_b[d, d].real.transpose(1, 0, 2)
        self.b2[:lld, :, :n, 0] = b2_b[d, d].real.transpose(1, 0, 2)

    def pack_diag(self, site_offset, nsites_total, a_img, b2_img):
        pa = a_img if isinstance(a_img, int) else a_img.ctypes.data
        pb = b2_img if isinstance(b2_img, int) else b2_img.ctypes.data
        self._check(self._L.rsrec_pack_diag(self._h, int(site_offset), int(nsites_total), C.c_void_p(pa), C.c_void_p(pb)))

    def pack_moments(self, site_offset, nsites_total, mu_img):
        pm = mu_img if isinstance(mu_img, int) else mu_img.ctypes.data
        self._check(self._L.rsrec_pack_moments(self._h, int(site_offset), int(nsites_total), C.c_void_p(pm)))

    @staticmethod
    def comm_unique_id():
        buf = C.create_string_buffer(128)
        if _lib.lib().rsrec_comm_unique_id(buf) != 0:
            raise _lib.RsrecError(2, "rsrec_comm_unique_id failed (RCCL not available?)")
        return buf.raw

    def comm_init(self, rank, nranks, ident=None, path=None, timeout_s=60.0):
        if path is not None:
            self._check(self._L.rsrec_comm_init_file(self._h, int(rank), int(nranks), os.fsencode(path), float(timeout_s)))
        else:
            self._check(self._L.rsrec_comm_init(self._h, int(rank), int(nranks), ident))

    def comm_size(self):
        r, n = C.c_int(), C.c_int()
        self._check(self._L.rsrec_comm_size(self._h, C.byref(r), C.byref(n)))
        return r.value, n.value

    def allreduce_sum(self, buf, n=None):
        if isinstance(buf, int):
            self._check(self._L.rsrec_allreduce_sum(self._h, C.c_void_p(buf), int(n)))
        else:
            if buf.dtype not in (np.float64, np.complex128):
                raise TypeError("allreduce_sum: float64 or complex128 arrays only, got %s" % buf.dtype)
            if not (buf.flags["C_CONTIGUOUS"] or buf.flags["F_CONTIGUOUS"]):
                raise ValueError("allreduce_sum: the array must be contiguous (it is reduced in place)")
            self._check(self._L.rsrec_allreduce_sum(self._h, C.c_void_p(buf.ctypes.data), buf.nbytes // 8))

    def recur_b_ij(self):
        lld = self.control.lld
        pairs = np.asarray(self.lattice.ijpair, dtype=np.int32)
        njij = len(pairs)
        start, end = site_partition(self.rank, self.nprocs, njij)
        slots, sa, sc = self._pair_seeds(pairs[start - 1:end], skip_diagonal_repeats=True)
        nch = len(slots)
        a_b = np.zeros((18, 18, lld, nch), np.complex128, order="F")
        b2_b = np.zeros_like(a_b)
        self._check(self._L.rsrec_block_lanczos_seeded(self._h, nch, 2, _ptr(sa), _ptr(sc), lld, _ptr(a_b), _ptr(b2_b)))
        self.a_b[:, :, :, slots] = a_b
        self.b2_b[:, :, :, slots] = b2_b

    @staticmethod
    def _pair_seeds(pairs, skip_diagonal_repeats):
        s2 = 1.0 / np.sqrt(2.0)
        slots, seeds, coefs = [], [], []
        for ij_loc, (i, j) in enumerate(pairs):
            for reci in range(4):
                a, b = s2, (s2, -s2, 1j * s2, -1j * s2)[reci]
                if i == j and skip_diagonal_repeats:
                    if reci > 0:
                        continue
                    a = b = 1.0
                seeds.append((i, j)); coefs.append((a, b))
                slots.append(ij_loc * 4 + reci)
        return slots, np.ascontiguousarray(seeds, dtype=np.int32), np.ascontiguousarray(coefs, dtype=np.complex128)

    def chebyshev_recur_ij(self):
        lld = self.control.lld
        a, b = chebyshev_scaling(self.en.energy_min, self.en.energy_max)
        pairs = np.asarray(self.lattice.ijpair, dtype=np.int32)
        start, end = site_partition(self.rank, self.nprocs, len(pairs))
        slots, sa, sc = self._pair_seeds(pairs[start - 1:end], skip_diagonal_repeats=False)
        nch = len(slots)
        mu = np.zeros((18, 18, 2 * lld + 2, nch), np.complex128, order="F")
        self._check(self._L.rsrec_chebyshev_seeded(self._h, nch, 2, _ptr(sa), _ptr(sc), lld, a, b, _ptr(mu)))
        self.mu_n[:, :, :, slots] = mu

    def zsqr(self):
        self._check(self._L.rsrec_zsqr(self._h, self.b2_b.shape[2] * self.b2_b.shape[3], _ptr(self.b2_b)))

    def chebyshev_recur(self):
        lld = self.control.lld
        a, b = chebyshev_scaling(self.en.energy_min, self.en.energy_max)
        start, end, seeds = self._my_sites()
        n = len(seeds)
        mu = np.zeros((18, 18, 2 * lld + 2, n), np.complex128, order="F")
        self._check(self._L.rsrec_chebyshev(self._h, n, _ptr(seeds), lld, a, b, _ptr(mu)))
        self.mu_n[:, :, :, :n] = mu

    def compute_moments_stochastic(self, v_a, v_b, cond_ll, vo_a=None, vo_b=None, seeds=None, coefs=None, atlist=None, diag=False,
                                   resident_only=False):
        a, b = chebyshev_scaling(self.en.energy_min, self.en.energy_max)
        if seeds is None:
            seeds = np.asarray(atlist, dtype=np.int32).reshape(-1, 1)
            coefs = np.ones(seeds.shape, np.complex128)
        seeds = np.ascontiguousarray(seeds, dtype=np.int32)
        coefs = np.ascontiguousarray(coefs, dtype=np.complex128)
        nvec, nseed = seeds.shape
        keep = [None if v is None else _fc(v, np.complex128) for v in (v_a, vo_a, v_b, vo_b)]
        if diag:
            mu = None if resident_only else np.zeros((18, cond_ll, cond_ll, nvec), np.complex128, order="F")
            self._check(self._L.rsrec_kubo_moments_diag(self._h, nvec, nseed, _ptr(seeds), _ptr(coefs), int(cond_ll), a, b,
                                                        _ptr(keep[0]), _ptr(keep[1]), _ptr(keep[2]), _ptr(keep[3]), _ptr(mu)))
            self.mu_diag_resident = (int(cond_ll), nvec)
            return mu
        mu = np.zeros((18, 18, cond_ll, cond_ll, nvec), np.complex128, order="F")
        self._check(self._L.rsrec_kubo_moments(self._h, nvec, nseed, _ptr(seeds), _ptr(coefs), int(cond_ll), a, b,
                                               _ptr(keep[0]), _ptr(keep[1]), _ptr(keep[2]), _ptr(keep[3]), _ptr(mu)))
        self.mu_nm_stochastic = mu
        return mu

    def ham_vec_matmul(self, psi_in, a, b):
        x = _fc(psi_in, np.complex128)
        out = np.zeros_like(x)
        self._check(self._L.rsrec_apply_operator(self._h, 2, None, None, _ptr(x), _ptr(out), float(a), float(b)))
        return out

    def ham_hoh_vec_matmul(self, psi_in, a, b):
        x = _fc(psi_in, np.complex128)
        out = np.zeros_like(x)
        self._check(self._L.rsrec_apply_operator(self._h, 0, None, None, _ptr(x), _ptr(out), float(a), float(b)))
        return out

    def chebyshev_orbital_mod(self, cr, alat, seeds=None, per_seed=False):
        lld = self.control.lld
        a, b = chebyshev_scaling(self.en.energy_min, self.en.energy_max)
        kk = self.lattice.kk
        sd = np.arange(1, kk + 1, dtype=np.int32) if seeds is None else np.ascontiguousarray(seeds, dtype=np.int32)
        crf = _fc(cr, np.float64)
        assert crf.shape == (3, kk)
        mu = np.zeros((18, 18, lld), np.complex128, order="F")
        ms = np.zeros((18, 18, lld, len(sd)), np.complex128, order="F") if per_seed else None
        self._check(self._L.rsrec_orbital_moments(self._h, len(sd), _ptr(sd), lld, a, b, _ptr(crf), float(alat), _ptr(mu), _ptr(ms)))
        if seeds is None:
            mu = mu / float(kk)
        return (mu, ms) if per_seed else mu

    def velo_vec_matmul(self, v_op, psi_in, vo_op=None):
        x = _fc(psi_in, np.complex128)
        out = np.zeros_like(x)
        v = _fc(v_op, np.complex128)
        vo = None if vo_op is None else _fc(vo_op, np.complex128)
        self._check(self._L.rsrec_apply_operator(self._h, 1, _ptr(v), _ptr(vo), _ptr(x), _ptr(out), 1.0, 0.0))
        return out

    def recur(self):
        lld = self.control.lld
        llmax = self.a.shape[0]
        start, end, seeds = self._my_sites()
        n = len(seeds)
        a = np.zeros((llmax, 18, n), np.float64, order="F")
        b2 = np.zeros_like(a)
        self._check(self._L.rsrec_scalar_lanczos(self._h, n, _ptr(seeds), lld, llmax, _ptr(a), _ptr(b2)))
        self.a[:, :, :n, 0] = a
        self.b2[:, :, :n, 0] = b2
```

Measured before the change: 65540.

## Fold the A_n Gram product into the Hamiltonian SpMM epilogue for Hermitian operators

Adds a GRAM variant of the SpMM kernel that computes per-group partial Gram blocks <psi|H psi> from the freshly computed H|psi> tiles while they are still in registers. The partials go to a scratch buffer, and a small groupsum kernel turns them into the same partial images the reduction expects. The separate k_mfma_adot pass over psi and hpsi is skipped on levels where every chain has enough groups. It only applies when a host-side check finds the Hamiltonian Hermitian with opposite neighbour slots, because it stores a compact set of Gram pieces and reconstructs the rest by symmetry. In exchange it adds a gram scratch buffer, extra MFMA work and register pressure inside the SpMM, and one more launch per level.

Result: faster. 67740 (median of 6 runs) (+3.4%).

```diff
diff --git a/rslmtoasa_amd/csrc/kernels_mfma.hpp b/rslmtoasa_amd/csrc/kernels_mfma.hpp
--- a/rslmtoasa_amd/csrc/kernels_mfma.hpp
+++ b/rslmtoasa_amd/csrc/kernels_mfma.hpp
@@ -117,13 +117,62 @@
 #endif
 }
 
+constexpr int S5_GRAM_DOUBLES = 584;
+constexpr long S5_GRAM_MIN_NEVER = 1L << 40;
+constexpr int S5_GRAM_MAXW = 8;
+__host__ __device__ inline bool s5_gram_folds(long ngroups, long min_groups) { return ngroups > 0 && ngroups >= min_groups; }
+__host__ __device__ inline int s5_gram_workgroups(int ngroups) { return ngroups / 4 < 1 ? 1 : (ngroups / 4 < S5_GRAM_MAXW ? ngroups / 4 : S5_GRAM_MAXW); }
+struct GramFold { const int* cum = nullptr; int nlev = 0; long min_groups = 0; };
+
+__global__ __launch_bounds__(640) void k_gram_groupsum(GramFold F, int level, const double* __restrict__ gpart, size_t cstride, double* __restrict__ partial ) {
+    __shared__ double sm[S5_GRAM_DOUBLES];
+    const int chain = blockIdx.y, w = blockIdx.x;
+    const int ngroups = F.cum[(size_t)chain * F.nlev + level] / GROUP;
+    if (!s5_gram_folds(ngroups, F.min_groups)) return;
+    double* img = partial + ((size_t)chain * gridDim.x + w) * 1296;
+    const int nw = s5_gram_workgroups(ngroups);
+    if (w >= nw) {
+        for (int e = threadIdx.x; e < 1296; e += blockDim.x) img[e] = 0.0;
+        return;
+    }
+    const size_t g0 = (size_t)w * ngroups / nw, g1 = (size_t)(w + 1) * ngroups / nw;
+    if (threadIdx.x < S5_GRAM_DOUBLES) {
+        const double* src = gpart + (size_t)chain * cstride + threadIdx.x;
+        double s = 0.0;
+        size_t q = 2 * g0;
+        for (; q + 16 <= 2 * g1; q += 16) {
+            double v[16];
+#pragma unroll
+            for (int i = 0; i < 16; ++i) v[i] = ld_stream(src + (q + i) * S5_GRAM_DOUBLES);
+#pragma unroll
+            for (int i = 0; i < 16; ++i) s += v[i];
+        }
+        for (; q < 2 * g1; ++q) s += ld_stream(src + q * S5_GRAM_DOUBLES);
+        sm[threadIdx.x] = s;
+    }
+    __syncthreads();
+    for (int e = threadIdx.x; e < 1296; e += blockDim.x) {
+        const int r = e / 36, c = e - 36 * r, a = r >> 1, b = c >> 1, part = c & 1;
+        double v = 0.0;
+        if ((r & 1) == 0) {
+            if (a < 16 && b < 16) v = sm[256 * part + 4 * (16 * (a & 3) + b) + (a >> 2)];
+            else if (a >= 16 && b < 16) v = sm[512 + 2 * (16 * (a - 16) + b) + part];
+            else if (a >= 16) v = sm[576 + 2 * (2 * (a - 16) + (b - 16)) + part];
+            else { const double t = sm[512 + 2 * (16 * (b - 16) + a) + part]; v = part ? -t : t; }
+        }
+        img[e] = v;
+    }
+}
+
 #ifndef ADOT_UNROLL
 #define ADOT_UNROLL 4
 #endif
 __global__ __launch_bounds__(MF_WAVES * 64, 2) void k_mfma_adot(ChainView CV, int level, int zero_block, const double* __restrict__ psi,
-                                                               const double* __restrict__ tvec, double* partial ) {
+                                                               const double* __restrict__ tvec, double* partial ,
+                                                               GramFold F = GramFold() ) {
     __shared__ double lds[MF_WAVES * 1296];
     const int chain = blockIdx.y;
+    if (F.cum && s5_gram_folds(F.cum[(size_t)chain * F.nlev + level] / GROUP, F.min_groups)) return;
     const int lane = threadIdx.x & 63;
     const int wave = __builtin_amdgcn_readfirstlane(threadIdx.x >> 6);
     const int ngroups = CV.count_of(chain, level) / GROUP;
diff --git a/rslmtoasa_amd/csrc/kernels_spmm5.hpp b/rslmtoasa_amd/csrc/kernels_spmm5.hpp
--- a/rslmtoasa_amd/csrc/kernels_spmm5.hpp
+++ b/rslmtoasa_amd/csrc/kernels_spmm5.hpp
@@ -588,7 +588,9 @@
 
 struct S5Epilogue { int kind = 0; const double* cur = nullptr; const double* old = nullptr; double a = 1.0, b = 0.0; };
 
-template <bool TWO, bool LDSA, bool OCT = false, int NSP = 1>
+struct S5Gram { double* out = nullptr; size_t cstride = 0; long min_groups = 0; };
+
+template <bool TWO, bool LDSA, bool OCT = false, int NSP = 1, bool GRAM = false>
 __global__ __launch_bounds__(NSP == 3 ? 768 : S5_WG_GROUPS * 128) void k_spmm5(SpmmDims D, const int* __restrict__ order_all, const int* __restrict__ cum,
                                                const int* __restrict__ nbr ,
                                                const int* __restrict__ izp, const double* __restrict__ frag, const int* __restrict__ meta, int ntr,
@@ -598,7 +600,8 @@
                                                int ntau = 0, int lds_tau = 0 ,
                                                int* __restrict__ queue = nullptr ,
                                                int spin_by_xcd = 1 ,
-                                               S5Epilogue epi = S5Epilogue()) {
+                                               S5Epilogue epi = S5Epilogue(), S5Gram gram = S5Gram()) {
+    static_assert(!GRAM || (!TWO && !OCT && NSP == 1), "the Gram epilogue: one input, whole groups of atoms");
     extern __shared__ double s5_lds[];
     const int lane = threadIdx.x & 63;
     const int wave = __builtin_amdgcn_readfirstlane(threadIdx.x >> 6);
@@ -640,6 +643,7 @@
     for (int chain = OCT ? GROUP * (int)blockIdx.y : (int)blockIdx.y; chain < D.nchains; chain += OCT ? GROUP * (int)gridDim.y : (int)gridDim.y) {
     const int count = cum[(chain / D.cpo) * D.nlev + D.level];
     int ngroups = count / GROUP;
+    const bool fold = GRAM && gram.out != nullptr && epi.kind == 0 && s5_gram_folds(ngroups, gram.min_groups);
     const int ob = D.obase[(chain / D.cpo) * D.nlev + D.level];
     const int* __restrict__ order = order_all + (size_t)(chain / D.cpo) * D.ostride + ob;
     const bool on_full_list = D.sat_base > 0 && ob == D.sat_base;
@@ -839,6 +843,105 @@
         if (kpart) continue;
 #endif
 
+        if constexpr (GRAM) if (fold) {
+            unsigned gl;
+            asm volatile("v_mbcnt_lo_u32_b32 %0, -1, 0\n\tv_mbcnt_hi_u32_b32 %0, -1, %0" : "=v"(gl));
+            const int lane = (int)gl, l15 = lane & 15, l4 = lane >> 4;
+            const double* __restrict__ ub = in_all + vo;
+            double4_t gre = {0, 0, 0, 0}, gim = {0, 0, 0, 0};
+            double sre[2] = {0.0, 0.0}, sim[2] = {0.0, 0.0}, kre[2] = {0.0, 0.0}, kim[2] = {0.0, 0.0};
+            auto rem_coef = [&](s5_d2 u, double& cr, double& ci) {
+                cr = l4 == 0 ? u[0] : (l4 == 1 ? u[1] : 0.0);
+                ci = l4 == 0 ? -u[1] : (l4 == 1 ? u[0] : 0.0);
+            };
+            auto gram_tiles = [&](auto t0c, auto t1c) {
+                constexpr int T0 = decltype(t0c)::value, T1 = decltype(t1c)::value, NT = T1 - T0;
+                s5_d2 gu[NT][3], gs[NT][3][2];
+#pragma unroll
+                for (int i = 0; i < NT; ++i) {
+                    const int t = T0 + i;
+                    const double* ab = ub + (size_t)BLD * ((t < 8) ? vatom[t] : my_rem_atom) + 324 * sig;
+#pragma unroll
+                    for (int p = 0; p < 3; ++p) {
+                        const int row = 36 * (p < 2 ? 4 * p + l4 : 8);
+                        if (t < 8) gu[i][p] = *reinterpret_cast<const s5_d2*>(ab + row + 2 * l15);
+#pragma unroll
+                        for (int e = 0; e < 2; ++e) gs[i][p][e] = *reinterpret_cast<const s5_d2*>(ab + row + 32 + 2 * e);
+                    }
+                }
+#pragma unroll
+                for (int i = 0; i < NT; ++i) {
+                    const int t = T0 + i;
+                    const double x8 = acc.r[t];
+                    if (t < 8) {
+#pragma unroll
+                        for (int p = 0; p < 2; ++p) {
+                            gre = __builtin_amdgcn_mfma_f64_16x16x4f64(gu[i][p][0], acc.m[t][2 * p], gre, 0, 0, 0);
+                            gre = __builtin_amdgcn_mfma_f64_16x16x4f64(gu[i][p][1], acc.m[t][2 * p + 1], gre, 0, 0, 0);
+                            gim = __builtin_amdgcn_mfma_f64_16x16x4f64(-gu[i][p][1], acc.m[t][2 * p], gim, 0, 0, 0);
+                            gim = __builtin_amdgcn_mfma_f64_16x16x4f64(gu[i][p][0], acc.m[t][2 * p + 1], gim, 0, 0, 0);
+                        }
+                        double cr, ci;
+                        rem_coef(gu[i][2], cr, ci);
+                        gre = __builtin_amdgcn_mfma_f64_16x16x4f64(cr, x8, gre, 0, 0, 0);
+                        gim = __builtin_amdgcn_mfma_f64_16x16x4f64(ci, x8, gim, 0, 0, 0);
+                    }
+                    double (&are)[2] = (t < 8) ? sre : kre;
+                    double (&aim)[2] = (t < 8) ? sim : kim;
+#pragma unroll
+                    for (int e = 0; e < 2; ++e) {
+#pragma unroll
+                        for (int p = 0; p < 2; ++p) {
+                            const double ur = gs[i][p][e][0], ui = gs[i][p][e][1], tr = acc.m[t][2 * p], ti = acc.m[t][2 * p + 1];
+                            are[e] = fma(ur, tr, are[e]); are[e] = fma(ui, ti, are[e]);
+                            aim[e] = fma(ur, ti, aim[e]); aim[e] = fma(-ui, tr, aim[e]);
+                        }
+                        double cr, ci;
+                        rem_coef(gs[i][2][e], cr, ci);
+                        are[e] = fma(cr, x8, are[e]);
+                        aim[e] = fma(ci, x8, aim[e]);
+                    }
+                }
+            };
+            gram_tiles(S5C<0>{}, S5C<2>{});
+            __builtin_amdgcn_sched_barrier(0);
+            gram_tiles(S5C<2>{}, S5C<4>{});
+            __builtin_amdgcn_sched_barrier(0);
+            gram_tiles(S5C<4>{}, S5C<6>{});
+            __builtin_amdgcn_sched_barrier(0);
+            gram_tiles(S5C<6>{}, S5C<8>{});
+            __builtin_amdgcn_sched_barrier(0);
+            gram_tiles(S5C<8>{}, S5C<9>{});
+            __builtin_amdgcn_sched_barrier(0);
+            auto sum_l4 = [&](double v) {
+                double s = __shfl(v, l15);
+                s += __shfl(v, l15 + 16); s += __shfl(v, l15 + 32); s += __shfl(v, l15 + 48);
+                return s;
+            };
+            auto sum_atoms = [&](double v) {
+                double s = __shfl(v, l15 & 1);
+#pragma unroll
+                for (int a = 1; a < GROUP; ++a) s += __shfl(v, 2 * a + (l15 & 1));
+                return s;
+            };
+            double* gp = gram.out + (size_t)chain * gram.cstride + ((size_t)g * 2 + sig) * S5_GRAM_DOUBLES;
+            s5_d2 v;
+#pragma unroll
+            for (int p = 0; p < 2; ++p) {
+                v[0] = gre[2 * p]; v[1] = gre[2 * p + 1];
+                *reinterpret_cast<s5_d2*>(gp + 4 * lane + 2 * p) = v;
+                v[0] = gim[2 * p]; v[1] = gim[2 * p + 1];
+                *reinterpret_cast<s5_d2*>(gp + 256 + 4 * lane + 2 * p) = v;
+            }
+#pragma unroll
+            for (int e = 0; e < 2; ++e) {
+                v[0] = sum_l4(sre[e]); v[1] = sum_l4(sim[e]);
+                if (l4 == e) *reinterpret_cast<s5_d2*>(gp + 512 + 2 * (16 * e + l15)) = v;
+                v[0] = sum_atoms(sum_l4(kre[e])); v[1] = sum_atoms(sum_l4(kim[e]));
+                if (lane < 2) *reinterpret_cast<s5_d2*>(gp + 576 + 2 * (2 * e + lane)) = v;
+            }
+        }
+        const int ekind = GRAM ? 0 : epi.kind;
         auto finish = [&](auto t0c, auto t1c) {
             constexpr int T0 = decltype(t0c)::value, T1 = decltype(t1c)::value, NT = T1 - T0;
             size_t eo[NT];
@@ -846,7 +949,7 @@
             for (int i = 0; i < NT; ++i) { const int t = T0 + i; eo[i] = (size_t)BLD * ((t < 8) ? vatom[t] : my_rem_atom) + 324 * sig + ((t < 8) ? 2 * l15 : 32 + 2 * (l15 & 1)); }
             s5_d2 ec[NT][2], ez[NT][2];
             double ecr[NT], ezr[NT];
-            if (epi.kind) {
+            if (ekind) {
                 const double* cb = epi.cur + vo;
 #pragma unroll
                 for (int i = 0; i < NT; ++i) {
@@ -854,7 +957,7 @@
                     for (int p = 0; p < 2; ++p) ec[i][p] = *reinterpret_cast<const s5_d2*>(cb + eo[i] + 36 * (4 * p + l4));
                     ecr[i] = cb[eo[i] + 288 + (l4 & 1)];
                 }
-                if (epi.kind == 2) {
+                if (ekind == 2) {
                     const double* zb = epi.old + vo;
 #pragma unroll
                     for (int i = 0; i < NT; ++i) {
@@ -872,16 +975,16 @@
 #pragma unroll
                 for (int p = 0; p < 2; ++p) {
                     s5_d2 v; v[0] = acc.m[t][2 * p]; v[1] = acc.m[t][2 * p + 1];
-                    if (epi.kind) {
+                    if (ekind) {
                         v[0] = (v[0] - epi.b * ec[i][p][0]) / epi.a; v[1] = (v[1] - epi.b * ec[i][p][1]) / epi.a;
-                        if (epi.kind == 2) { v[0] = v[0] * 2.0 - ez[i][p][0]; v[1] = v[1] * 2.0 - ez[i][p][1]; }
+                        if (ekind == 2) { v[0] = v[0] * 2.0 - ez[i][p][0]; v[1] = v[1] * 2.0 - ez[i][p][1]; }
                     }
                     if (a != zero_block) *reinterpret_cast<s5_d2*>(ob + 36 * (4 * p + l4)) = v;
                 }
                 double r = acc.r[t];
-                if (epi.kind) {
+                if (ekind) {
                     r = (r - epi.b * ecr[i]) / epi.a;
-                    if (epi.kind == 2) r = r * 2.0 - ezr[i];
+                    if (ekind == 2) r = r * 2.0 - ezr[i];
                 }
                 if (a != zero_block && l4 < 2) ob[288 + l4] = r;
             }
diff --git a/rslmtoasa_amd/csrc/rsrec.hip b/rslmtoasa_amd/csrc/rsrec.hip
--- a/rslmtoasa_amd/csrc/rsrec.hip
+++ b/rslmtoasa_amd/csrc/rsrec.hip
@@ -123,6 +123,12 @@
     int kubo_diag_nvec = 0, kubo_diag_ll = 0;
     long opt_orth3 = 1;
     long opt_graph = 1;
+    long opt_s5_gram_min = 256;
+    int ham_hermitian = 0;
+    std::vector<int> opp_slot;
+    int opp_epoch = -1;
+    DevBuf d_gram;
+    double n_gram_folded = 0, n_gram_all = 0, n_gram_levels = 0;
     hipGraphExec_t graph_exec = nullptr;
     std::vector<uintptr_t> graph_key;
     bool capturing = false;
@@ -139,6 +145,7 @@
         double atom_steps, block_mults;
         DevBuf order, cum;
         std::vector<int> level_max;
+        std::vector<int> hop_min, hop_max;
         std::vector<double> level_groups;
         std::vector<double> mult_hist;
         struct ClassRun { int tau, lo, hi; };
@@ -190,6 +197,7 @@
     {"s5_octet", &rsrec_handle::opt_s5_octet},
     {"s5_spin_xcd", &rsrec_handle::opt_s5_spin_xcd},
     {"s5_run_min", &rsrec_handle::opt_s5_run_min},
+    {"s5_gram_min", &rsrec_handle::opt_s5_gram_min},
 };
 
 int fail(rsrec_t* h, int code, const char* fmt, ...) {
@@ -409,9 +417,9 @@
 
 extern "C" int rsrec_get_timing(rsrec_t* h, double* out, int n) {
     if (!h || !out) return RSREC_ERR_ARG;
-    const double v[13] = {h->t_total_ms, h->t_hop_ms, h->n_hop_launch, h->n_atom_steps, h->n_block_mult, h->t_rest_ms, h->t_host_ms, (double)h->hop_fuses_a, h->n_hop_mfma_flop,
-                          h->n_req_flop, (double)h->n_asm_reused, (double)h->n_octet_launch, h->t_rot_ms};
-    for (int i = 0; i < n && i < 13; ++i) out[i] = v[i];
+    const double v[14] = {h->t_total_ms, h->t_hop_ms, h->n_hop_launch, h->n_atom_steps, h->n_block_mult, h->t_rest_ms, h->t_host_ms, (double)h->hop_fuses_a, h->n_hop_mfma_flop,
+                          h->n_req_flop, (double)h->n_asm_reused, (double)h->n_octet_launch, h->t_rot_ms, h->n_gram_folded};
+    for (int i = 0; i < n && i < 14; ++i) out[i] = v[i];
     return RSREC_OK;
 }
 
@@ -527,6 +535,47 @@
     return RSREC_OK;
 }
 
+namespace {
+
+bool check_hermitian(rsrec_t* h, const double* st) {
+    if (h->ntype != 1 || h->nmax != 0 || h->hoh) return false;
+    const int ns = h->nslots, kk = h->kk;
+    if (h->opp_epoch != h->lattice_epoch) {
+        h->opp_epoch = h->lattice_epoch;
+        std::vector<int> opp(ns, -1);
+        bool ok = true;
+        opp[0] = 0;
+        for (int i = 0; i < kk && ok; ++i)
+            for (int s = 1; s < ns && ok; ++s) {
+                const int j = h->nbr[(size_t)i * ns + s];
+                if (j < 0) continue;
+                int back = -1, nback = 0;
+                for (int q = 0; q < ns; ++q) if (h->nbr[(size_t)j * ns + q] == i) { back = q; ++nback; }
+                if (nback != 1 || back == 0 || (opp[s] >= 0 && opp[s] != back)) ok = false;
+                else opp[s] = back;
+            }
+        for (int s = 0; s < ns && ok; ++s) if (opp[s] < 0 || opp[opp[s]] != s) ok = false;
+        if (!ok) opp.clear();
+        h->opp_slot.swap(opp);
+    }
+    if (h->opp_slot.empty()) return false;
+    const size_t B = 2 * (size_t)BLK;
+    double big = 0.0;
+    for (size_t e = 0; e < B * ns; ++e) big = std::max(big, std::fabs(st[e]));
+    const double tol = 1e-12 * big;
+    for (int s = 0; s < ns; ++s) {
+        const double *a = st + B * s, *b = st + B * h->opp_slot[s];
+        for (int r = 0; r < NB; ++r)
+            for (int c = 0; c < NB; ++c) {
+                const double dr = b[2 * (c + NB * r)] - a[2 * (r + NB * c)], di = b[2 * (c + NB * r) + 1] + a[2 * (r + NB * c) + 1];
+                if (!(std::fabs(dr) <= tol && std::fabs(di) <= tol)) return false;
+            }
+    }
+    return true;
+}
+
+}
+
 extern "C" int rsrec_set_hamiltonian(rsrec_t* h, int nslots, int hoh, int nsp, const double* ee, const double* lsham, const double* eeo,
                                      const double* enim, const double* hall, const double* hallo) {
     if (!h) return RSREC_ERR_ARG;
@@ -549,6 +598,7 @@
     if (!hoh)
         for (int t = 0; t < ntype; ++t)
             for (size_t e = 0; e < B; ++e) st[B * nslots * t + e] += lsham[B * t + e];
+    h->ham_hermitian = check_hermitian(h, st.data()) ? 1 : 0;
     h->n_asm_reused = 0;
     auto resident = [&](int part, int which, const double* arr, int ncls) -> const double* {
         const size_t n = B * nslots * ncls;
@@ -655,13 +705,14 @@
     int batch = 1, nblk = 1;
 };
 
-int plan_batch(rsrec_t* h, int nchains, int nvec, size_t vec_elems_per_chain, BatchPlan& bp) {
+int plan_batch(rsrec_t* h, int nchains, int nvec, size_t vec_elems_per_chain, BatchPlan& bp, size_t extra_bytes_per_chain = 0) {
     release_kubo_buffers(h, true, true);
     size_t free_b = 0, total_b = 0;
     HIPCK(h, hipMemGetInfo(&free_b, &total_b));
     size_t reusable = 0;
     for (int v = 0; v < 5; ++v) reusable += h->d_vec[v].bytes;
-    const double per_chain = (double)nvec * vec_elems_per_chain * sizeof(double2) + (double)h->kk * 4 + 4096;
+    if (extra_bytes_per_chain) reusable += h->d_gram.bytes;
+    const double per_chain = (double)nvec * vec_elems_per_chain * sizeof(double2) + (double)h->kk * 4 + 4096 + (double)extra_bytes_per_chain;
     long cap = (long)((0.85 * (double)(free_b + reusable)) / per_chain);
     if (cap < 1) return fail(h, RSREC_ERR_DEVICE, "not enough device memory for one chain (%.1f MB needed, %.1f MB free)", per_chain / 1e6, free_b / 1e6);
     long b = h->opt_batch > 0 ? h->opt_batch : 64;
@@ -836,6 +887,7 @@
     XFER(xfer_h2d(h, e->cum.p, cum.data(), cum.size() * 4));
     HIPCK(h, hipStreamSynchronize(h->stream));
     e->level_max.assign(nlev, 0);
+    e->hop_min.assign(nlev, INT32_MAX); e->hop_max.assign(nlev, 0);
     e->level_groups.assign((size_t)nlev * ntau_h, 0.0);
     {
         std::vector<double> sat_hist(ntau_h, 0.0);
@@ -853,6 +905,7 @@
             for (int l = 0; l < nlev; ++l) {
                 const int cnt = cum[(size_t)c * nlev + l];
                 e->level_max[l] = std::max(e->level_max[l], cnt);
+                e->hop_min[l] = std::min(e->hop_min[l], cnt); e->hop_max[l] = std::max(e->hop_max[l], cnt);
                 const bool sat = cum[(size_t)(nb + c) * nlev + l] == sat_off;
                 e->level_max[l] = std::max(e->level_max[l], cum[(size_t)(2 * nb + c) * nlev + l]);
                 if (sat) e->level_sat[l] += 1;
@@ -890,6 +943,7 @@
     h->t_total_ms = h->t_hop_ms = h->t_rest_ms = h->t_host_ms = h->t_rot_ms = 0;
     h->n_hop_launch = h->n_atom_steps = h->n_block_mult = h->n_hop_mfma_flop = h->n_req_flop = 0;
     h->n_octet_launch = 0;
+    h->n_gram_folded = h->n_gram_all = h->n_gram_levels = 0;
     h->ev_used = 0;
     h->n_recursion_calls++;
 }
@@ -1007,6 +1061,7 @@
         const int ask = (int)std::min<size_t>((size_t)optin, S5_LDS_LIMIT);
         if (hipFuncSetAttribute(reinterpret_cast<const void*>(k_spmm5<false, true>), hipFuncAttributeMaxDynamicSharedMemorySize, ask) == hipSuccess &&
             hipFuncSetAttribute(reinterpret_cast<const void*>(k_spmm5<true, true>), hipFuncAttributeMaxDynamicSharedMemorySize, ask) == hipSuccess &&
+            hipFuncSetAttribute(reinterpret_cast<const void*>(k_spmm5<false, true, false, 1, true>), hipFuncAttributeMaxDynamicSharedMemorySize, ask) == hipSuccess &&
             hipFuncSetAttribute(reinterpret_cast<const void*>(k_spmm5<false, true, false, 3>), hipFuncAttributeMaxDynamicSharedMemorySize, ask) == hipSuccess &&
             hipFuncSetAttribute(reinterpret_cast<const void*>(k_spmm5<true, true, false, 3>), hipFuncAttributeMaxDynamicSharedMemorySize, ask) == hipSuccess)
             h->s5_lds_limit = (size_t)ask;
@@ -1015,7 +1070,7 @@
 }
 template <bool TWO>
 void launch_s5_one(rsrec_t* h, dim3 grid, const SpmmDims& SD, const int* order, const int* cum, const int* iz, const Spmm5Operator& op, int set,
-                   const double* in, double* out, const double* in2, const double* extra, int ntau, S5Epilogue epi, int one) {
+                   const double* in, double* out, const double* in2, const double* extra, int ntau, S5Epilogue epi, int one, S5Gram gram = S5Gram()) {
     const size_t lds_bytes = (size_t)op.ntr * S5_TRIPLE * sizeof(double);
     const bool want = h->opt_s5_lds >= 1;
     s5_prepare(h);
@@ -1039,15 +1094,22 @@
             const unsigned thr3 = 64u * (unsigned)std::min<long>(12, std::max<long>(8, h->opt_s5_waves));
             const size_t lds3 = std::min(lds_limit, lds_bytes + (size_t)S5_TRIPLE_BYTES);
             k_spmm5<TWO, true, false, 3><<<g2, thr3, lds3, h->stream>>>(SD, order, cum, h->d_nbr5.as<int>(), iz, op.frag_set(set), op.meta_set(set), op.ntr, in, out, in2, nullptr, ntau, one, queue, spin_by_xcd, epi);
+        } else if constexpr (!TWO) {
+            if (gram.out) k_spmm5<false, true, false, 1, true><<<g2, thr, lds_bytes, h->stream>>>(SD, order, cum, h->d_nbr5.as<int>(), iz, op.frag_set(set), op.meta_set(set), op.ntr, in, out, in2, nullptr, ntau, one, queue, spin_by_xcd, epi, gram);
+            else k_spmm5<false, true><<<g2, thr, lds_bytes, h->stream>>>(SD, order, cum, h->d_nbr5.as<int>(), iz, op.frag_set(set), op.meta_set(set), op.ntr, in, out, in2, nullptr, ntau, one, queue, spin_by_xcd, epi);
         } else
         k_spmm5<TWO, true><<<g2, thr, lds_bytes, h->stream>>>(SD, order, cum, h->d_nbr5.as<int>(), iz, op.frag_set(set), op.meta_set(set), op.ntr, in, out, in2, nullptr, ntau, one, queue, spin_by_xcd, epi);
+    } else if constexpr (!TWO) {
+        if (gram.out) k_spmm5<false, false, false, 1, true><<<grid, S5_WG_GROUPS * 128, 0, h->stream>>>(SD, order, cum, h->d_nbr5.as<int>(), iz, op.frag_set(set), op.meta_set(set), op.ntr, in, out, in2, extra, ntau, 0, nullptr, 1, epi, gram);
+        else k_spmm5<false, false><<<grid, S5_WG_GROUPS * 128, 0, h->stream>>>(SD, order, cum, h->d_nbr5.as<int>(), iz, op.frag_set(set), op.meta_set(set), op.ntr, in, out, in2, extra, ntau, 0, nullptr, 1, epi);
     } else
         k_spmm5<TWO, false><<<grid, S5_WG_GROUPS * 128, 0, h->stream>>>(SD, order, cum, h->d_nbr5.as<int>(), iz, op.frag_set(set), op.meta_set(set), op.ntr, in, out, in2, extra, ntau, 0, nullptr, 1, epi);
 }
 
 template <bool TWO>
 void launch_s5(rsrec_t* h, dim3 grid, const SpmmDims& SD0, const int* order, const int* cum, const int* iz, const Spmm5Operator& op, int set,
-               const double* in, double* out, const double* in2 = nullptr, const double* extra = nullptr, int ntau = 0, S5Epilogue epi = S5Epilogue()) {
+               const double* in, double* out, const double* in2 = nullptr, const double* extra = nullptr, int ntau = 0, S5Epilogue epi = S5Epilogue(),
+               S5Gram gram = S5Gram() ) {
     SpmmDims SD = SD0;
     const int one = op.single_class(set);
     const rsrec_handle::RegionEntry* E = h->cur_entry;
@@ -1079,7 +1141,7 @@
         h->n_octet_launch++;
     }
     if (!multi) {
-        launch_s5_one<TWO>(h, grid, SD, order, cum, iz, op, set, in, out, in2, extra, ntau, epi, one);
+        launch_s5_one<TWO>(h, grid, SD, order, cum, iz, op, set, in, out, in2, extra, ntau, epi, one, gram);
         if (oct_aside) (void)hipStreamWaitEvent(h->stream, h->ev_oct_out, 0);
     } else {
         SD.sat_base = E->sat_base;
@@ -1201,13 +1263,14 @@
     return RC;
 }
 
-int recursion_begin(rsrec_t* h, RecursionCall& RC, int nvec, int skip_vec, int coef_slots) {
+int recursion_begin(rsrec_t* h, RecursionCall& RC, int nvec, int skip_vec, int coef_slots, size_t gram_doubles_per_chain = 0) {
     if (RC.mfma && !RC.ci) XFER(ensure_s4(h));
     RC.nvec = nvec; RC.skip_vec = skip_vec;
     BatchPlan bp;
-    XFER(plan_batch(h, RC.nchains, nvec - (skip_vec >= 0 ? 1 : 0), RC.velems / 2, bp));
+    XFER(plan_batch(h, RC.nchains, nvec - (skip_vec >= 0 ? 1 : 0), RC.velems / 2, bp, gram_doubles_per_chain * sizeof(double)));
     const int B = RC.B = bp.batch; RC.nblk = bp.nblk;
     for (int v = 0; v < nvec; ++v) if (v != skip_vec) HIPCK(h, h->d_vec[v].reserve((size_t)B * RC.velems * sizeof(double)));
+    if (gram_doubles_per_chain) HIPCK(h, h->d_gram.reserve((size_t)B * gram_doubles_per_chain * sizeof(double)));
     XFER(reserve_partials(h, B, (size_t)B * 256 * 2 * 1296 * sizeof(double)));
     XFER(ensure_side_stream(h));
     RC.side = h->opt_side && h->side_stream;
@@ -1294,7 +1357,7 @@
     return RSREC_OK;
 }
 int apply_h(rsrec_t* h, RecursionCall& RC, const RecursionBatch& b, int step, const double* src, double* dst, double* hps, const double* extra, int ntau,
-            S5Epilogue epi = S5Epilogue()) {
+            S5Epilogue epi = S5Epilogue(), S5Gram gram = S5Gram()) {
     const bool hoh = h->hoh != 0;
     const int lv_final = hoh ? 2 * step : step;
     const Spmm5Operator& OP = *RC.op; const DevProblem& P = RC.P; const ChainView& CV = b.CV;
@@ -1306,7 +1369,7 @@
         SD.level = lv_final;
         launch_s5<true>(h, s5_grid(h, b.grid_mf, lv_final), SD, CV.order, CV.cum, P.iz, OP, 1, hps, dst, src, extra, ntau, epi);
     } else if (extra) launch_s5<true>(h, s5_grid(h, b.grid_mf, lv_final), SD, CV.order, CV.cum, P.iz, OP, 0, src, dst, src, extra, ntau, epi);
-    else launch_s5<false>(h, s5_grid(h, b.grid_mf, lv_final), SD, CV.order, CV.cum, P.iz, OP, 0, src, dst, nullptr, nullptr, 0, epi);
+    else launch_s5<false>(h, s5_grid(h, b.grid_mf, lv_final), SD, CV.order, CV.cum, P.iz, OP, 0, src, dst, nullptr, nullptr, 0, epi, gram);
     RC.hop_ev.emplace_back(e0, next_event(h)); h->n_hop_launch += hoh ? 2 : 1;
     return RSREC_OK;
 }
@@ -1386,7 +1449,12 @@
     const bool oop = MFMA && h->opt_orth_oop != 0 && h->opt_orth3 != 2;
     const int nvec = MFMA ? (oop && hoh ? 5 : 4) : (hoh ? 3 : 2);
     const bool use_v1 = !MFMA || hoh || oop;
-    XFER(recursion_begin(h, RC, nvec, use_v1 ? -1 : 1, nseed));
+    const size_t gram_groups = ((size_t)kk + 7 * (size_t)(h->nmax + h->ntype) + 8 + GROUP - 1) / GROUP;
+    const bool gram_eligible = MFMA && ci && !hoh && !rot && h->ntype == 1 && h->nmax == 0 && h->ham_hermitian && h->opt_s5_split != 3 &&
+                               RC.op->single_class(0) >= 0 && (h->opt_nblk <= 0 || 2 * h->opt_nblk >= S5_GRAM_MAXW) &&
+                               s5_gram_folds((long)gram_groups, h->opt_s5_gram_min);
+    const size_t gram_cstride = gram_eligible ? gram_groups * 2 * S5_GRAM_DOUBLES : 0;
+    XFER(recursion_begin(h, RC, nvec, use_v1 ? -1 : 1, nseed, gram_cstride));
     const int B = RC.B, nblk = RC.nblk;
     HIPCK(h, h->d_frags.reserve((size_t)B * 3 * 27 * 64 * sizeof(double)));
     HIPCK(h, h->d_bmats.reserve((size_t)B * 2 * BLK * sizeof(double2)));
@@ -1404,6 +1472,13 @@
         RecursionBatch bt;
         XFER(recursion_batch(h, RC, seed_atoms, seed_coef, c0, nb, bt));
         const ChainView &CV = bt.CV, &CVp = bt.CVp;
+        const rsrec_handle::RegionEntry* RE = h->cur_entry;
+        auto fold_at = [&](int lv) -> int {
+            if (!gram_eligible || !RE || lv < 0 || lv >= (int)RE->hop_max.size()) return 0;
+            if (!s5_gram_folds(RE->hop_max[lv] / GROUP, h->opt_s5_gram_min)) return 0;
+            return s5_gram_folds(RE->hop_min[lv] / GROUP, h->opt_s5_gram_min) ? 2 : 1;
+        };
+        for (int ll = 0; ll < nsteps; ++ll) { const int f = fold_at(ll + 1); h->n_gram_folded += f > 0; h->n_gram_all += f == 2; h->n_gram_levels += 1; }
         auto enqueue_levels = [&]() -> int {
             XFER(clear_vectors(h, RC, nb, MFMA && !hoh ? 2 : -1));
             HIPCK(h, hipMemsetAsync(dA, 0, (size_t)nb * cstride * sizeof(double2), h->stream));
@@ -1421,9 +1496,13 @@
             for (int ll = 0; ll < nsteps; ++ll) {
                 const int lv_final = hoh ? 2 * ll + 2 : ll + 1;
                 if (MFMA) {
-                    XFER(apply_h(h, RC, bt, ll + 1, psi, hpsi, pmn, bt.la_extra, ntau));
+                    const int folds = fold_at(lv_final);
+                    const GramFold GF{folds ? CV.cum : nullptr, RC.nlev, h->opt_s5_gram_min};
+                    XFER(apply_h(h, RC, bt, ll + 1, psi, hpsi, pmn, bt.la_extra, ntau, S5Epilogue(),
+                                 folds ? S5Gram{h->d_gram.as<double>(), gram_cstride, h->opt_s5_gram_min} : S5Gram()));
                     const dim3 gl = level_grid(h, bt.grid_mf, lv_final);
-                    k_mfma_adot<<<gl, MF_WAVES * 64, 0, h->stream>>>(CVp, lv_final, kk, psi, hpsi, gpartial);
+                    if (folds < 2) k_mfma_adot<<<gl, MF_WAVES * 64, 0, h->stream>>>(CVp, lv_final, kk, psi, hpsi, gpartial, GF);
+                    if (folds) k_gram_groupsum<<<gl, 640, 0, h->stream>>>(GF, lv_final, h->d_gram.as<double>(), gram_cstride, gpartial);
                     int n2 = gl.x; const double* p2 = presum(h, gpartial, nb, n2, 1296);
                     XFER(side_reduce_wait(h, SR));
                     k_reduce_a_u<<<nb, 1024, 0, h->stream>>>(p2, n2, dA + (size_t)ll * BLK, cstride, h->d_bmats.as<double2>(), bfrags, ci);
@@ -1469,7 +1548,7 @@
                                           (uintptr_t)h->d_status.p, (uintptr_t)h->d_seed.p, (uintptr_t)h->d_seedcoef.p, (uintptr_t)h->d_la_extra.p, (uintptr_t)h->d_s5queue.p,
                                           (uintptr_t)h->cur_entry, (uintptr_t)h->p2_slot, (uintptr_t)OP.single_class(0), (uintptr_t)OP.spin_mixing,
                                           (uintptr_t)h->lattice_epoch, (uintptr_t)OP.sched_epoch, (uintptr_t)h->nslots, (uintptr_t)h->nmax, (uintptr_t)h->ntype, (uintptr_t)h->hslots,
-                                          (uintptr_t)B, (uintptr_t)h->n_cu};
+                                          (uintptr_t)B, (uintptr_t)h->n_cu, (uintptr_t)h->d_gram.p, (uintptr_t)gram_eligible};
             for (int v = 0; v < nvec; ++v) key.push_back((uintptr_t)h->d_vec[v].p);
             for (const OptionEntry& o : OPTIONS)
                 if (o.member != &rsrec_handle::opt_graph) key.push_back((uintptr_t)(h->*o.member));
@@ -1481,6 +1560,7 @@
         XFER(xfer_d2h(h, b2_b + (size_t)c0 * cstride * 2, dB, (size_t)nb * cstride * sizeof(double2)));
         HIPCK(h, hipStreamSynchronize(h->stream));
     }
+    if (MFMA && h->n_gram_levels > 0 && h->n_gram_all == h->n_gram_levels) h->hop_fuses_a = 1;
     return recursion_end(h, RC, 1, lld, seed_coef != nullptr);
 }
 
diff --git a/rslmtoasa_amd/recursion.py b/rslmtoasa_amd/recursion.py
--- a/rslmtoasa_amd/recursion.py
+++ b/rslmtoasa_amd/recursion.py
@@ -108,10 +108,10 @@
 
 
     def timing(self):
-        out = (C.c_double * 13)()
-        self._L.rsrec_get_timing(self._h, out, 13)
+        out = (C.c_double * 14)()
+        self._L.rsrec_get_timing(self._h, out, 14)
         keys = ("total_ms", "hop_ms", "hop_launches", "atom_steps", "block_multiplies", "rest_ms", "host_ms", "hop_fuses_a", "hop_mfma_flop", "hop_required_flop",
-                "operator_arrays_from_device", "octet_launches", "rotate_ms")
+                "operator_arrays_from_device", "octet_launches", "rotate_ms", "gram_folded_launches")
         return dict(zip(keys, list(out)))
 
     def restore_to_default(self):
```
